# Simon-Kotchou/ViT.rs

Hardware: AMD Instinct MI355X
Metric: images/sec (train step) ViT-B/16 224² bf16 at 1/2/4/8 MI355X; % MFMA roofline (higher is better)
Workload: dtype bf16; 1 GPU; vit_b16 224x224 train step (fwd+bwd+SGD), batch 256/GPU, bf16; model=vit_b16, global_batch=256, seq_len=197, parallelism=dp1

## Files before the change

### include/vit_ops.h

```cpp
#ifndef VIT_OPS_H
#define VIT_OPS_H

#include <stddef.h>
#include <stdint.h>

#ifdef __cplusplus
extern "C" {
#endif

int vit_init(int device);
void vit_set_stream(void* hip_stream);
void* vit_get_stream(void);
int vit_sync(void);
int vit_last_error(const char** msg);
void vit_clear_error(void);
void* vit_malloc(size_t bytes);
void vit_free(void* p);
int vit_memcpy_h2d(void* dst, const void* src, size_t bytes);
int vit_memcpy_d2h(void* dst, const void* src, size_t bytes);
int vit_memcpy_d2d(void* dst, const void* src, size_t bytes);
int vit_memset(void* dst, int value, size_t bytes);
enum {
    VIT_HIT_GEMM_128 = 0,
    VIT_HIT_GEMM_256x256 = 16,
// ... 22 lines not shown
float vit_event_elapsed_ms(void* start, void* stop);

void residual_forward(float* out, const float* inp1, const float* inp2, int N);
void matmul_forward(float* out, const float* inp, const float* weight, const float* bias,
                    int B, int T, int C, int OC);
void attention_forward(float* out, float* preatt, float* att, const float* inp,
                       int B, int T, int C, int NH);
void layernorm_forward(float* out, float* mean, float* rstd, const float* inp,
                       const float* weight, const float* bias, int B, int T, int C);
void gelu_forward(float* out, const float* inp, int N);
void softmax_forward(float* probs, const float* logits, int B, int T, int V);
void crossentropy_forward(float* losses, const float* probs, const int* targets,
                          int B, int T, int V);
void residual_backward(float* dinp1, float* dinp2, const float* dout, int N);
void matmul_backward(float* dinp, float* dweight, float* dbias, const float* dout,
                     const float* inp, const float* weight, int B, int T, int C, int OC);
void attention_backward(float* dinp, float* dpreatt, float* datt, const float* dout,
                        const float* inp, const float* att, int B, int T, int C, int NH);
void layernorm_backward(float* dinp, float* dweight, float* dbias, const float* dout,
                        const float* inp, const float* weight, const float* mean,
                        const float* rstd, int B, int T, int C);
void gelu_backward(float* dinp, const float* inp, const float* dout, int N);
void crossentropy_softmax_backward(float* dlogits, const float* dlosses, const float* probs,
                                   const int* targets, int B, int T, int V);
void softmax_crossentropy_soft_forward(float* probs, float* losses, const float* logits,
                                       const int* ta, const int* tb, float lam, float eps,
                                       int B, int T, int V);
void crossentropy_soft_softmax_backward(float* dlogits, const float* dlosses, const float* probs,
                                        const int* ta, const int* tb, float lam, float eps,
                                        int B, int T, int V);
void patch_embed_forward(float* encoded, const float* pixels, const float* patch_w,
                         const float* patch_b, const float* cls, const float* wpe,
                         int B, int IMG, int P, int C);
void patch_embed_backward(float* dpatch_w, float* dpatch_b, float* dcls, float* dwpe,
                          const float* dencoded, const float* pixels, int B, int IMG, int P,
                          int C);
void sgd_step(float* params, const float* grads, long long n, float lr);
void grad_sumsq(double* out, const float* x, long long n);

void matmul_forward_bf16(uint16_t* out, const uint16_t* inp, const uint16_t* weight,
                         const float* bias, int B, int T, int C, int OC);
void matmul_backward_bf16(float* dinp, float* dweight, float* dbias, const uint16_t* dout,
                          const uint16_t* inp, const uint16_t* weight, int B, int T, int C,
                          int OC);
int vit_attention_kernel_kind(int T, int C, int NH);
void attention_forward_fused_bf16(uint16_t* out, float* lse, const uint16_t* inp,
                                  int B, int T, int C, int NH);
void attention_backward_fused_bf16(uint16_t* dinp, const uint16_t* dout, const uint16_t* inp,
                                   const uint16_t* out, const float* lse, int B, int T, int C,
                                   int NH);
void attention_backward_fused_bf16_ex(uint16_t* dinp, const uint16_t* dout, const uint16_t* inp,
                                      const uint16_t* out, const float* lse, int B, int T, int C, int NH,
                                      float* dqkv_bias);
void layernorm_forward_bf16(uint16_t* out, float* mean, float* rstd, const float* inp,
                            const float* weight, const float* bias, int B, int T, int C);
void layernorm_backward_bf16(float* dinp, float* dweight, float* dbias, const uint16_t* dout,
                             const float* inp, const float* weight, const float* mean,
                             const float* rstd, int B, int T, int C);
void gelu_forward_bf16(uint16_t* out, const uint16_t* inp, int N);
void gelu_backward_bf16(float* dinp, const uint16_t* inp, const uint16_t* dout, int N);
void gemm_bf16_ex(void* C, long long ldc, const uint16_t* A, long long lda, int a_kcontig,
                  const uint16_t* B, long long ldb, int b_kcontig, const float* bias,
                  float* dbias, int M, int N, int K, int epi, int splitk);
void gemm_bf16_fused(void* C, void* C2, long long ldc, const void* aux, long long ldaux,
                     const uint16_t* A, long long lda, int a_kcontig, const uint16_t* B,
                     long long ldb, int b_kcontig, const float* bias, float* colsum_out, int M,
                     int N, int K, int epi);
long long mx_scale_size(long long rows, int K);
void quantize_mx_bf16_ex(uint8_t* q, uint8_t* scales, const uint16_t* x, long long R, int K,
                         long long ldx, long long ldq);
void quantize_mx_f32_ex(uint8_t* q, uint8_t* scales, const float* x, long long R, int K,
                        long long ldx, long long ldq);
long long mx_cols_padded(long long R);
void quantize_mx_cols_bf16_ex(uint8_t* q, uint8_t* scales, const uint16_t* x, long long R, int C,
                              long long ldx);
void quantize_mx_rowcol_bf16_ex(uint8_t* qr, uint8_t* scales_r, uint8_t* qc, uint8_t* scales_c,
                                const uint16_t* x, long long R, int C, long long ldx, long long ldqc,
                                long long tok_off, long long ntok);
void layernorm_backward_stream(uint16_t* dres_out, uint8_t* lo_out, const uint16_t* dres_in, const uint8_t* lo_in,
                               float* dweight, float* dbias, float* dres_colsum, const uint16_t* dout, const float* inp,
                               const float* weight, const float* mean, const float* rstd, long long R, int C);
void layernorm_backward_stream_mx(uint16_t* dres_out, uint8_t* lo_out, const uint16_t* dres_in, const uint8_t* lo_in,
                                  float* dweight, float* dbias, float* dres_colsum, const uint16_t* dout,
                                  const float* inp, const float* weight, const float* mean, const float* rstd,
                                  long long R, int C, uint8_t* qr, uint8_t* scales_r, uint8_t* qc, uint8_t* scales_c,
                                  long long ldqc, long long tok_off, long long ntok);
void layernorm_forward_mx(uint8_t* qr, uint8_t* scales_r, uint8_t* qc, uint8_t* scales_c, float* mean,
                          float* rstd, const float* inp, const float* weight, const float* bias, long long R,
                          int C, long long ldqc, long long tok_off, long long ntok);
void gemm_fp8_fused(void* C, void* C2, long long ldc, const void* aux, long long ldaux,
                    const uint8_t* A, const uint8_t* a_scale, long long lda, const uint8_t* B,
                    const uint8_t* b_scale, long long ldb, const float* bias, float* colsum_out,
                    int M, int N, int K, int epi);
void gemm_fp8_fused_mx(void* C, void* C2, long long ldc, const void* aux, long long ldaux, const uint8_t* A,
                       const uint8_t* a_scale, long long lda, const uint8_t* B, const uint8_t* b_scale,
                       long long ldb, const float* bias, float* colsum_out, int M, int N, int K, int epi,
                       uint8_t* mx_q, uint8_t* mx_s);
void gemm_fp8_fused_mxc(void* C, void* C2, long long ldc, const void* aux, long long ldaux, const uint8_t* A,
                        const uint8_t* a_scale, long long lda, const uint8_t* B, const uint8_t* b_scale,
                        long long ldb, const float* bias, float* colsum_out, int M, int N, int K, int epi,
                        uint8_t* mx_q, uint8_t* mx_s, uint8_t* mxc_q, uint8_t* mxc_s, long long mxc_ld,
                        long long mxc_off);
void gemm_bf16_set_variant(int variant);
void gemm_bf16_set_debug(int flags);
void gemm_bf16_set_trace(unsigned long long* trace);
void convert_f32_to_bf16(uint16_t* out, const float* inp, long long n);
// ... 7 lines not shown
```

### vit.rs_amd/__init__.py

```python
import ctypes
import os
import sys

import numpy as np

HERE = os.path.dirname(os.path.abspath(__file__))
LIB_PATH = os.environ.get("VIT_LIB") or os.path.join(HERE, "libvit_hip.so")

from . import data
from . import mix
from . import groups
from . import augment

VIT_FP32, VIT_BF16, VIT_FP8 = 0, 1, 2
MIX_NONE, MIX_MIXUP, MIX_CUTMIX = 0, 1, 2
_lib = None


class VitError(RuntimeError):
    pass


class VitConfigC(ctypes.Structure):
    _fields_ = [("img", ctypes.c_int), ("patch", ctypes.c_int), ("in_ch", ctypes.c_int),
# ... 10 lines not shown
    _fields_ = [("cfg", VitConfigC), ("num_params", ctypes.c_longlong), ("has_opt", ctypes.c_int),
                ("step", ctypes.c_int), ("adamw", AdamWC)]


def _cfg_c(cfg):
    return VitConfigC(cfg.img, cfg.patch, cfg.in_ch, cfg.channels, cfg.num_layers, cfg.num_heads,
                      cfg.num_classes)


def build(quiet=True):
    import subprocess
    jobs = str(min(8, os.cpu_count() or 1))
    subprocess.run(["make", "-s", "-j", jobs, "-C", HERE], check=True,
                   stdout=subprocess.DEVNULL if quiet else None)


_VOID = [("vit_clear_error", []), ("vit_set_stream", [ctypes.c_void_p]),
         ("vit_free", [ctypes.c_void_p]), ("vit_event_destroy", [ctypes.c_void_p]),
         ("vit_trainer_destroy", [ctypes.c_void_p]), ("vit_trainer_timing_reset", [ctypes.c_void_p]),
         ("vit_loader_close", [ctypes.c_void_p]), ("vit_jpeg_loader_close", [ctypes.c_void_p]), ("vit_kernel_hits_reset", [])]

P, I, LL, F, S = ctypes.c_void_p, ctypes.c_int, ctypes.c_longlong, ctypes.c_float, ctypes.c_size_t
_SIGS = {
    "vit_init": (I, [I]), "vit_get_stream": (P, []), "vit_sync": (I, []),
    "vit_last_error": (I, [ctypes.POINTER(ctypes.c_char_p)]),
    "vit_malloc": (P, [S]), "vit_memcpy_h2d": (I, [P, P, S]), "vit_memcpy_d2h": (I, [P, P, S]),
    "vit_memcpy_d2d": (I, [P, P, S]), "vit_memset": (I, [P, I, S]),
    "vit_event_create": (P, []), "vit_event_record": (I, [P]), "vit_event_elapsed_ms": (F, [P, P]),
    "residual_forward": (None, [P, P, P, I]),
    "matmul_forward": (None, [P, P, P, P, I, I, I, I]),
    "attention_forward": (None, [P, P, P, P, I, I, I, I]),
    "layernorm_forward": (None, [P, P, P, P, P, P, I, I, I]),
    "gelu_forward": (None, [P, P, I]),
    "softmax_forward": (None, [P, P, I, I, I]),
    "crossentropy_forward": (None, [P, P, P, I, I, I]),
    "residual_backward": (None, [P, P, P, I]),
    "matmul_backward": (None, [P, P, P, P, P, P, I, I, I, I]),
    "attention_backward": (None, [P, P, P, P, P, P, I, I, I, I]),
    "layernorm_backward": (None, [P, P, P, P, P, P, P, P, I, I, I]),
    "gelu_backward": (None, [P, P, P, I]),
    "crossentropy_softmax_backward": (None, [P, P, P, P, I, I, I]),
    "softmax_crossentropy_soft_forward": (None, [P, P, P, P, P, F, F, I, I, I]),
    "crossentropy_soft_softmax_backward": (None, [P, P, P, P, P, F, F, I, I, I]),
    "patch_embed_forward": (None, [P, P, P, P, P, P, I, I, I, I]),
    "patch_embed_backward": (None, [P, P, P, P, P, P, I, I, I, I]),
    "sgd_step": (None, [P, P, LL, F]),
    "grad_sumsq": (None, [P, P, LL]),
    "matmul_forward_bf16": (None, [P, P, P, P, I, I, I, I]),
    "matmul_backward_bf16": (None, [P, P, P, P, P, P, I, I, I, I]),
    "attention_forward_fused_bf16": (None, [P, P, P, I, I, I, I]),
    "vit_attention_kernel_kind": (I, [I, I, I]),
    "attention_backward_fused_bf16": (None, [P, P, P, P, P, I, I, I, I]),
    "attention_backward_fused_bf16_ex": (None, [P, P, P, P, P, I, I, I, I, P]),
    "layernorm_forward_bf16": (None, [P, P, P, P, P, P, I, I, I]),
    "layernorm_backward_bf16": (None, [P, P, P, P, P, P, P, P, I, I, I]),
    "gelu_forward_bf16": (None, [P, P, I]),
    "gelu_backward_bf16": (None, [P, P, P, I]),
    "gemm_bf16_ex": (None, [P, LL, P, LL, I, P, LL, I, P, P, I, I, I, I, I]),
    "gemm_bf16_fused": (None, [P, P, LL, P, LL, P, LL, I, P, LL, I, P, P, I, I, I, I]),
    "mx_scale_size": (LL, [LL, I]),
    "quantize_mx_bf16_ex": (None, [P, P, P, LL, I, LL, LL]),
    "quantize_mx_f32_ex": (None, [P, P, P, LL, I, LL, LL]),
    "mx_cols_padded": (LL, [LL]),
    "quantize_mx_cols_bf16_ex": (None, [P, P, P, LL, I, LL]),
    "quantize_mx_rowcol_bf16_ex": (None, [P, P, P, P, P, LL, I, LL, LL, LL, LL]),
    "layernorm_forward_mx": (None, [P, P, P, P, P, P, P, P, P, LL, I, LL, LL, LL]),
    "layernorm_backward_stream": (None, [P, P, P, P, P, P, P, P, P, P, P, P, LL, I]),
    "layernorm_backward_stream_mx": (None, [P, P, P, P, P, P, P, P, P, P, P, P, LL, I, P, P, P, P, LL, LL, LL]),
    "gemm_fp8_fused": (None, [P, P, LL, P, LL, P, P, LL, P, P, LL, P, P, I, I, I, I]),
    "gemm_fp8_fused_mx": (None, [P, P, LL, P, LL, P, P, LL, P, P, LL, P, P, I, I, I, I, P, P]),
    "gemm_fp8_fused_mxc": (None, [P, P, LL, P, LL, P, P, LL, P, P, LL, P, P, I, I, I, I, P, P, P, P, LL, LL]),
    "gemm_bf16_set_variant": (None, [I]), "gemm_bf16_set_debug": (None, [I]),
    "gemm_bf16_set_trace": (None, [P]),
    "vit_kernel_hits": (I, [P, I]),
    "convert_f32_to_bf16": (None, [P, P, LL]),
    "convert_bf16_to_f32": (None, [P, P, LL]),
    "vit_trainer_create": (P, [ctypes.POINTER(VitConfigC), I, I, I]),
    "vit_trainer_num_params": (LL, [P]), "vit_trainer_device_bytes": (LL, [P]),
    "vit_trainer_set_params": (I, [P, P]), "vit_trainer_get_params": (I, [P, P]),
    "vit_trainer_get_grads": (I, [P, P]), "vit_trainer_set_batch": (I, [P, P, P]),
    "vit_trainer_set_batch_device": (I, [P, P, P]),
    "vit_trainer_set_label_smoothing": (I, [P, F]),
    "vit_trainer_mix_batch": (I, [P, I, F, I, I, I, I]),
    "vit_trainer_get_pixels": (I, [P, P]),
    "vit_trainer_forward": (I, [P, I]), "vit_trainer_zero_grad": (I, [P]),
    "vit_trainer_backward": (I, [P]), "vit_trainer_step": (I, [P, F]),
    "vit_trainer_train_step": (I, [P, F, I]), "vit_trainer_mean_loss": (F, [P]),
    "vit_trainer_get_logits": (I, [P, P]), "vit_trainer_sync": (I, [P]),
    "vit_trainer_stream": (P, [P]),
    "vit_layout_query": (I, [ctypes.POINTER(VitConfigC), P, P, ctypes.POINTER(LL)]),
    "vit_dp_unique_id_size": (I, []), "vit_dp_get_unique_id": (I, [ctypes.c_char_p]),
    "vit_trainer_dp_init": (I, [P, I, I, ctypes.c_char_p, I]),
    "vit_trainer_dp_ranks": (I, [P]),
    "vit_trainer_get_dp_snapshot": (I, [P, P]),
    "vit_trainer_set_timing": (I, [P, I]), "vit_trainer_set_concurrency": (I, [P, I]),
    "vit_trainer_set_option": (I, [P, ctypes.c_char_p, I]),
    "vit_trainer_timing": (I, [P, ctypes.POINTER(ctypes.c_char_p), ctypes.POINTER(ctypes.c_double),
                               ctypes.POINTER(ctypes.c_longlong), ctypes.POINTER(ctypes.c_double), I]),
    "vit_trainer_step_adamw": (I, [P, F, F, F, F, F]),
    "vit_trainer_get_adamw_state": (I, [P, P, P, ctypes.POINTER(I)]),
    "vit_trainer_set_grad_clip": (I, [P, F]), "vit_trainer_grad_norm": (F, [P]),
    "vit_trainer_set_param_groups": (I, [P, P, P]),
    "vit_trainer_get_param_groups": (I, [P, P, P, ctypes.POINTER(I)]),
    "vit_trainer_eval": (I, [P, P, ctypes.POINTER(I)]),
    "vit_config_num_params": (LL, [ctypes.POINTER(VitConfigC)]),
    "vit_checkpoint_read_info": (I, [ctypes.c_char_p, P]),
# ... 591 lines not shown
```

### vit.rs_amd/csrc/attention.hip

```cpp
#include <string>

#include "attn_fused.h"

namespace vit {

__global__ __launch_bounds__(256) void attn_fwd_f32_k(float* __restrict__ out,
                                                      float* __restrict__ preatt,
                                                      float* __restrict__ att,
                                                      const float* __restrict__ inp, int B, int T,
                                                      int C, int NH) {
    extern __shared__ float sc[];
    const int lane = threadIdx.x & 63, w = threadIdx.x >> 6;
    const long long nrows = (long long)B * T * NH;
    const long long bth = blockIdx.x * 4LL + w;
    const bool valid = bth < nrows;
    const int hs = C / NH;
    const long long C3 = 3LL * C;
    const float scale = 1.0f / sqrtf((float)hs);
    float* s = sc + w * T;
    long long b = 0, t = 0, h = 0;
    if (valid) {
        b = bth / ((long long)T * NH);
        t = (bth / NH) % T;
        h = bth % NH;
// ... 440 lines not shown
    }
}

bool attn_fused_supported(int T, int C, int NH) {
    return NH > 0 && C % NH == 0 && T >= 1 && T <= fa_max_t(C / NH) && C % 8 == 0 && !getenv("VIT_ATTN_GENERIC");
}

__global__ __launch_bounds__(256) void attn_colsum_part_k(float* __restrict__ scratch, const float* __restrict__ part,
                                                          int R, int NH, int C, int HS) {
    __shared__ float4 red[256];
    const int sh = blockIdx.x, sct = sh / NH, h = sh - sct * NH, ch = blockIdx.y, nch = gridDim.y;
    const int lpr = HS / 4, nb = 256 / lpr, d4 = threadIdx.x % lpr, lb = threadIdx.x / lpr;
    const int r0 = (int)((long long)R * ch / nch), r1 = (int)((long long)R * (ch + 1) / nch);
    float4 t[4] = {};
    const long long rs = (long long)NH * 3 * HS;
    const float* base = part + (long long)h * 3 * HS + sct * HS + 4 * d4;
    int r = lb < nb ? r0 + lb : r1;
    for (; r + 3 * nb < r1; r += 4 * nb)
#pragma unroll
        for (int u = 0; u < 4; u++) {
            const float4 v = *reinterpret_cast<const float4*>(base + (long long)(r + u * nb) * rs);
            t[u].x += v.x; t[u].y += v.y; t[u].z += v.z; t[u].w += v.w;
        }
    for (; r < r1; r += nb) {
        const float4 v = *reinterpret_cast<const float4*>(base + (long long)r * rs);
        t[0].x += v.x; t[0].y += v.y; t[0].z += v.z; t[0].w += v.w;
    }
    red[threadIdx.x] = make_float4(t[0].x + t[1].x + t[2].x + t[3].x, t[0].y + t[1].y + t[2].y + t[3].y,
                                   t[0].z + t[1].z + t[2].z + t[3].z, t[0].w + t[1].w + t[2].w + t[3].w);
    __syncthreads();
    if (lb == 0) {
        float4 a = red[d4];
        for (int j = 1; j < nb; j++) {
            const float4 b = red[j * lpr + d4];
            a.x += b.x; a.y += b.y; a.z += b.z; a.w += b.w;
        }
        *reinterpret_cast<float4*>(scratch + (long long)ch * 3 * C + sct * C + h * HS + 4 * d4) = a;
    }
}
__global__ __launch_bounds__(256) void attn_colsum_final_k(float* __restrict__ out, const float* __restrict__ scratch,
                                                           int nch, int C3, int store) {
    const int j = blockIdx.x * 256 + threadIdx.x;
    if (j >= C3) return;
    float a = 0.f;
    for (int ch = 0; ch < nch; ch++) a += scratch[(long long)ch * C3 + j];
    out[j] = store ? a : out[j] + a;
}

size_t attn_backward_ws_floats(int B, int T, int C, int NH) {
    const size_t per_bh = std::max((size_t)T, (size_t)3 * (C / NH) * (fa::ATTN_PART_ROWS + 1));
    return (size_t)B * NH * per_bh + (size_t)cdiv((long long)B * T, 256) * 3 * C;
}

void attn_forward_fused(bf16_t* out, float* lse, const bf16_t* qkv, int B, int T, int C, int NH,
                        hipStream_t s) {
    if (!attn_fused_supported(T, C, NH)) {
        if (!attn_generic_supported(T, C, NH)) {
            set_error("attention_forward_fused: unsupported shape (T=%d C=%d NH=%d)", T, C, NH);
            return;
        }
        const size_t lds = gen::lds_bytes(T, C / NH, gen::nw_fwd(C / NH));
        switch (C / NH) {
#define VIT_GEN_FWD(HS)                                                                              \
    case HS:                                                                                         \
        if (!gen_lds_attr((const void*)gen::fwd_k<HS>, lds)) { set_error("attention: LDS attribute"); return; } \
        gen::fwd_k<HS><<<dim3(B * NH, gen::CHUNKS), gen::nw_fwd(HS) * 64, lds, s>>>(out, lse, qkv, T, C, NH); \
        break;
            VIT_GEN_FWD(32) VIT_GEN_FWD(64) VIT_GEN_FWD(80) VIT_GEN_FWD(96) VIT_GEN_FWD(128)
#undef VIT_GEN_FWD
            default: set_error("attention: no generic kernel for head size %d", C / NH); return;
        }
        after_launch("attention_forward_generic");
        count_hit(VIT_HIT_ATTN_GENERIC);
        return;
    }
    bool ok = false;
    switch (C / NH) {
        case 32: ok = fa_forward_h32(out, lse, qkv, B, T, C, NH, s); break;
        case 64: ok = fa_forward_h64(out, lse, qkv, B, T, C, NH, s); break;
        case 80: ok = fa_forward_h80(out, lse, qkv, B, T, C, NH, s); break;
        case 96: ok = fa_forward_h96(out, lse, qkv, B, T, C, NH, s); break;
        case 128: ok = fa_forward_h128(out, lse, qkv, B, T, C, NH, s); break;
    }
    if (!ok) { set_error("fused attention: no kernel for T=%d head size %d", T, C / NH); return; }
    after_launch("attention_forward_fused");
}

void attn_backward_fused(bf16_t* dqkv, const bf16_t* dout, const bf16_t* qkv, const bf16_t* out,
                         const float* lse, int B, int T, int C, int NH, hipStream_t s,
                         float* dqkv_colsum, float* ws, bool colsum_store) {
    if (!attn_fused_supported(T, C, NH)) {
        if (!attn_generic_supported(T, C, NH)) {
            set_error("attention_backward_fused: unsupported shape (T=%d C=%d NH=%d)", T, C, NH);
            return;
        }
        if (!ws) ws = (float*)workspace(attn_backward_ws_floats(B, T, C, NH) * sizeof(float));
        if (!ws) return;
        const size_t lds = gen::lds_bytes(T, C / NH, gen::nw_bwd(C / NH));
        const dim3 g(B * NH, gen::CHUNKS);
        switch (C / NH) {
#define VIT_GEN_BWD(HS)                                                                            \
    case HS:                                                                                       \
        if (!gen_lds_attr((const void*)gen::bwd_q_k<HS>, lds) ||                                   \
            !gen_lds_attr((const void*)gen::bwd_kv_k<HS>, lds)) {                                  \
            set_error("attention: LDS attribute");                                                 \
            return;                                                                                \
        }                                                                                          \
        gen::bwd_q_k<HS><<<g, gen::nw_bwd(HS) * 64, lds, s>>>(dqkv, ws, dout, qkv, out, lse, T, C, NH);    \
        gen::bwd_kv_k<HS><<<g, gen::nw_bwd(HS) * 64, lds, s>>>(dqkv, ws, dout, qkv, lse, T, C, NH);        \
        break;
            VIT_GEN_BWD(32) VIT_GEN_BWD(64) VIT_GEN_BWD(80) VIT_GEN_BWD(96) VIT_GEN_BWD(128)
#undef VIT_GEN_BWD
            default: set_error("attention: no generic kernel for head size %d", C / NH); return;
        }
        after_launch("attention_backward_generic");
        count_hit(VIT_HIT_ATTN_GENERIC);
        if (dqkv_colsum) {
            if (colsum_store) VIT_HIP(hipMemsetAsync(dqkv_colsum, 0, 3 * (size_t)C * sizeof(float), s));
            colsum_bf16(dqkv_colsum, dqkv, B * T, 3 * C, 3LL * C, s, ws + (size_t)B * NH * T);
        }
        return;
    }
    const int HS = C / NH;
    if (!ws) ws = (float*)workspace(attn_backward_ws_floats(B, T, C, NH) * sizeof(float));
    if (!ws) return;
    float* part = dqkv_colsum ? ws : nullptr;
    int rows = 0;
    switch (HS) {
        case 32: rows = fa_backward_h32(dqkv, dout, qkv, out, lse, B, T, C, NH, part, s); break;
        case 64: rows = fa_backward_h64(dqkv, dout, qkv, out, lse, B, T, C, NH, part, s); break;
        case 80: rows = fa_backward_h80(dqkv, dout, qkv, out, lse, B, T, C, NH, part, s); break;
        case 96: rows = fa_backward_h96(dqkv, dout, qkv, out, lse, B, T, C, NH, part, s); break;
        case 128: rows = fa_backward_h128(dqkv, dout, qkv, out, lse, B, T, C, NH, part, s); break;
    }
    if (!rows) { set_error("fused attention backward: no kernel for T=%d head size %d", T, HS); return; }
    after_launch("attention_backward_fused");
    if (dqkv_colsum) {
        const int nch = std::min(8, B);
        float* scratch = part + (size_t)B * rows * NH * 3 * HS;
        attn_colsum_part_k<<<dim3(3 * NH, nch), 256, 0, s>>>(scratch, part, B * rows, NH, C, HS);
        attn_colsum_final_k<<<cdiv(3 * C, 256), 256, 0, s>>>(dqkv_colsum, scratch, nch, 3 * C, colsum_store ? 1 : 0);
        after_launch("attention_colsum_reduce");
    }
}

}

using namespace vit;
extern "C" {
void attention_forward(float* out, float* preatt, float* att, const float* inp, int B, int T, int C,
                       int NH) {
    attn_forward_f32(out, preatt, att, inp, B, T, C, NH, stream());
}
void attention_backward(float* dinp, float* dpreatt, float* datt, const float* dout,
                        const float* inp, const float* att, int B, int T, int C, int NH) {
    attn_backward_f32(dinp, dpreatt, datt, dout, inp, att, B, T, C, NH, stream());
}
int vit_attention_kernel_kind(int T, int C, int NH) {
    if (attn_fused_supported(T, C, NH)) return 1;
    if (attn_generic_supported(T, C, NH)) return 2;
    return 0;
}
void attention_forward_fused_bf16(uint16_t* out, float* lse, const uint16_t* inp, int B, int T,
                                  int C, int NH) {
    attn_forward_fused(out, lse, inp, B, T, C, NH, stream());
}
void attention_backward_fused_bf16(uint16_t* dinp, const uint16_t* dout, const uint16_t* inp,
                                   const uint16_t* out, const float* lse, int B, int T, int C,
                                   int NH) {
    attn_backward_fused(dinp, dout, inp, out, lse, B, T, C, NH, stream());
}
void attention_backward_fused_bf16_ex(uint16_t* dinp, const uint16_t* dout, const uint16_t* inp,
                                      const uint16_t* out, const float* lse, int B, int T, int C, int NH,
                                      float* dqkv_bias) {
    attn_backward_fused(dinp, dout, inp, out, lse, B, T, C, NH, stream(), dqkv_bias);
}
}
```

### vit.rs_amd/csrc/attn_fused.h

```cpp
#pragma once
#include "ops_internal.h"

namespace vit {
namespace fa {

#ifndef VIT_ATTN_DIAG
#define VIT_ATTN_DIAG 0
#endif
#if VIT_ATTN_DIAG & 4
static __device__ unsigned long long attn_trace[8 * 16 * 16 * 16];
#define ATTN_STAMP(k)                                                                                   \
    do {                                                                                                \
        if (blockIdx.x < 8 && it < 16 && lane == 0)                                                     \
            attn_trace[((blockIdx.x * 16 + it) * 16 + w) * 16 + (k)] = __builtin_amdgcn_s_memtime();   \
    } while (0)
#else
#define ATTN_STAMP(k) \
    do {              \
    } while (0)
#endif

constexpr float LOG2E = 1.4426950408889634f;

template <int HS>
// ... 116 lines not shown
__device__ __forceinline__ void store4(bf16_t* dst, f32x4_t v, float mul) {
    *reinterpret_cast<uint2*>(dst) = pack4_bf16(v, mul);
}

__device__ __forceinline__ __amdgpu_buffer_rsrc_t buf_rsrc(const void* base, uint32_t bytes) {
    return __builtin_amdgcn_make_buffer_rsrc(const_cast<void*>(base), (short)0, (int)bytes, 0x00020000);
}
__device__ __forceinline__ uint4 buf_ld16(__amdgpu_buffer_rsrc_t r, uint32_t off) {
    return __builtin_bit_cast(uint4, __builtin_amdgcn_raw_buffer_load_b128(r, off, 0, 0));
}
__device__ __forceinline__ float buf_ldf(__amdgpu_buffer_rsrc_t r, uint32_t off) {
    return __builtin_bit_cast(float, __builtin_amdgcn_raw_buffer_load_b32(r, off, 0, 0));
}
typedef uint32_t v2u32_t __attribute__((ext_vector_type(2)));
template <int HS>
__device__ __forceinline__ bf16x8_t frag_buf(__amdgpu_buffer_rsrc_t r, uint32_t ld_bytes, int row, int s, int lane) {
    const uint32_t off = (uint32_t)row * ld_bytes + 2u * (32 * s + 4 * (lane >> 4));
    const bf16x4_t lo = __builtin_bit_cast(bf16x4_t, __builtin_amdgcn_raw_buffer_load_b64(r, off, 0, 0));
    bf16x4_t hi = {};
    if (!(Geo<HS>::HALF && s == Geo<HS>::KS - 1))
        hi = __builtin_bit_cast(bf16x4_t, __builtin_amdgcn_raw_buffer_load_b64(r, off + 32, 0, 0));
    return __builtin_shufflevector(lo, hi, 0, 1, 2, 3, 4, 5, 6, 7);
}

__device__ __forceinline__ int gray8(int r) { return (r ^ (r >> 1)) & 7; }
__device__ __forceinline__ int sl_off(int row, int byte) { return row * 128 + ((((byte >> 4) ^ gray8(row)) << 4) | (byte & 15)); }
__device__ __forceinline__ int ds_off(int row, int byte) { return row * 64 + ((((byte >> 3) ^ gray8(row)) << 3) | (byte & 7)); }
__device__ __forceinline__ bf16x4_t lds4(const char* img, int off) { return *reinterpret_cast<const bf16x4_t*>(img + off); }
__device__ __forceinline__ bf16x4_t lds4tr(const char* img, int off) {
    return __builtin_amdgcn_ds_read_tr16_b64_v4bf16(LDS_PTR(bf16x4_t, img + off));
}
__device__ __forceinline__ bf16x8_t frag_row_sw(const char* img, int r0, int s, int lane) {
    const int i = lane & 15, g = lane >> 4;
    return __builtin_shufflevector(lds4(img, sl_off(r0 + i, 64 * s + 8 * g)), lds4(img, sl_off(r0 + i, 64 * s + 32 + 8 * g)),
                                   0, 1, 2, 3, 4, 5, 6, 7);
}
__device__ __forceinline__ bf16x8_t frag_tr_sw(const char* img, int kb, int c0, int lane) {
    const int i = lane & 15, g = lane >> 4, r = kb + 4 * g + (i >> 2), b = 2 * c0 + 8 * (i & 3);
    return __builtin_shufflevector(lds4tr(img, sl_off(r, b)), lds4tr(img, sl_off(r + 16, b)), 0, 1, 2, 3, 4, 5, 6, 7);
}
__device__ __forceinline__ bf16x8_t frag_tr_ds(const char* img, int kb, int c0, int lane) {
    const int i = lane & 15, g = lane >> 4, r = kb + 4 * g + (i >> 2), b = 2 * c0 + 8 * (i & 3);
    return __builtin_shufflevector(lds4tr(img, ds_off(r, b)), lds4tr(img, ds_off(r + 16, b)), 0, 1, 2, 3, 4, 5, 6, 7);
}

template <int HS, int NKT>
constexpr int fwd_lds_bytes() { return NKT * 16 * (Geo<HS>::SK + Geo<HS>::SV) * 2; }
template <int HS, int NKT>
constexpr int fwd_occ() { return fwd_lds_bytes<HS, NKT>() <= 80 * 1024 ? 2 : 1; }

#ifndef VIT_ATTN_FWD_BUF
#define VIT_ATTN_FWD_BUF 1
#endif
template <int HS, int NKT, int NS = NKT>
__global__ __launch_bounds__(256, (fwd_occ<HS, NKT>())) void attn_fwd_k(bf16_t* __restrict__ out,
                                                                        float* __restrict__ lse,
                                                                        const bf16_t* __restrict__ qkv,
                                                                        int T, int C, int NH) {
    using G = Geo<HS>;
    constexpr int TP = NKT * 16;
    __shared__ __attribute__((aligned(16))) bf16_t Ks[TP * G::SK];
    __shared__ __attribute__((aligned(16))) bf16_t Vs[TP * G::SV];
    const int bh = blockIdx.x, b = bh / NH, h = bh % NH;
    const long long C3 = 3LL * C;
    const bf16_t* base = qkv + (long long)b * T * C3 + h * HS;
    const int lane = threadIdx.x & 63, w = threadIdx.x >> 6, i = lane & 15, g = lane >> 4;
    [[maybe_unused]] int it = 15;
    ATTN_STAMP(0);
    [[maybe_unused]] const auto rq = buf_rsrc(base, (uint32_t)(T * C3 * 2));
    [[maybe_unused]] const auto ro = buf_rsrc(out + (long long)b * T * C + h * HS, (uint32_t)(T * C * 2));
    [[maybe_unused]] const auto rl = buf_rsrc(lse + (long long)bh * T, (uint32_t)(T * 4));
    auto load_q = [&](int qt, bf16x8_t (&qf)[G::KS]) {
#pragma unroll
        for (int s = 0; s < G::KS; s++) {
            if constexpr (VIT_ATTN_FWD_BUF) qf[s] = frag_buf<HS>(rq, (uint32_t)(C3 * 2), qt * 16 + i, s, lane);
            else qf[s] = frag_glb<HS>(base, C3, qt * 16 + i, T, s, lane);
        }
    };
    const int nqt = (T + 15) / 16;
    bf16x8_t qn[G::KS];
    load_q(w, qn);
    if constexpr (VIT_ATTN_FWD_BUF) {
        const auto rkv = buf_rsrc(base + C, (uint32_t)(T * C3 * 2 - 2 * C));
        constexpr int CH = G::CH, PER = (TP * CH + 255) / 256;
        uint4 v[2][PER];
#pragma unroll
        for (int o = 0; o < 2; o++)
#pragma unroll
            for (int j = 0; j < PER; j++) {
                const int idx = j * 256 + (int)threadIdx.x, t = idx / CH, cc = idx - t * CH;
                v[o][j] = buf_ld16(rkv, (uint32_t)t * (uint32_t)(C3 * 2) + (uint32_t)(o * C * 2) + 16 * cc);
            }
#pragma unroll
        for (int o = 0; o < 2; o++)
#pragma unroll
            for (int j = 0; j < PER; j++) {
                const int idx = j * 256 + (int)threadIdx.x, t = idx / CH, cc = idx - t * CH;
                if ((TP * CH) % 256 == 0 || idx < TP * CH)
                    *reinterpret_cast<uint4*>((o ? Vs + t * G::SV : Ks + t * G::SK) + cc * 8) = v[o][j];
            }
    } else {
        bf16_t* const img[2] = {Ks, Vs};
        const int st[2] = {G::SK, G::SV};
        const bf16_t* const src[2] = {base + C, base + 2 * C};
        const long long ld[2] = {C3, C3};
        load_images<HS, TP, 256, 2>(img, st, src, ld, T);
    }
    ATTN_STAMP(1);
    __syncthreads();
    ATTN_STAMP(2);
    const float c = LOG2E / sqrtf((float)HS);
#ifndef VIT_ATTN_FWD_SPLIT
#define VIT_ATTN_FWD_SPLIT 1
#endif
    const RowBases<HS> kb(Ks, G::SK, lane);
    for (int qt = w; qt < nqt; qt += 4) {
        const int q = qt * 16 + i;
        it = qt / 4;
        ATTN_STAMP(0);
        bf16x8_t qf[G::KS];
#pragma unroll
        for (int s = 0; s < G::KS; s++) qf[s] = qn[s];
        if (qt + 4 < nqt) load_q(qt + 4, qn);
        f32x4_t sacc[NKT];
#pragma unroll
        for (int kt = NS; kt < NKT; kt++) sacc[kt] = f32x4_t{0.f, 0.f, 0.f, 0.f};
#pragma unroll
        for (int kt = 0; kt < NS; kt++) {
            f32x4_t a = {0.f, 0.f, 0.f, 0.f};
#pragma unroll
            for (int s = 0; s < G::KS; s++) {
                if constexpr (VIT_ATTN_FWD_SPLIT) a = mfma(kb.frag(kt * 16, G::SK, s), qf[s], a);
// ... 1011 lines not shown
        bwd_slice_b<HS, NSL, NW, XK>(Ks, dSs, dq, C3, q0, T, scale, w, lane, xds_s, xk_s);
        ATTN_STAMP(4);
        __syncthreads();
        ATTN_STAMP(5);
    }
    it = 15;
    ATTN_STAMP(6);
    constexpr int NWR = NW + (XK ? 1 : 0);
    bwd_item_end<HS>(R, dq, C, key0, T, scale,
                     dsum ? dsum + ((long long)(b * NWR + w) * NH + h) * 3 * HS : nullptr, lane, it);
    ATTN_STAMP(7);
    if constexpr (XK) {
        if (xo >= 0) {
            const int o = xo, d = o < HS ? o : o - HS;
            const float v = o < HS ? xacc * scale : xacc;
            dq[(long long)(T - 1) * C3 + (o < HS ? C : 2 * C) + d] = f2bf(v);
            if (dsum) {
                float* row = dsum + ((long long)(b * NWR + NW) * NH + h) * 3 * HS;
                row[(o < HS ? HS : 2 * HS) + d] = v;
                if (o < HS) row[d] = scale * xsds * xk_s[d];
            }
        }
    }
}

template <int HS, int NKT, int KK = 2>
#ifndef VIT_ATTN_SKEW
#define VIT_ATTN_SKEW 1
#endif

struct Bwdp {
    using G = Geo<HS>;
    static constexpr int TP = NKT * 16, NW = NKT / KK, NT = NW * 64, NSL = TP / 32, CH = G::CH;
    static constexpr int SK = G::SK, SV = G::SV, SL = slice_stride<HS>(), SDS = sds_stride<HS>();
    static constexpr int K_OFF = 0;
    static constexpr int V_OFF = K_OFF + 2 * TP * SV * 2;
    static constexpr int Q_OFF = V_OFF + TP * SK * 2;
    static constexpr int D_OFF = Q_OFF + 2 * 32 * SL * 2;
    static constexpr int NDS = VIT_ATTN_SKEW ? 2 : 1;
    static constexpr int S_OFF = D_OFF + 2 * 32 * SL * 2;
    static constexpr int L_OFF = S_OFF + NDS * TP * SDS * 2;
    static constexpr int E_OFF = L_OFF + 2 * TP * 4;
    static constexpr int BYTES = E_OFF + 2 * 32 * 4;
    static constexpr int PER = (32 * CH + NT - 1) / NT;
    static constexpr int PERS = (2 * 32 * CH + NT - 1) / NT;
};
template <int HS, int NKT, int KK = 2>
constexpr bool bwdp_fits() {
    using Z = Bwdp<HS, NKT, KK>;
    return Z::BYTES <= 160 * 1024 && (64 % Geo<HS>::CH) == 0 && HS <= 64 && Z::NW <= ATTN_PART_ROWS &&
           NKT % KK == 0 && (KK == 2 ? bwd1_fits<HS, NKT>() : KK == 4 ? (HS == 64 && Z::NW <= 4) : Z::NW <= 16);
}

template <int HS, int NKT, int KK>
__global__ __launch_bounds__(NKT / KK * 64, 1) void attn_bwdp_k(bf16_t* __restrict__ dqkv,
                                                               const bf16_t* __restrict__ dout,
                                                               const bf16_t* __restrict__ qkv,
                                                               const bf16_t* __restrict__ out,
                                                               const float* __restrict__ lse, int T,
                                                               int C, int NH, int BH, float* __restrict__ dsum,
                                                               int stagger) {
    using G = Geo<HS>;
    using Z = Bwdp<HS, NKT, KK>;
    if (stagger > 0 && ((blockIdx.x >> 3) & 1)) {
        const uint64_t t0 = __builtin_amdgcn_s_memrealtime();
        while (__builtin_amdgcn_s_memrealtime() - t0 < (uint64_t)stagger) __builtin_amdgcn_s_sleep(8);
    }
    constexpr int TP = Z::TP, NW = Z::NW, NT = Z::NT, NSL = Z::NSL, SK = Z::SK, SV = Z::SV, SL = Z::SL;
    static_assert((32 * G::CH) % 64 == 0 && NT % 64 == 0, "slice pieces are whole waves");
    constexpr int KS = G::KS, CH = G::CH, PER = Z::PER, PERS = Z::PERS;
    __shared__ __attribute__((aligned(16))) char lds[Z::BYTES];
    bf16_t* Kimg = reinterpret_cast<bf16_t*>(lds + Z::K_OFF);
    bf16_t* Vst = reinterpret_cast<bf16_t*>(lds + Z::V_OFF);
    bf16_t* Qs = reinterpret_cast<bf16_t*>(lds + Z::Q_OFF);
    bf16_t* Ds = reinterpret_cast<bf16_t*>(lds + Z::D_OFF);
    bf16_t* dSs = reinterpret_cast<bf16_t*>(lds + Z::S_OFF);
    float* lse_s = reinterpret_cast<float*>(lds + Z::L_OFF);
    float* del_s = reinterpret_cast<float*>(lds + Z::E_OFF);
    const long long C3 = 3LL * C;
    const int tid = threadIdx.x, lane = tid & 63;
    const int w = __builtin_amdgcn_readfirstlane(tid >> 6);
    const int key0 = w * 16 * KK;
#ifndef VIT_ATTN_SLICE_ALL
#define VIT_ATTN_SLICE_ALL 0
#endif
    constexpr bool SPLIT_SLICE = !VIT_ATTN_SLICE_ALL && Bwdp<HS, NKT, KK>::PER == 1 && (32 * G::CH) % 64 == 0;
    const bool slice_wave = !SPLIT_SLICE || w < 32 * G::CH / 64;
    const float scale = 1.0f / sqrtf((float)HS);
    const float c = LOG2E * scale;
    auto qkv_of = [&](int bh) { return qkv + (long long)(bh / NH) * T * C3 + (bh % NH) * HS; };
    auto row_of = [&](const bf16_t* p, int bh) { return p + (long long)(bh / NH) * T * C + (bh % NH) * HS; };
    uint4 pq[PER], pd[PER], po[PER];
    struct Src { __amdgpu_buffer_rsrc_t q, d, o, kv, l; };
    auto src_of = [&](int bh) {
        Src r;
        r.q = buf_rsrc(qkv_of(bh), (uint32_t)(T * C3 * 2));
        r.d = buf_rsrc(row_of(dout, bh), (uint32_t)(T * C * 2));
        r.o = buf_rsrc(row_of(out, bh), (uint32_t)(T * C * 2));
        r.kv = buf_rsrc(qkv_of(bh) + C, (uint32_t)(T * C3 * 2 - 2 * C));
        r.l = buf_rsrc(lse + (long long)bh * T, (uint32_t)(T * 4));
        return r;
    };
    auto fetch_slice = [&](const Src& sr, int q0) {
        const auto rq = sr.q, rd = sr.d, ro = sr.o;
#pragma unroll
        for (int j = 0; j < PER; j++) {
            const int idx = (j * NT + tid) % (32 * CH), t = idx / CH, cc = idx - t * CH;
            const uint32_t r = (uint32_t)(q0 + t);
            pq[j] = buf_ld16(rq, r * (uint32_t)(C3 * 2) + 16 * cc);
            pd[j] = buf_ld16(rd, r * (uint32_t)(C * 2) + 16 * cc);
            po[j] = buf_ld16(ro, r * (uint32_t)(C * 2) + 16 * cc);
        }
    };
    auto put_slice = [&](int buf) {
#pragma unroll
        for (int j = 0; j < PER; j++) {
            const int idx = (j * NT + tid) % (32 * CH), t = idx / CH, cc = idx - t * CH;
            float dl = dot8_bf16(po[j], pd[j]);
#pragma unroll
            for (int o = 1; o < CH; o <<= 1) dl += __shfl_xor(dl, o, 64);
            slice_put<HS>(Qs + buf * 32 * SL, t, cc, pq[j]);
            slice_put<HS>(Ds + buf * 32 * SL, t, cc, pd[j]);
            if (cc == 0) del_s[buf * 32 + t] = dl;
        }
    };
    uint4 ps[PERS];
    float lse_n = INFINITY;
    auto fetch_side = [&](const Src& sr, int rb) {
        const auto rk = sr.kv;
#pragma unroll
        for (int j = 0; j < PERS; j++) {
            const int idx = (j * NT + tid) % (64 * CH), op = idx >= 32 * CH, rem = idx - op * 32 * CH, t = rem / CH,
                      cc = rem - t * CH, row = 32 * rb + t;
            ps[j] = buf_ld16(rk, (uint32_t)row * (uint32_t)(C3 * 2) + (uint32_t)(op * C * 2) + 16 * cc);
        }
    };
    auto put_side = [&](int kbuf, int rb) {
#pragma unroll
        for (int j = 0; j < PERS; j++) {
            const int idx = (j * NT + tid) % (64 * CH), op = idx >= 32 * CH, rem = idx - op * 32 * CH, t = rem / CH,
                      cc = rem - t * CH, row = 32 * rb + t;
            bf16_t* dst = op ? Vst + row * SK : Kimg + kbuf * TP * SV + row * SV;
            *reinterpret_cast<uint4*>(dst + cc * 8) = ps[j];
        }
    };
    auto load_kv = [&](BwdRegs<HS, KK>& R, int kbuf) {
#pragma unroll
        for (int kk = 0; kk < KK; kk++)
#pragma unroll
            for (int s = 0; s < KS; s++) {
                R.kf[kk][s] = frag_row<HS>(Kimg + kbuf * TP * SV, SV, key0 + 16 * kk, s, lane);
                R.vf[kk][s] = frag_row<HS>(Vst, SK, key0 + 16 * kk, s, lane);
            }
    };
    int bh = blockIdx.x;
    if (bh >= BH) return;
    fetch_slice(src_of(bh), 0);
    {
        bf16_t* const img[2] = {Kimg, Vst};
        const int st[2] = {SV, SK};
        const bf16_t* const src[2] = {qkv_of(bh) + C, qkv_of(bh) + 2 * C};
        const long long ld[2] = {C3, C3};
        load_images<HS, TP, NT, 2>(img, st, src, ld, T);
    }
    for (int t = tid; t < TP; t += NT) lse_s[t] = t < T ? lse[(long long)bh * T + t] : INFINITY;
    put_slice(0);
    if constexpr ((VIT_ATTN_DIAG & 1) != 0) fetch_side(src_of(bh), 0);
    __syncthreads();
    BwdRegs<HS, KK> R;
    load_kv(R, 0);
    int kb = 0, it = 0;
#pragma unroll 1
    for (int n = 0; bh < BH; n++, bh += gridDim.x) {
        const int bhn = bh + gridDim.x;
        const bool has_next = bhn < BH;
        const int bhc = has_next ? bhn : bh;
        const Src s_cur = src_of(bh), s_nxt = src_of(bhc);
        bf16_t* dq = dqkv + (long long)(bh / NH) * T * C3 + (bh % NH) * HS;
        const float* lse_cur = lse_s + (n & 1) * TP;
        R.zero();
#pragma unroll 1
        for (int sl = 0; sl < NSL; sl++, it++) {
            const int cur = it & 1, q0 = sl * 32;
            ATTN_STAMP(0);
            if constexpr (!(VIT_ATTN_DIAG & 1)) {
                if (slice_wave) {
                    if (sl + 1 < NSL) fetch_slice(s_cur, q0 + 32);
                    else fetch_slice(s_nxt, 0);
                }
                fetch_side(s_nxt, sl);
                if (sl == 0) lse_n = buf_ldf(s_nxt.l, 4 * tid);
            }
            if constexpr (VIT_ATTN_SKEW) {
                bf16_t* dS_a = dSs + (sl & 1) * TP * Z::SDS;
                bwd_slice_a<HS, KK>(R, Qs + cur * 32 * SL, Ds + cur * 32 * SL, lse_cur + q0, del_s + cur * 32,
                                    dS_a + key0 * Z::SDS, c, lane);
                ATTN_STAMP(1);
                if (sl > 0)
                    bwd_slice_b<HS, NSL, NW>(Kimg + kb * TP * SV, dSs + ((sl - 1) & 1) * TP * Z::SDS, dq, C3,
                                             q0 - 32, T, scale, w, lane);
                ATTN_STAMP(2);
                if (slice_wave) put_slice(cur ^ 1);
                if (sl == 0 && tid < TP) lse_s[((n + 1) & 1) * TP + tid] = tid < T ? lse_n : INFINITY;
                ATTN_STAMP(3);
                __syncthreads();
                ATTN_STAMP(4);
                put_side(kb ^ 1, sl);
                ATTN_STAMP(5);
            } else {
                bwd_slice_a<HS, KK>(R, Qs + cur * 32 * SL, Ds + cur * 32 * SL, lse_cur + q0, del_s + cur * 32,
                                    dSs + key0 * Z::SDS, c, lane);
                __syncthreads();
                put_slice(cur ^ 1);
                put_side(kb ^ 1, sl);
                if (sl == 0 && tid < TP) lse_s[((n + 1) & 1) * TP + tid] = tid < T ? lse_n : INFINITY;
                bwd_slice_b<HS, NSL, NW>(Kimg + kb * TP * SV, dSs, dq, C3, q0, T, scale, w, lane);
                __syncthreads();
            }
        }
        if constexpr (VIT_ATTN_SKEW) {
            bwd_slice_b<HS, NSL, NW>(Kimg + kb * TP * SV, dSs + ((NSL - 1) & 1) * TP * Z::SDS, dq, C3,
                                     (NSL - 1) * 32, T, scale, w, lane);
            __syncthreads();
        }
        ATTN_STAMP(6);
        bwd_item_end<HS, KK>(R, dq, C, key0, T, scale,
                             dsum ? dsum + ((long long)((bh / NH) * NW + w) * NH + bh % NH) * 3 * HS : nullptr, lane,
                             it);
        ATTN_STAMP(7);
        if (has_next) {
            kb ^= 1;
            load_kv(R, kb);
        }
    }
}

template <int HS>
constexpr int max_tp() {
    int tp = 32;
    while (tp + 32 <= 320 && (tp + 32) * (Geo<HS>::SK + Geo<HS>::SV) * 2 <= 160 * 1024 &&
           2 * (tp + 32) * Geo<HS>::SK * 2 + 2 * (tp + 32) * 4 + 8 * HS * 4 <= 160 * 1024)
        tp += 32;
    return tp;
}

template <int HS, int NKT>
bool launch_fwd(bf16_t* out, float* lse, const bf16_t* qkv, int B, int T, int C, int NH, hipStream_t s) {
    if (T > NKT * 16 || T <= (NKT - 2) * 16) return false;
#ifndef VIT_ATTN_FWD_TRIM
#define VIT_ATTN_FWD_TRIM 1
#endif
    if (VIT_ATTN_FWD_TRIM && (NKT - 1) * 16 >= T)
        attn_fwd_k<HS, NKT, NKT - 1><<<B * NH, 256, 0, s>>>(out, lse, qkv, T, C, NH);
    else
        attn_fwd_k<HS, NKT><<<B * NH, 256, 0, s>>>(out, lse, qkv, T, C, NH);
    count_hit(VIT_HIT_ATTN_FWD_MFMA);
    return true;
}
int attn_bwd_variant();
int attn_cu_count();
template <int HS, int NKT>
int launch_bwd(bf16_t* dqkv, const bf16_t* dout, const bf16_t* qkv, const bf16_t* out, const float* lse, int B,
               int T, int C, int NH, float* part, hipStream_t s) {
    const int v = attn_bwd_variant(), BH = B * NH;
    constexpr int NK4 = (NKT + 7) / 8 * 8;
    if constexpr (bwdp_fits<HS, NK4, 4>()) {
        if (v == 4) {
            attn_bwdp_k<HS, NK4, 4><<<std::min(BH, attn_cu_count()), NK4 / 4 * 64, 0, s>>>(dqkv, dout, qkv, out, lse,
                                                                                          T, C, NH, BH, part, 0);
            count_hit(VIT_HIT_ATTN_BWD_PERSISTENT);
            return NK4 / 4;
        }
    }
    if constexpr (bwdp_fits<HS, NKT, 2>()) {
        if (v == 0) {
            static const int stagger = [] {
                const char* e = getenv("VIT_ATTN_STAGGER");
                return e ? atoi(e) : 0;
            }();
            attn_bwdp_k<HS, NKT, 2><<<std::min(BH, attn_cu_count()), NKT / 2 * 64, 0, s>>>(dqkv, dout, qkv, out, lse,
                                                                                         T, C, NH, BH, part, stagger);
            count_hit(VIT_HIT_ATTN_BWD_PERSISTENT);
            return NKT / 2;
        }
    }
    if constexpr (bwd1_fits<HS, NKT>()) {
        if (v != 2) {
            attn_bwd1_k<HS, NKT><<<BH, NKT / 2 * 64, 0, s>>>(dqkv, dout, qkv, out, lse, T, C, NH, part);
            count_hit(VIT_HIT_ATTN_BWD_ONEPASS);
            return NKT / 2;
        }
    }
    if constexpr (NKT > 2 && bwd1_fits_xk<HS, NKT - 2>()) {
        if (v != 2 && T == (NKT - 2) * 16 + 1) {
            constexpr int NW = (NKT - 2) / 2;
            attn_bwd1_k<HS, NKT - 2, true><<<BH, NW * 64, 0, s>>>(dqkv, dout, qkv, out, lse, T, C, NH, part);
            count_hit(VIT_HIT_ATTN_BWD_XKEY);
            return NW + 1;
        }
    }
    attn_bwd_pair_k<HS, NKT><<<2 * cdiv(BH, 8) * 8, 256, 0, s>>>(dqkv, dout, qkv, out, lse, T, C, NH, BH, part);
    count_hit(VIT_HIT_ATTN_BWD_PAIR);
    return 1;
}
template <int HS, int NKT = 2>
bool dispatch_fwd(int nkt, bf16_t* out, float* lse, const bf16_t* qkv, int B, int T, int C, int NH,
                  hipStream_t s) {
    if constexpr (NKT * 16 > max_tp<HS>()) {
        return false;
    } else {
        if (nkt == NKT) return launch_fwd<HS, NKT>(out, lse, qkv, B, T, C, NH, s);
        return dispatch_fwd<HS, NKT + 2>(nkt, out, lse, qkv, B, T, C, NH, s);
    }
}
template <int HS, int NKT = 2>
int dispatch_bwd(int nkt, bf16_t* dqkv, const bf16_t* dout, const bf16_t* qkv, const bf16_t* out,
                 const float* lse, int B, int T, int C, int NH, float* part, hipStream_t s) {
    if constexpr (NKT * 16 > max_tp<HS>()) {
        return 0;
    } else {
        if (nkt == NKT) return launch_bwd<HS, NKT>(dqkv, dout, qkv, out, lse, B, T, C, NH, part, s);
        return dispatch_bwd<HS, NKT + 2>(nkt, dqkv, dout, qkv, out, lse, B, T, C, NH, part, s);
    }
}

}

#define VIT_FA_DECLARE(HS)                                                                         \
    bool fa_forward_h##HS(bf16_t* out, float* lse, const bf16_t* qkv, int B, int T, int C, int NH, \
                          hipStream_t s);                                                          \
    int fa_backward_h##HS(bf16_t* dqkv, const bf16_t* dout, const bf16_t* qkv, const bf16_t* out, \
                          const float* lse, int B, int T, int C, int NH, float* part, hipStream_t s); \
    int fa_max_t_h##HS();
VIT_FA_DECLARE(32)
VIT_FA_DECLARE(64)
VIT_FA_DECLARE(80)
VIT_FA_DECLARE(96)
VIT_FA_DECLARE(128)

#define VIT_FA_DEFINE(HS)                                                                           \
    bool fa_forward_h##HS(bf16_t* out, float* lse, const bf16_t* qkv, int B, int T, int C, int NH,  \
                          hipStream_t s) {                                                          \
        return fa::dispatch_fwd<HS>(cdiv(T, 32) * 2, out, lse, qkv, B, T, C, NH, s);                \
    }                                                                                               \
    int fa_backward_h##HS(bf16_t* dqkv, const bf16_t* dout, const bf16_t* qkv, const bf16_t* out,   \
                          const float* lse, int B, int T, int C, int NH, float* part, hipStream_t s) { \
        return fa::dispatch_bwd<HS>(cdiv(T, 32) * 2, dqkv, dout, qkv, out, lse, B, T, C, NH, part, s); \
    }                                                                                               \
    int fa_max_t_h##HS() { return fa::max_tp<HS>(); }

}
```

### vit.rs_amd/csrc/gemm.h

```cpp
#pragma once
#include "common.h"

namespace vit {

enum Epi {
    EPI_F32_STORE = 0,
    EPI_F32_ACC = 1,
    EPI_F32_ATOMIC = 2,
    EPI_BF16_STORE = 3,
    EPI_BF16_GELU = 4,
    EPI_F32_RESID = 5,
    EPI_BF16_DGELU = 6,
    EPI_F32_SLAB = 7,
    EPI_BF16_GELU_D = 8,
    EPI_BF16_MUL = 9,
};
constexpr bool epi_aux16(int e) { return e == EPI_BF16_DGELU || e == EPI_BF16_MUL; }
constexpr bool epi_bias(int e) { return e != EPI_F32_ATOMIC && e != EPI_F32_SLAB && !epi_aux16(e); }
constexpr bool epi_mx(int e) { return e == EPI_BF16_GELU || e == EPI_BF16_GELU_D || epi_aux16(e); }

struct GemmArgs {
    const void* A = nullptr;
    long long lda = 0;
    bool a_kcontig = true;
    const void* B = nullptr;
    long long ldb = 0;
    bool b_kcontig = true;
    void* C = nullptr;
    long long ldc = 0;
    void* C2 = nullptr;
    const void* aux = nullptr;
    long long ldaux = 0;
    const float* bias = nullptr;
    float* dbias = nullptr;
    float* colsum_out = nullptr;
    float* colsum_part = nullptr;
    int M = 0, N = 0, K = 0;
    int epi = EPI_F32_STORE;
    int splitk = 0;
    int fill_pct = 0;
    bool rows_gathered = false;
    float* ws = nullptr;
    size_t ws_bytes = 0;
    const void* a_scale = nullptr;
    const void* b_scale = nullptr;
    uint8_t* mx_q = nullptr;
    uint8_t* mx_s = nullptr;
    uint8_t* mxc_q = nullptr;
    uint8_t* mxc_s = nullptr;
    long long mxc_ld = 0;
    long long mxc_off = 0;
};

void gemm_f32(const GemmArgs& a, hipStream_t s);
void gemm_bf16(const GemmArgs& a, hipStream_t s);
bool gemm_bf16_supported(const GemmArgs& a);
void gemm_set_variant(int v);
void gemm_set_debug(int flags);
int gemm_cu_count();
int gemm_persist_grid();
struct GemmParams;
void gemm_set_trace(unsigned long long* trace);
bool gemm_pp_shape(const GemmArgs& a);
void gemm_bf16_pp(const GemmArgs& a, const GemmParams& p, hipStream_t s);
int gemm_colsum_rows(const GemmArgs& a, bool fp8);
bool gemm_streaming();

void gemm_fp8(const GemmArgs& a, hipStream_t s);
bool gemm_fp8_supported(const GemmArgs& a);
void quantize_mx_bf16(uint8_t* q, uint8_t* sl, const bf16_t* x, long long R, int K, long long ldx,
                      long long ldq, hipStream_t s);
void quantize_mx_f32(uint8_t* q, uint8_t* sl, const float* x, long long R, int K, long long ldx,
                     long long ldq, hipStream_t s);
void quantize_mx_batched_bf16(uint8_t* q, uint8_t* sl, const bf16_t* x, long long R, int K, int count,
                              long long xs, long long qs, long long ss, hipStream_t s);
void quantize_mx_batched_f32(uint8_t* q, uint8_t* sl, const float* x, long long R, int K, int count,
                             long long xs, long long qs, long long ss, hipStream_t s);
void quantize_mx_cols_bf16(uint8_t* q, uint8_t* sl, const bf16_t* x, long long R, int C, long long ldx, hipStream_t s);
void quantize_mx_cols_batched_bf16(uint8_t* q, uint8_t* sl, const bf16_t* x, long long R, int C, long long ldx,
                                   int count, long long xs, long long qs, long long ss, hipStream_t s);
bool quantize_mx_rowcol_bf16(uint8_t* qr, uint8_t* slr, uint8_t* qc, uint8_t* slc, const bf16_t* x, long long R,
                             int C, long long ldx, long long ldqc, long long tok_off, long long ntok, hipStream_t s);
long long mx_cols_kp(long long R);
long long mx_rows_padded(long long rows);
size_t mx_scale_bytes(long long rows, int K);
bool ln_forward_mx_supported(int C);
bool ln_backward_mx_supported(int C);
bool ln_backward_bf16_stream_mx(bf16_t* dres_out, uint8_t* lo_out, const bf16_t* dres_in, const uint8_t* lo_in,
                                float* dw, float* db, float* dres_colsum, const bf16_t* dout, const float* inp,
// ... 23 lines not shown
```

### vit.rs_amd/csrc/gemm.hip

```cpp
#include "gemm_common.h"

#include <cstdlib>

#ifndef VIT_G2_ONEPHASE
#define VIT_G2_ONEPHASE 0
#endif

namespace vit {

namespace bf {
constexpr int BM = 128, BN = 128, BK = 64, NT = 256;
constexpr int SK = 72;
constexpr int SMN = 144;
constexpr int TILE = 9216;
static_assert(BM * SK == TILE && BK * SMN == TILE, "image sizes");

template <bool KC, int ROWS>
struct Stager {
    uint4 r[4];
    __device__ __forceinline__ void load(const bf16_t* __restrict__ base, long long ld, int row0,
                                         int rows_lim, int k0, int k_lim, int tid) {
#pragma unroll
        for (int c = 0; c < 4; c++) {
            const int idx = c * NT + tid;
// ... 909 lines not shown
        const long long e = i * 4;
        const int m = (int)(e / N), n = (int)(e - (long long)m * N);
        float4 acc = reinterpret_cast<const float4*>(slab)[i];
        for (int z = 1; z < splits; z++) {
            const float4 t = *reinterpret_cast<const float4*>(slab + z * plane + e);
            acc.x += t.x; acc.y += t.y; acc.z += t.z; acc.w += t.w;
        }
        float4* c = reinterpret_cast<float4*>(C + (long long)m * ldc + n);
        float4 o = *c;
        o.x += acc.x; o.y += acc.y; o.z += acc.z; o.w += acc.w;
        *c = o;
    }
}

static int g_variant = -1;
static int g_debug_flags = 0;
static bool known_variant(int v) { return v == 1 || v == 2 || v == 7 || v == 11; }
static constexpr int kDefaultVariant = 7;
static int gemm_variant() {
    if (g_variant < 0) {
        const char* e = getenv("VIT_GEMM");
        g_variant = e ? atoi(e) : kDefaultVariant;
        if (!known_variant(g_variant)) g_variant = kDefaultVariant;
    }
    return g_variant;
}
void gemm_set_variant(int v) { g_variant = known_variant(v) ? v : -1; }
int gemm_cu_count() {
    static int n = [] {
        int dev = 0, cu = 0;
        (void)hipGetDevice(&dev);
        (void)hipDeviceGetAttribute(&cu, hipDeviceAttributeMultiprocessorCount, dev);
        return cu > 0 ? cu : 256;
    }();
    return n;
}
int gemm_persist_grid() {
    static const int n = [] {
        const char* e = getenv("VIT_PERSIST_CUS");
        const int v = e ? atoi(e) : 0;
        return v >= 64 && v <= gemm_cu_count() ? v : gemm_cu_count();
    }();
    return n;
}
bool gemm_streaming() { return gemm_variant() == 7 || gemm_variant() == 11; }
void gemm_set_debug(int flags) { g_debug_flags = flags; }
static int g_debug_flags_fwd() { return g_debug_flags; }
static unsigned long long* g_trace = nullptr;
void gemm_set_trace(unsigned long long* trace) { g_trace = trace; }

GemmParams make_gemm_params(const GemmArgs& a, int kchunk) {
    GemmParams p;
    p.A = a.A; p.B = a.B; p.C = a.C; p.C2 = a.C2; p.aux = a.aux; p.bias = a.bias; p.dbias = a.dbias; p.colsum_out = nullptr;
    p.lda = a.lda; p.ldb = a.ldb; p.ldc = a.ldc; p.ldaux = a.ldaux;
    if (g_debug_flags & 32) p.ldc = 0;
    p.M = a.M; p.N = a.N; p.K = a.K; p.kchunk = kchunk;
    p.no_epi = (g_debug_flags & 2) ? 1 : 0;
    p.dbg = g_debug_flags & 0xF0;
    static const int gm_env = [] {
        const char* e = getenv("VIT_GEMM_GM");
        return e && *e ? atoi(e) : -1;
    }();
    const int gm_dbg = (g_debug_flags >> 16) & 0xF;
    p.gm = gm_dbg ? gm_dbg - 1 : gm_env >= 0 ? gm_env : (a.K <= 768 ? 8 : 0);
    p.stagger = ((g_debug_flags >> 8) & 0xFF) * 50;
    p.trace = g_trace;
    p.mx_q = a.mx_q;
    p.mx_s = a.mx_s;
    p.mx_rg = (int)(mx_rows_padded(a.M) / 32);
    p.mxc_q = a.mxc_q;
    p.mxc_s = a.mxc_s;
    p.mxc_ld = a.mxc_ld;
    p.mxc_off = (int)a.mxc_off;
    p.mxc_rg = (int)(mx_rows_padded(a.N) / 32);
    p.tiles = 1;
    return p;
}

int choose_split_waves(int tiles, int nk) {
    const int slots = 256;
    int best = 1;
    double best_eff = 0.0;
    for (int s = 1; s <= 32 && nk / s >= 16; s++) {
        const int blocks = tiles * s;
        const int waves = (blocks + slots - 1) / slots;
        const double eff = (double)blocks / (waves * (double)slots) * (blocks >= slots / 2 ? 1.0 : blocks / (slots / 2.0));
        if (eff > best_eff + 1e-9) { best_eff = eff; best = s; }
        if (eff >= 0.9) break;
    }
    return best;
}

static int choose_split(int tiles, int K, int ktile, int want_blocks) {
    int nk = cdiv(K, ktile);
    int s = 1;
    while (tiles * s < want_blocks && nk / (s * 2) >= 8) s *= 2;
    return s;
}

static int grid_blocks(long long n) {
    long long b = (n + 255) / 256;
    return (int)(b < 1 ? 1 : (b > 4096 ? 4096 : b));
}
float* slab_buffer(const GemmArgs& a, int split) {
    const size_t need = (size_t)split * a.M * a.N * sizeof(float);
    float* slab = a.ws ? (a.ws_bytes >= need ? a.ws : nullptr) : (float*)workspace(need);
// ... 144 lines not shown
        if (eff > best_eff + 1e-9) { best_eff = eff; best = s; }
        if (eff >= 0.9) break;
    }
    return best;
}

static void gemm_bf16_g4(const GemmArgs& a, hipStream_t s) {
    const int tiles = cdiv(a.M, g4::BM) * cdiv(a.N, g4::BN);
    int split = a.splitk > 0 ? a.splitk : choose_split_g4(tiles, a.K / g4::KTILE, a.fill_pct);
    int kchunk = cdiv(cdiv(a.K, split), g4::KTILE) * g4::KTILE;
    split = cdiv(a.K, kchunk);
    GemmArgs b = a;
    float* slab = nullptr;
    if (split > 1) {
        if (!(slab = slab_buffer(a, split))) return;
        b.epi = EPI_F32_SLAB;
        b.C = slab;
        b.ldc = a.N;
    } else {
        b.epi = EPI_F32_ACC;
    }
    GemmParams p = make_gemm_params(b, kchunk);
    p.tiles = tiles;
    dim3 grid(tiles, split);
    if (slab) g4::gemm_kernel<EPI_F32_SLAB><<<grid, g4::NT, 0, s>>>(p);
    else g4::gemm_kernel<EPI_F32_ACC><<<grid, g4::NT, 0, s>>>(p);
    after_launch("gemm_bf16_256x128");
    count_hit(VIT_HIT_GEMM_256x128 + b.epi);
    if (slab) slab_reduce(a, slab, split, s);
    if (a.dbias) colsum_bf16(a.dbias, (const bf16_t*)a.A, a.K, a.M, a.lda, s);
}

void gemm_bf16(const GemmArgs& a, hipStream_t s) {
    if (a.M <= 0 || a.N <= 0) return;
    if (a.mx_q || a.mxc_q) {
        set_error("gemm_bf16: the fused MX output is an fp8-engine feature");
        return;
    }
    if (!gemm_bf16_supported(a)) {
        set_error("gemm_bf16: unsupported shape/alignment M=%d N=%d K=%d lda=%lld ldb=%lld",
                  a.M, a.N, a.K, a.lda, a.ldb);
        return;
    }
    if (gemm_variant() != 1 && a.epi == EPI_F32_ATOMIC && !a.a_kcontig && !a.b_kcontig &&
        a.K % g4::KTILE == 0 && a.M >= 256 && a.N >= 128 && a.N % 4 == 0 &&
        (a.splitk > 0 || !a.ws ||
         (size_t)choose_split_g4(cdiv(a.M, g4::BM) * cdiv(a.N, g4::BN), a.K / g4::KTILE) * a.M * a.N * sizeof(float) <=
             a.ws_bytes)) {
        gemm_bf16_g4(a, s);
        return;
    }
    const bool gathered = a.rows_gathered && a.M >= 1 && a.a_kcontig && a.epi != EPI_F32_ATOMIC;
    const bool big = a.K % g2::KTILE == 0 && (a.M >= 256 || gathered) && a.N >= 256 && gemm_variant() != 1;
    if (big) {
        const int tiles = cdiv(a.M, g2::BM) * cdiv(a.N, g2::BN);
        int split = 1;
        if (a.epi == EPI_F32_ATOMIC) split = a.splitk > 0 ? a.splitk : choose_split_waves(tiles, a.K / g2::KTILE);
        int kchunk = cdiv(cdiv(a.K, split), g2::KTILE) * g2::KTILE;
        split = cdiv(a.K, kchunk);
        GemmArgs b = a;
        float* slab = nullptr;
        if (a.epi == EPI_F32_ATOMIC) {
            if (split > 1) {
                if (!(slab = slab_buffer(a, split))) return;
                b.epi = EPI_F32_SLAB;
                b.C = slab;
                b.ldc = a.N;
            } else {
                b.epi = EPI_F32_ACC;
            }
        }
        GemmParams p = make_gemm_params(b, kchunk);
        p.tiles = tiles;
        float* cs_rows = colsum_rows_begin(a);
        if ((a.colsum_out || a.colsum_part) && epi_aux16(a.epi) && !cs_rows) return;
        p.colsum_out = cs_rows;
        const bool late_db = a.dbias && !a.a_kcontig && split > 1;
        if (late_db) p.dbias = nullptr;
        if (split == 1 && pp_taken(b)) {
            gemm_bf16_pp(b, p, s);
            after_launch("gemm_bf16_pp");
            count_hit(VIT_HIT_GEMM_256x256 + b.epi);
            count_hit(VIT_HIT_GEMM_PP);
            colsum_rows_end(a, cs_rows, s);
            return;
        }
        dim3 grid(tiles, split);
        if (a.a_kcontig && a.b_kcontig) launch_g2<true, true>(b, p, grid, s);
        else if (a.a_kcontig && !a.b_kcontig) launch_g2<true, false>(b, p, grid, s);
        else if (!a.a_kcontig && !a.b_kcontig) launch_g2<false, false>(b, p, grid, s);
        else launch_g2<false, true>(b, p, grid, s);
        after_launch("gemm_bf16_256");
        count_hit(VIT_HIT_GEMM_256x256 + b.epi);
        if (slab) slab_reduce(a, slab, split, s);
        colsum_rows_end(a, cs_rows, s);
        if (late_db) colsum_bf16(a.dbias, (const bf16_t*)a.A, a.K, a.M, a.lda, s);
        return;
    }
    const int tiles = cdiv(a.M, bf::BM) * cdiv(a.N, bf::BN);
    int split = 1;
    if (a.epi == EPI_F32_ATOMIC) split = a.splitk > 0 ? a.splitk : choose_split(tiles, a.K, bf::BK, 512);
    int kchunk = cdiv(cdiv(a.K, split), bf::BK) * bf::BK;
    if (kchunk <= 0) kchunk = bf::BK;
    split = cdiv(a.K > 0 ? a.K : 1, kchunk);
    GemmArgs b = a;
    float* slab = nullptr;
    if (a.epi == EPI_F32_ATOMIC) {
        if (split > 1) {
            if (!(slab = slab_buffer(a, split))) return;
            b.epi = EPI_F32_SLAB; b.C = slab; b.ldc = a.N;
        } else {
            b.epi = EPI_F32_ACC;
        }
    }
    GemmParams p = make_gemm_params(b, kchunk);
    const bool late_db = a.dbias && !a.a_kcontig && split > 1;
    if (late_db) p.dbias = nullptr;
    dim3 grid(tiles, split);
    if (a.a_kcontig && a.b_kcontig) launch_bf16<true, true>(b, p, grid, s);
    else if (a.a_kcontig && !a.b_kcontig) launch_bf16<true, false>(b, p, grid, s);
    else if (!a.a_kcontig && !a.b_kcontig) launch_bf16<false, false>(b, p, grid, s);
    else launch_bf16<false, true>(b, p, grid, s);
    after_launch("gemm_bf16");
    count_hit(VIT_HIT_GEMM_128 + b.epi);
    if (slab) slab_reduce(a, slab, split, s);
    if (late_db) colsum_bf16(a.dbias, (const bf16_t*)a.A, a.K, a.M, a.lda, s);
    if ((a.colsum_out || a.colsum_part) && epi_aux16(a.epi)) {
        float* rows = colsum_rows_begin(a);
        if (!rows) return;
// ... 16 lines not shown
```

### vit.rs_amd/csrc/gemm_common.h

```cpp
#pragma once
#include "gemm.h"

namespace vit {

struct GemmParams {
    const void* A;
    const void* B;
    void* C;
    void* C2;
    const void* aux;
    const float* bias;
    float* dbias;
    float* colsum_out;
    long long lda, ldb, ldc, ldaux;
    int M, N, K;
    int kchunk;
    int no_epi;
    int dbg;
    int stagger;
    unsigned long long* trace;
    int tiles;
    int gm;
    uint8_t* mx_q;
    uint8_t* mx_s;
    int mx_rg;
    uint8_t* mxc_q;
    uint8_t* mxc_s;
    long long mxc_ld;
    int mxc_off, mxc_rg;
};

__device__ __forceinline__ int mx_scale_byte(float amax) {
    if (!(amax > 0.f)) return 127;
    const uint32_t u = __float_as_uint(amax);
    const int e = (int)((u >> 23) & 0xff), mant = (int)(u & 0x7fffff);
    int s = e - 8 + (mant > 0x600000 ? 1 : 0);
    return s < 0 ? 0 : (s > 254 ? 254 : s);
}
__device__ __forceinline__ void mx_out8(const GemmParams& p, int m, int n, uint32_t w0, uint32_t w1, uint32_t w2,
                                        uint32_t w3, int lane) {
    const uint32_t w[4] = {w0, w1, w2, w3};
    float v[8];
#pragma unroll
    for (int e = 0; e < 4; e++) {
        v[2 * e] = __uint_as_float(w[e] << 16);
        v[2 * e + 1] = __uint_as_float(w[e] & 0xffff0000u);
    }
    float amax = 0.f;
#pragma unroll
    for (int j = 0; j < 8; j++) amax = fmaxf(amax, fabsf(v[j]));
    amax = fmaxf(amax, __shfl_xor(amax, 1, 64));
    amax = fmaxf(amax, __shfl_xor(amax, 2, 64));
    const int sb = mx_scale_byte(amax);
    if ((lane & 3) == 0) {
        const int kb = n >> 5;
        p.mx_s[((long long)(kb >> 1) * p.mx_rg + (m >> 5)) * 64 + (kb & 1) * 32 + (m & 31)] = (uint8_t)sb;
    }
    const float inv = __uint_as_float((uint32_t)(254 - sb) << 23);
    int t0 = __builtin_amdgcn_cvt_pk_fp8_f32(v[0] * inv, v[1] * inv, 0, false);
    t0 = __builtin_amdgcn_cvt_pk_fp8_f32(v[2] * inv, v[3] * inv, t0, true);
    int t1 = __builtin_amdgcn_cvt_pk_fp8_f32(v[4] * inv, v[5] * inv, 0, false);
    t1 = __builtin_amdgcn_cvt_pk_fp8_f32(v[6] * inv, v[7] * inv, t1, true);
    *reinterpret_cast<uint2*>(p.mx_q + (long long)m * p.N + n) = make_uint2((uint32_t)t0, (uint32_t)t1);
}

__device__ __forceinline__ void stage_back8(float* w, uint32_t w0, uint32_t w1, uint32_t w2, uint32_t w3) {
// ... 150 lines not shown
        const float4 o1 = reinterpret_cast<const float4*>(q)[1];
        v[0] += o0.x; v[1] += o0.y; v[2] += o0.z; v[3] += o0.w;
        v[4] += o1.x; v[5] += o1.y; v[6] += o1.z; v[7] += o1.w;
        st_f32(q);
    } else if constexpr (EPI == EPI_F32_SLAB) {
        st_f32((float*)p.C + (long long)split_index(p.tiles) * p.M * p.ldc + off);
    } else if constexpr (EPI == EPI_BF16_STORE) {
        *reinterpret_cast<uint4*>((bf16_t*)p.C + off) = pack8(v);
    } else if constexpr (EPI == EPI_BF16_GELU) {
        float gv[8];
#pragma unroll
        for (int j = 0; j < 8; j++) gv[j] = gelu_fast_f(v[j]);
        *reinterpret_cast<uint4*>((bf16_t*)p.C + off) = pack8(v);
        const uint4 g8 = pack8(gv);
        if (p.C2) *reinterpret_cast<uint4*>((bf16_t*)p.C2 + off) = g8;
        if constexpr (MX) {
            if (p.mx_q) mx_out8(p, m, n, g8.x, g8.y, g8.z, g8.w, lane);
            if (wb) stage_back8(wb, g8.x, g8.y, g8.z, g8.w);
        }
    } else if constexpr (EPI == EPI_F32_RESID) {
        const float* r = (const float*)p.aux + (long long)m * p.ldaux + n;
        const float4 r0 = reinterpret_cast<const float4*>(r)[0];
        const float4 r1 = reinterpret_cast<const float4*>(r)[1];
        v[0] += r0.x; v[1] += r0.y; v[2] += r0.z; v[3] += r0.w;
        v[4] += r1.x; v[5] += r1.y; v[6] += r1.z; v[7] += r1.w;
        st_f32((float*)p.C + off);
    } else if constexpr (EPI == EPI_BF16_GELU_D) {
        float gv[8], dv[8];
#pragma unroll
        for (int j = 0; j < 8; j++) gelu_pair_fast_f(v[j], gv[j], dv[j]);
        *reinterpret_cast<uint4*>((bf16_t*)p.C + off) = pack8(dv);
        const uint4 g8 = pack8(gv);
        if (p.C2) *reinterpret_cast<uint4*>((bf16_t*)p.C2 + off) = g8;
        if constexpr (MX) {
            if (p.mx_q) mx_out8(p, m, n, g8.x, g8.y, g8.z, g8.w, lane);
            if (wb) stage_back8(wb, g8.x, g8.y, g8.z, g8.w);
        }
    } else if constexpr (epi_aux16(EPI)) {
        const uint4 h = *reinterpret_cast<const uint4*>((const bf16_t*)p.aux + (long long)m * p.ldaux + n);
        const uint32_t hw[4] = {h.x, h.y, h.z, h.w};
        {
#pragma clang fp contract(off)
#pragma unroll
        for (int j = 0; j < 4; j++) {
            const float lo = __uint_as_float(hw[j] << 16), hi = __uint_as_float(hw[j] & 0xffff0000u);
            if constexpr (EPI == EPI_BF16_DGELU) {
                v[2 * j] *= gelu_grad_fast_f(lo);
                v[2 * j + 1] *= gelu_grad_fast_f(hi);
            } else {
                v[2 * j] *= lo;
                v[2 * j + 1] *= hi;
            }
        }
#pragma unroll
        for (int j = 0; j < 8; j++) cs[j] += v[j];
        }
        const uint4 d8 = pack8(v);
        if (p.C) *reinterpret_cast<uint4*>((bf16_t*)p.C + off) = d8;
        if constexpr (MX) {
            if (p.mx_q) mx_out8(p, m, n, d8.x, d8.y, d8.z, d8.w, lane);
            if (wb) stage_back8(wb, d8.x, d8.y, d8.z, d8.w);
        }
    }
}

constexpr int STG_LD = 68;
constexpr int STG_WAVE_BYTES = 64 * STG_LD * 4;
typedef unsigned int epi_u32x4v __attribute__((ext_vector_type(4)));
template <int EPI>
struct EpiAux {
    static constexpr bool AUX16 = epi_aux16(EPI);
    static constexpr bool AUX32 = EPI == EPI_F32_RESID || EPI == EPI_F32_ACC;
    static constexpr int N = AUX16 ? 8 : (AUX32 ? 16 : 0);
    epi_u32x4v ax[N > 0 ? N : 1];
    __device__ __forceinline__ void load(const GemmParams& p, int rr, int mrow, int n) {
        if constexpr (AUX16) {
#pragma unroll
            for (int it = 0; it < 8; it++)
                ax[it] = epi_ld16(p, (const bf16_t*)p.aux + (long long)(mrow + it * 8 + rr) * p.ldaux + n);
        } else if constexpr (AUX32) {
            const float* src = EPI == EPI_F32_RESID ? (const float*)p.aux : (const float*)p.C;
            const long long ld = EPI == EPI_F32_RESID ? p.ldaux : p.ldc;
#pragma unroll
            for (int it = 0; it < 8; it++) {
                const float* q = src + (long long)(mrow + it * 8 + rr) * ld + n;
                ax[2 * it] = epi_ld16(p, q);
                ax[2 * it + 1] = epi_ld16(p, q + 4);
            }
        }
    }
};
template <int EPI>
__device__ __forceinline__ void staged_pass_interior(const GemmParams& p, const float* st, int rr,
                                                     int cc, int mrow, int n, float (&cs)[8],
                                                     const float* bpre, const EpiAux<EPI>* pre = nullptr) {
    const int cc_lane = cc >> 3;
    typedef unsigned int u32x4 __attribute__((ext_vector_type(4)));
    float bv[8] = {0.f, 0.f, 0.f, 0.f, 0.f, 0.f, 0.f, 0.f};
    if constexpr (epi_bias(EPI)) {
        if (bpre) {
#pragma unroll
            for (int j = 0; j < 8; j++) bv[j] = bpre[j];
        } else if (p.bias) {
            const float4 b0 = *reinterpret_cast<const float4*>(p.bias + n);
            const float4 b1 = *reinterpret_cast<const float4*>(p.bias + n + 4);
            bv[0] = b0.x; bv[1] = b0.y; bv[2] = b0.z; bv[3] = b0.w;
            bv[4] = b1.x; bv[5] = b1.y; bv[6] = b1.z; bv[7] = b1.w;
        }
// ... 94 lines not shown
        const f32x4_t lo = *reinterpret_cast<const f32x4_t*>(st + r * STG_LD + cc);
        const f32x4_t hi = *reinterpret_cast<const f32x4_t*>(st + r * STG_LD + cc + 4);
        v[0] = lo[0]; v[1] = lo[1]; v[2] = lo[2]; v[3] = lo[3];
        v[4] = hi[0]; v[5] = hi[1]; v[6] = hi[2]; v[7] = hi[3];
        const int m = m0 + pass * 64 + r, n = n0 + cc;
        if (m >= p.M) continue;
        if (n + 8 <= p.N) {
            epilogue8<EPI>(p, m, n, v, cs, lane,
                           epi_mx(EPI) && p.mxc_q ? const_cast<float*>(st) + r * STG_LD + cc : nullptr);
        } else if (n + 4 <= p.N) {
            f32x4_t t = lo;
            epilogue<EPI>(p, m, n, t);
            if constexpr (epi_aux16(EPI)) {
#pragma clang fp contract(off)
                cs[0] += t[0];
                cs[1] += t[1];
                cs[2] += t[2];
                cs[3] += t[3];
            }
        }
    }
}
__device__ __forceinline__ void mx_cols_pass(const GemmParams& p, const float* st, int lane, int mrow, int n0) {
    if (mrow >= p.M) return;
    typedef unsigned int u32x4 __attribute__((ext_vector_type(4)));
    const int c = n0 + lane;
#pragma unroll
    for (int b = 0; b < 2; b++) {
        float v[32];
        float amax = 0.f;
#pragma unroll
        for (int i = 0; i < 32; i++) {
            v[i] = st[(32 * b + i) * STG_LD + lane];
            amax = fmaxf(amax, fabsf(v[i]));
        }
        const int sb = mx_scale_byte(amax);
        const int tok = p.mxc_off + mrow + 32 * b, kb = tok >> 5;
        p.mxc_s[((long long)(kb >> 1) * p.mxc_rg + (c >> 5)) * 64 + (kb & 1) * 32 + (c & 31)] = (uint8_t)sb;
        const float inv = __uint_as_float((uint32_t)(254 - sb) << 23);
        uint32_t w[8];
#pragma unroll
        for (int j = 0; j < 8; j++) {
            int t = __builtin_amdgcn_cvt_pk_fp8_f32(v[4 * j] * inv, v[4 * j + 1] * inv, 0, false);
            t = __builtin_amdgcn_cvt_pk_fp8_f32(v[4 * j + 2] * inv, v[4 * j + 3] * inv, t, true);
            w[j] = (uint32_t)t;
        }
        uint8_t* dst = p.mxc_q + (long long)c * p.mxc_ld + tok;
        *reinterpret_cast<u32x4*>(dst) = u32x4{w[0], w[1], w[2], w[3]};
        *reinterpret_cast<u32x4*>(dst + 16) = u32x4{w[4], w[5], w[6], w[7]};
    }
}
template <int EPI>
__device__ __forceinline__ bool staged_interior(const GemmParams& p, int m0, int n0) {
    return EPI != EPI_F32_ATOMIC && m0 + 128 <= p.M && n0 + 64 <= p.N;
}
template <int EPI>
__device__ __forceinline__ void staged_colsum(const GemmParams& p, int lane, int m0, int n0, float (&cs)[8]) {
    if constexpr (epi_aux16(EPI)) {
        if (p.colsum_out) {
            const int rr = lane >> 3, cc = (lane & 7) * 8;
#pragma unroll
            for (int j = 0; j < 8; j++) {
                float t = cs[j];
                t += __shfl_xor(t, 8, 64);
                t += __shfl_xor(t, 16, 64);
                t += __shfl_xor(t, 32, 64);
                cs[j] = t;
            }
            if (rr == 0 && m0 < p.M) {
#pragma unroll
                for (int j = 0; j < 8; j++)
                    if (n0 + cc + j < p.N) p.colsum_out[(long long)(m0 >> 7) * p.N + n0 + cc + j] = cs[j];
            }
        }
    }
}

template <int EPI>
__device__ __forceinline__ void staged_bias_prefetch(const GemmParams& p, int lane, int n0, float (&bv)[8]) {
#pragma unroll
    for (int j = 0; j < 8; j++) bv[j] = 0.f;
    if constexpr (epi_bias(EPI)) {
        const int n = n0 + (lane & 7) * 8;
        if (p.bias && n + 8 <= p.N) {
            const float4 b0 = *reinterpret_cast<const float4*>(p.bias + n);
            const float4 b1 = *reinterpret_cast<const float4*>(p.bias + n + 4);
            bv[0] = b0.x; bv[1] = b0.y; bv[2] = b0.z; bv[3] = b0.w;
            bv[4] = b1.x; bv[5] = b1.y; bv[6] = b1.z; bv[7] = b1.w;
        }
    }
}
template <int EPI>
__device__ __forceinline__ void staged_epilogue(const GemmParams& p, f32x4_t (&acc)[8][4],
                                                char* stage, int lane, int m0, int n0,
                                                const float* bpre = nullptr) {
    float* st = reinterpret_cast<float*>(stage);
    const int i = lane & 15, g = lane >> 4;
    float cs[8] = {0.f, 0.f, 0.f, 0.f, 0.f, 0.f, 0.f, 0.f};
    const bool interior = staged_interior<EPI>(p, m0, n0);
    auto stage_pass = [&](int pass) {
#pragma unroll
        for (int a = 0; a < 4; a++)
#pragma unroll
            for (int b = 0; b < 4; b++)
                *reinterpret_cast<f32x4_t*>(st + (a * 16 + i) * STG_LD + b * 16 + 4 * g) = acc[pass * 4 + a][b];
    };
    if (interior && EpiAux<EPI>::N > 0) {
        const int rr = lane >> 3, n = n0 + (lane & 7) * 8;
        EpiAux<EPI> a0, a1;
        a0.load(p, rr, m0, n);
        a1.load(p, rr, m0 + 64, n);
        stage_pass(0);
// ... 245 lines not shown
```

### vit.rs_amd/csrc/ops.hip

```cpp
#include "ops_internal.h"
#include "ln_common.h"

namespace vit {

__global__ void residual_fwd_k(float* __restrict__ out, const float* __restrict__ a,
                               const float* __restrict__ b, long long n) {
    for (long long i = blockIdx.x * (long long)blockDim.x + threadIdx.x; i < n;
         i += (long long)gridDim.x * blockDim.x)
        out[i] = a[i] + b[i];
}
__global__ void residual_bwd_k(float* __restrict__ d1, float* __restrict__ d2,
                               const float* __restrict__ dout, long long n) {
    for (long long i = blockIdx.x * (long long)blockDim.x + threadIdx.x; i < n;
         i += (long long)gridDim.x * blockDim.x) {
        const float g = dout[i];
        d1[i] += g;
        d2[i] += g;
    }
}
__global__ void gelu_fwd_k(float* __restrict__ out, const float* __restrict__ inp, long long n) {
    for (long long i = blockIdx.x * (long long)blockDim.x + threadIdx.x; i < n;
         i += (long long)gridDim.x * blockDim.x)
        out[i] = gelu_f(inp[i]);
}
// ... 295 lines not shown
                pri[j] = reinterpret_cast<const float4*>(io.dinp + r * C)[lane + 64 * j];
            }
        }
        pmu = mean[r];
        prs = rstd[r];
    };
    long long row = blockIdx.x * 4LL + wave;
    if (row < rows) fetch(row);
    for (; row < rows; row += nwaves) {
        float4 dy[NV], xr[NV], ri[NV], nr[NV];
#pragma unroll
        for (int j = 0; j < NV; j++) {
            dy[j] = pdy[j];
            xr[j] = px[j];
            ri[j] = pri[j];
            if constexpr (ST) {
                const uint32_t q = plo[j];
                ri[j] = make_float4(lo8_decode(ri[j].x, q), lo8_decode(ri[j].y, q >> 8), lo8_decode(ri[j].z, q >> 16),
                                    lo8_decode(ri[j].w, q >> 24));
            }
        }
        const float mu = pmu, rs = prs;
        fetch(row + nwaves < rows ? row + nwaves : row);
        __builtin_amdgcn_sched_barrier(0);
        float4 dvv[NV];
        ln_bwd_row<NV>(dy, xr, w4, mu, rs, C, nr, dvv);
#pragma unroll
        for (int j = 0; j < NV; j++) {
            const int k = lane + 64 * j;
            {
                float4 b = pb[k], w = pw[k];
                b.x += dy[j].x; b.y += dy[j].y; b.z += dy[j].z; b.w += dy[j].w;
                w.x += nr[j].x * dy[j].x; w.y += nr[j].y * dy[j].y;
                w.z += nr[j].z * dy[j].z; w.w += nr[j].w * dy[j].w;
                pb[k] = b;
                pw[k] = w;
            }
            const float4 dv = dvv[j];
            const float4 t = make_float4(ri[j].x + dv.x, ri[j].y + dv.y, ri[j].z + dv.z, ri[j].w + dv.w);
            if constexpr (ST) {
                float4 u = ps[k];
                u.x += t.x; u.y += t.y; u.z += t.z; u.w += t.w;
                ps[k] = u;
                const uint2 h = make_uint2(pack_bf16x2(t.x, t.y), pack_bf16x2(t.z, t.w));
                reinterpret_cast<uint2*>(io.hi_out + row * C)[k] = h;
                reinterpret_cast<uint32_t*>(io.lo_out + row * C)[k] =
                    lo8_encode(t.x, __uint_as_float(h.x << 16)) |
                    (lo8_encode(t.y, __uint_as_float(h.x & 0xffff0000u)) << 8) |
                    (lo8_encode(t.z, __uint_as_float(h.y << 16)) << 16) |
                    (lo8_encode(t.w, __uint_as_float(h.y & 0xffff0000u)) << 24);
            } else {
                reinterpret_cast<float4*>(io.dinp + row * C)[k] = t;
            }
        }
    }
    lnb_flush(io, sm, C);
}

struct SoftCE {
    float* losses;
    const int *ta, *tb;
    float lam, oml, eps;
};
template <bool SOFT>
__global__ __launch_bounds__(256) void softmax_k(float* __restrict__ probs,
                                                 const float* __restrict__ logits, int V, SoftCE sc) {
    __shared__ float red[4];
    __shared__ float red2[4];
    const long long row = blockIdx.x;
    const float* l = logits + row * V;
    float* pr = probs + row * V;
    const int lane = threadIdx.x & 63, w = threadIdx.x >> 6;
    float m = -10000.0f;
    for (int i = threadIdx.x; i < V; i += 256) m = fmaxf(m, l[i]);
    m = warp_max(m);
    if (lane == 0) red[w] = m;
    __syncthreads();
    m = fmaxf(fmaxf(red[0], red[1]), fmaxf(red[2], red[3]));
    __syncthreads();
    float s = 0.f, sd = 0.f;
    for (int i = threadIdx.x; i < V; i += 256) {
        const float d = l[i] - m;
        const float e = expf(d);
        pr[i] = e;
        s += e;
        if constexpr (SOFT) sd += d;
    }
    s = warp_sum(s);
    if constexpr (SOFT) sd = warp_sum(sd);
    if (lane == 0) {
        red[w] = s;
        if constexpr (SOFT) red2[w] = sd;
    }
    __syncthreads();
    s = red[0] + red[1] + red[2] + red[3];
    const float inv = 1.0f / s;
    for (int i = threadIdx.x; i < V; i += 256) pr[i] = pr[i] * inv;
    if constexpr (SOFT) {
        if (threadIdx.x == 0) {
            sd = red2[0] + red2[1] + red2[2] + red2[3];
            const int a = sc.ta[row], b = sc.tb ? sc.tb[row] : a;
            float loss = __builtin_nanf("");
            if (a >= 0 && a < V && b >= 0 && b < V) {
                const float hard = sc.lam * (l[a] - m) + sc.oml * (l[b] - m);
                loss = logf(s) - ((1.0f - sc.eps) * hard + (sc.eps / (float)V) * sd);
            }
// ... 257 lines not shown
    const long long i = blockIdx.x * (long long)blockDim.x + threadIdx.x;
    if (i >= n) return;
    float s = 0.f;
    for (int y = 0; y < nch; y++) s += part[y * n + i];
    dwpe[i] += s;
    tsum[i] = s;
}
__global__ void patch_small_grads_fin_k(float* __restrict__ dcls, float* __restrict__ dpb,
                                        const float* __restrict__ tsum, int T, int C) {
    const int c = blockIdx.x * blockDim.x + threadIdx.x;
    if (c >= C) return;
    float ps[8] = {0.f, 0.f, 0.f, 0.f, 0.f, 0.f, 0.f, 0.f};
    int t = 1;
    for (; t + 8 <= T; t += 8) {
#pragma unroll
        for (int j = 0; j < 8; j++) ps[j] += tsum[(long long)(t + j) * C + c];
    }
    for (int j = 0; t < T; t++, j++) ps[j] += tsum[(long long)t * C + c];
    const float s = ((ps[0] + ps[1]) + (ps[2] + ps[3])) + ((ps[4] + ps[5]) + (ps[6] + ps[7]));
    dcls[c] += tsum[c];
    dpb[c] += s;
}

template <typename TO>
static void ln_forward_any(TO* out, float* mean, float* rstd, const float* inp, const float* w,
                           const float* b, long long rows, int C, hipStream_t s, long long rstride = 1) {
    if (rows <= 0) return;
    const int g = cdiv(rows, 4);
    const bool vec = C % 256 == 0 && C <= 2048 && (((uintptr_t)inp | (uintptr_t)out | (uintptr_t)w | (uintptr_t)b) & 15) == 0;
    switch (vec ? C / 256 : 0) {
        case 1: ln_fwd_vec_k<1, TO><<<g, 256, 0, s>>>(out, mean, rstd, inp, w, b, rows, C, rstride); break;
        case 2: ln_fwd_vec_k<2, TO><<<g, 256, 0, s>>>(out, mean, rstd, inp, w, b, rows, C, rstride); break;
        case 3: ln_fwd_vec_k<3, TO><<<g, 256, 0, s>>>(out, mean, rstd, inp, w, b, rows, C, rstride); break;
        case 4: ln_fwd_vec_k<4, TO><<<g, 256, 0, s>>>(out, mean, rstd, inp, w, b, rows, C, rstride); break;
        case 5: ln_fwd_vec_k<5, TO><<<g, 256, 0, s>>>(out, mean, rstd, inp, w, b, rows, C, rstride); break;
        case 6: ln_fwd_vec_k<6, TO><<<g, 256, 0, s>>>(out, mean, rstd, inp, w, b, rows, C, rstride); break;
        case 8: ln_fwd_vec_k<8, TO><<<g, 256, 0, s>>>(out, mean, rstd, inp, w, b, rows, C, rstride); break;
        default: ln_fwd_k<TO><<<g, 256, 0, s>>>(out, mean, rstd, inp, w, b, rows, C, rstride); break;
    }
    after_launch("layernorm_forward");
}
void ln_forward_f32(float* out, float* mean, float* rstd, const float* inp, const float* w,
                    const float* b, long long rows, int C, hipStream_t s) {
    ln_forward_any<float>(out, mean, rstd, inp, w, b, rows, C, s);
}
void ln_forward_bf16(bf16_t* out, float* mean, float* rstd, const float* inp, const float* w,
                     const float* b, long long rows, int C, hipStream_t s, long long row_stride) {
    ln_forward_any<bf16_t>(out, mean, rstd, inp, w, b, rows, C, s, row_stride);
}
int ln_bwd_blocks(long long rows);
template <typename TD, bool ST>
static void ln_backward_any(LnbIo io, const TD* dout, const float* inp, const float* w,
                            const float* mean, const float* rstd, long long rows, int C, hipStream_t s,
                            float* ws = nullptr) {
    if (rows <= 0) return;
    const bool reduce = io.part == nullptr;
    const int nsum = io.dsum ? 3 * C : 2 * C;
    if (reduce) {
        io.part = ws ? ws : (float*)workspace((size_t)ln_bwd_blocks(rows) * nsum * sizeof(float));
        if (!io.part) return;
    }
    const bool vec = C % 256 == 0 && C <= 2048 &&
                     (((uintptr_t)io.dinp | (uintptr_t)dout | (uintptr_t)inp | (uintptr_t)w |
                       (uintptr_t)io.hi_in | (uintptr_t)io.hi_out | (uintptr_t)io.lo_in | (uintptr_t)io.lo_out) & 15) == 0;
    const int grid = ln_bwd_blocks(rows);
    const size_t lds = 12 * (size_t)C * sizeof(float);
    if (lds > 160 * 1024) { set_error("layernorm_backward: C=%d exceeds the LDS column partials", C); return; }
    if (!vec) {
        if (lds > 64 * 1024) VIT_HIP(hipFuncSetAttribute((const void*)ln_bwd_k<TD, ST>,
                                                         hipFuncAttributeMaxDynamicSharedMemorySize, (int)lds));
        ln_bwd_k<TD, ST><<<grid, 256, lds, s>>>(io, dout, inp, w, mean, rstd, rows, C);
    } else {
#define VIT_LNB(NV)                                                                                        \
    if (lds > 64 * 1024) VIT_HIP(hipFuncSetAttribute((const void*)ln_bwd_vec_k<NV, TD, ST>,                 \
                                                     hipFuncAttributeMaxDynamicSharedMemorySize, (int)lds)); \
    ln_bwd_vec_k<NV, TD, ST><<<grid, 256, lds, s>>>(io, dout, inp, w, mean, rstd, rows, C)
        switch (C / 256) {
            case 1: VIT_LNB(1); break;
            case 2: VIT_LNB(2); break;
            case 3: VIT_LNB(3); break;
            case 4: VIT_LNB(4); break;
            case 5: VIT_LNB(5); break;
            case 6: VIT_LNB(6); break;
            case 7: VIT_LNB(7); break;
            default: VIT_LNB(8); break;
        }
#undef VIT_LNB
    }
    after_launch("layernorm_backward");
    if (reduce) {
        const RowsJob jobs[3] = {{io.dweight, io.part, grid, nsum, C}, {io.dbias, io.part + C, grid, nsum, C},
                                 {io.dsum, io.part + 2 * C, grid, nsum, C}};
        rows_reduce_add(jobs, io.dsum ? 3 : 2, s);
    }
}
int ln_bwd_blocks(long long rows) {
    const long long g = (rows + 15) / 16;
    return (int)(g < 1 ? 1 : (g > 768 ? 768 : g));
}
void ln_backward_f32(float* dinp, float* dw, float* db, const float* dout, const float* inp,
                     const float* w, const float* mean, const float* rstd, long long rows, int C,
                     hipStream_t s, float* ws) {
    LnbIo io{};
    io.dinp = dinp; io.dweight = dw; io.dbias = db;
    ln_backward_any<float, false>(io, dout, inp, w, mean, rstd, rows, C, s, ws);
}
void ln_backward_bf16_stream(bf16_t* dres_out, uint8_t* lo_out, const bf16_t* dres_in, const uint8_t* lo_in,
                             float* dw, float* db, float* dres_colsum, const bf16_t* dout, const float* inp,
                             const float* w, const float* mean, const float* rstd, long long rows, int C,
                             hipStream_t s, float* part) {
    if (!dres_out || !lo_out || !dres_in || !lo_in) { set_error("layernorm_backward: the bf16 stream needs its 4 planes"); return; }
    if (((uintptr_t)lo_in | (uintptr_t)lo_out) & 3) { set_error("layernorm_backward: lo8 planes need 4-B alignment"); return; }
    LnbIo io{};
    io.hi_out = dres_out; io.lo_out = lo_out; io.hi_in = dres_in; io.lo_in = lo_in;
    io.dweight = dw; io.dbias = db; io.dsum = dres_colsum; io.part = part;
    ln_backward_any<bf16_t, true>(io, dout, inp, w, mean, rstd, rows, C, s);
}
__global__ __launch_bounds__(256) void transpose_bf16_k(bf16_t* __restrict__ out,
                                                        const bf16_t* __restrict__ in, int R, int Cc,
                                                        long long stride) {
    __shared__ uint16_t tile[64][64 + 2];
    const long long mo = (long long)blockIdx.z * stride;
    const int r0 = blockIdx.y * 64, c0 = blockIdx.x * 64;
    const int t = threadIdx.x, tr = t >> 2, tc = (t & 3) * 16;
#pragma unroll
    for (int h = 0; h < 2; h++) {
        const int r = r0 + tr, c = c0 + tc + h * 8;
        const uint4 ld = *reinterpret_cast<const uint4*>(in + mo + (long long)min(r, R - 1) * Cc + min(c, Cc - 8));
        const uint4 v = (r < R && c < Cc) ? ld : make_uint4(0, 0, 0, 0);
        const uint16_t* e = reinterpret_cast<const uint16_t*>(&v);
#pragma unroll
        for (int j = 0; j < 8; j++) tile[tr][tc + h * 8 + j] = e[j];
    }
    __syncthreads();
#pragma unroll
    for (int h = 0; h < 2; h++) {
        const int oc = c0 + tr, orr = r0 + tc + h * 8;
        if (oc >= Cc || orr >= R) continue;
        uint16_t e[8];
#pragma unroll
        for (int j = 0; j < 8; j++) e[j] = tile[tc + h * 8 + j][tr];
        *reinterpret_cast<uint4*>(out + mo + (long long)oc * R + orr) = *reinterpret_cast<const uint4*>(e);
    }
}
void transpose_bf16(bf16_t* out, const bf16_t* in, int R, int Cc, int count, long long stride,
                    hipStream_t s) {
    if (R <= 0 || Cc <= 0 || count <= 0) return;
    if (R % 8 || Cc % 8) { set_error("transpose_bf16: dims must be multiples of 8 (%d x %d)", R, Cc); return; }
    dim3 grid(cdiv(Cc, 64), cdiv(R, 64), count);
    transpose_bf16_k<<<grid, 256, 0, s>>>(out, in, R, Cc, stride);
    after_launch("transpose_bf16");
}
void convert_f2bf(bf16_t* out, const float* inp, long long n, hipStream_t s) {
    if (n <= 0) return;
    f2bf_k<<<grid_for(n, 256), 256, 0, s>>>(out, inp, n);
    after_launch("convert_f32_to_bf16");
}
void sgd(float* p, const float* g, long long n, float lr, hipStream_t s) {
    if (n <= 0) return;
    sgd_k<<<grid_for(n, 256), 256, 0, s>>>(p, g, n, lr);
    after_launch("sgd_step");
}
void sgd_clip(float* p, const float* g, long long n, float lr, const ClipRec* rec, hipStream_t s) {
    if (n <= 0) return;
    sgd_clip_k<<<grid_for(n, 256), 256, 0, s>>>(p, g, n, lr, rec);
    after_launch("sgd_step_clipped");
}
int group_grid(int ntiles) { return ntiles < 2048 ? ntiles : 2048; }
void sgd_groups(float* p, const float* g, const GroupTab& gt, int tile_begin, int ntiles, float lr,
// ... 401 lines not shown
```

### vit.rs_amd/csrc/ops_internal.h

```cpp
#pragma once
#include "common.h"
#include "gemm.h"
#include "../../include/vit_ops.h"

namespace vit {
int grid_for(long long n, int threads);
void ln_forward_f32(float* out, float* mean, float* rstd, const float* inp, const float* w,
                    const float* b, long long rows, int C, hipStream_t s);
void ln_forward_bf16(bf16_t* out, float* mean, float* rstd, const float* inp, const float* w,
                     const float* b, long long rows, int C, hipStream_t s, long long row_stride = 1);
void ln_backward_f32(float* dinp, float* dw, float* db, const float* dout, const float* inp,
                     const float* w, const float* mean, const float* rstd, long long rows, int C,
                     hipStream_t s, float* ws = nullptr);
void ln_backward_bf16_stream(bf16_t* dres_out, uint8_t* lo_out, const bf16_t* dres_in, const uint8_t* lo_in,
                             float* dw, float* db, float* dres_colsum, const bf16_t* dout, const float* inp,
                             const float* w, const float* mean, const float* rstd, long long rows, int C,
                             hipStream_t s, float* part = nullptr);
int ln_bwd_blocks(long long rows);
void convert_f2bf(bf16_t* out, const float* inp, long long n, hipStream_t s);
void sgd(float* p, const float* g, long long n, float lr, hipStream_t s);
void sgd_clip(float* p, const float* g, long long n, float lr, const ClipRec* rec, hipStream_t s);
int group_grid(int ntiles);
void sgd_groups(float* p, const float* g, const GroupTab& gt, int tile_begin, int ntiles, float lr,
                const ClipRec* rec, hipStream_t s);
int sumsq_blocks(long long n);
void sumsq_partials(double* slots, const float* x, long long n, hipStream_t s);
void sumsq_finish(double* out, const double* slots, int nslots, hipStream_t s);
void clip_finish(ClipRec* rec, const double* slots, int nslots, float max_norm, hipStream_t s);
void softmax_rows(float* probs, const float* logits, long long rows, int V, hipStream_t s);
void ce_forward(float* losses, const float* probs, const int* targets, long long rows, int V,
                hipStream_t s);
void ce_backward(float* dlogits, const float* dlosses, const float* probs, const int* targets,
                 long long rows, int V, hipStream_t s);
void softmax_ce_soft(float* probs, float* losses, const float* logits, const int* ta, const int* tb,
                     float lam, float eps, long long rows, int V, hipStream_t s);
void ce_soft_backward(float* dlogits, const float* dlosses, const float* probs, const int* ta,
                      const int* tb, float lam, float eps, long long rows, int V, hipStream_t s);
void mixup_batch(float* px, int* labels_b, const int* labels, int B, int IMG, float lam, hipStream_t s);
void cutmix_batch(float* px, int* labels_b, const int* labels, int B, int IMG, int x0, int y0, int x1,
                  int y1, hipStream_t s);
void im2col_f32(float* out, const float* px, int B, int IMG, int P, hipStream_t s);
void im2col_bf16(bf16_t* out, const float* px, int B, int IMG, int P, hipStream_t s);
void im2col_pad_bf16(bf16_t* out, const float* px, int B, int IMG, int P, int KPP, hipStream_t s);
void patch_assemble(float* enc, const float* emb, const float* cls, const float* wpe, int B,
                    int NP, int C, hipStream_t s);
void transpose_bf16(bf16_t* out, const bf16_t* in, int R, int Cc, int count, long long stride,
                    hipStream_t s);
void patch_gather_f32(float* out, const float* denc, int B, int NP, int C, hipStream_t s);
void patch_gather_bf16(bf16_t* out, const float* denc, int B, int NP, int C, hipStream_t s);
void patch_gather_f32(float* out, const bf16_t* denc, const uint8_t* lo, int B, int NP, int C, hipStream_t s);
void patch_gather_bf16(bf16_t* out, const bf16_t* denc, int B, int NP, int C, hipStream_t s);
void patch_small_grads(float* dcls, float* dwpe, float* dpb, const float* denc, int B, int T,
                       int C, hipStream_t s, float* ws = nullptr);
constexpr int PSG_CHUNKS = 16;
void patch_small_grads(float* dcls, float* dwpe, float* dpb, const bf16_t* denc, const uint8_t* lo, int B, int T,
                       int C, hipStream_t s, float* ws = nullptr, float* part = nullptr);
void attn_forward_f32(float* out, float* preatt, float* att, const float* inp, int B, int T, int C,
                      int NH, hipStream_t s);
void attn_backward_f32(float* dinp, float* dpreatt, float* datt, const float* dout,
                       const float* inp, const float* att, int B, int T, int C, int NH,
                       hipStream_t s);
bool attn_fused_supported(int T, int C, int NH);
bool attn_generic_supported(int T, int C, int NH);
void attn_forward_fused(bf16_t* out, float* lse, const bf16_t* qkv, int B, int T, int C, int NH,
                        hipStream_t s);
size_t attn_backward_ws_floats(int B, int T, int C, int NH);
void attn_backward_fused(bf16_t* dqkv, const bf16_t* dout, const bf16_t* qkv, const bf16_t* out,
                         const float* lse, int B, int T, int C, int NH, hipStream_t s,
                         float* dqkv_colsum = nullptr, float* ws = nullptr, bool colsum_store = false);
}
```

### vit.rs_amd/csrc/trainer.hip

```cpp
#include <rccl/rccl.h>

#include <algorithm>
#include <cmath>
#include <cstdlib>
#include <cstring>
#include <string>
#include <vector>

#include "augment.h"
#include "ops_internal.h"
#include "../../include/vit_trainer.h"
#include "../../include/vit_checkpoint.h"
#include "../../include/vit_data.h"
#include "../../include/vit_jpeg.h"

namespace vit {
bool jpeg_loader_decode_to(vit_jpeg_loader_t* l, uint8_t* out, int img, hipStream_t st, const int** labels,
                           int expect_n);
namespace {

enum TIdx {
    P_PATCH_W, P_PATCH_B, P_CLS, P_WPE, P_LN1W, P_LN1B, P_QKVW, P_QKVB, P_ATTPROJW, P_ATTPROJB,
    P_LN2W, P_LN2B, P_FCW, P_FCB, P_FCPROJW, P_FCPROJB, P_LNFW, P_LNFB, P_HEADW, P_HEADB
};
// ... 610 lines not shown
        }
        emb_tmp = alloc<float>((long long)B * NP * C);
        la.resize(L);
        if (!lowp()) {
            gemm_ws_bytes = (size_t)32 << 20;
            gemm_ws = alloc<float>((long long)(gemm_ws_bytes / sizeof(float)));
        }
        if (lowp()) {
            if (!(attn_fused_supported(T, C, NH) || attn_generic_supported(T, C, NH)) || C % 8) {
                set_error("trainer: bf16 / fp8 path needs head size 32, 64, 80, 96 or 128 and C %% 8 == 0 (T=%d C=%d NH=%d)", T, C, NH);
                return false;
            }
            const char* pp = getenv("VIT_PATCH_PAD");
            patch_f32 = KP % 8 != 0 && pp && pp[0] == '0';
            patch_pad = KP % 8 != 0 && !patch_f32;
            KPP = patch_pad ? (KP + 63) / 64 * 64 : KP;
            pbf = alloc<bf16_t>(arena_elems);
            pbfT = alloc<bf16_t>(arena_elems);
            if (patch_f32) {
                patches_f = alloc<float>((long long)B * NP * KP);
                dpatch_f = alloc<float>((long long)B * NP * C);
            } else {
                patches_bf = alloc<bf16_t>((long long)B * NP * KPP);
            }
            if (patch_pad) {
                wpatch_pad = alloc<bf16_t>((long long)C * KPP);
                dwpatch_pad = alloc<float>((long long)C * KPP);
                if (wpatch_pad) VIT_HIP(hipMemset(wpatch_pad, 0, (size_t)C * KPP * 2));
            }
            for (int l = 0; l < L; l++) {
                LayerActs& a = la[l];
                a.ln1 = alloc<bf16_t>(BT * C);
                a.ln1_mean = alloc<float>(BT);
                a.ln1_rstd = alloc<float>(BT);
                a.qkv = alloc<bf16_t>(BT * 3 * C);
                a.atty = alloc<bf16_t>(BT * C);
                a.lse = alloc<float>(BT * NH);
                a.res2 = alloc<float>(BT * C);
                a.ln2 = alloc<bf16_t>(BT * C);
                a.ln2_mean = alloc<float>(BT);
                a.ln2_rstd = alloc<float>(BT);
                a.fchd = alloc<bf16_t>(BT * 4 * C);
                a.fchg = alloc<bf16_t>(BT * 4 * C);
                a.res3 = alloc<float>(BT * C);
            }
            if (prec == VIT_BF16 && !has_error()) {
                LayerActs& a = la[L - 1];
                VIT_HIP(hipMemsetAsync(a.ln2_mean, 0, (size_t)BT * 4, s));
                VIT_HIP(hipMemsetAsync(a.ln2_rstd, 0, (size_t)BT * 4, s));
                VIT_HIP(hipMemsetAsync(a.res2, 0, (size_t)BT * C * 4, s));
                VIT_HIP(hipMemsetAsync(a.ln2, 0, (size_t)BT * C * 2, s));
                VIT_HIP(hipMemsetAsync(a.fchd, 0, (size_t)BT * 4 * C * 2, s));
                VIT_HIP(hipMemsetAsync(a.fchg, 0, (size_t)BT * 4 * C * 2, s));
            }
            dln_bf = alloc<bf16_t>(BT * C);
            dres_bf = alloc<bf16_t>(BT * C);
            dres_bf2 = alloc<bf16_t>(BT * C);
            dres_lo = alloc<uint8_t>(BT * C);
            dres_lo2 = alloc<uint8_t>(BT * C);
            dfch = alloc<bf16_t>(BT * 4 * C);
            datty = alloc<bf16_t>(BT * C);
            dqkv = alloc<bf16_t>(BT * 3 * C);
            if (!patch_f32) dpatch_bf = alloc<bf16_t>((long long)B * NP * C);
            gemm_ws_bytes = (size_t)32 * 4 * C * (size_t)std::max(C, KP) * sizeof(float);
            gemm_ws = alloc<float>((long long)(gemm_ws_bytes / sizeof(float)));
            attn_part = alloc<float>((long long)attn_backward_ws_floats(B, T, C, NH) + MAXMB * 3LL * C);
            {
                const long long lnr = (long long)MAXMB * ln_bwd_blocks(BT), fcr = cdiv(BT, 96) + MAXMB;
                sg_ln2 = 0;
                sg_ln1 = sg_ln2 + lnr * 3 * C;
                sg_fcb = sg_ln1 + lnr * 3 * C;
                sg_qkv = sg_fcb + fcr * 4 * C;
                const long long n = sg_qkv + (long long)MAXMB * 3 * C;
                sg_part[0] = alloc<float>(n);
                sg_part[1] = alloc<float>(n);
            }
            if (fp8()) {
                const long long ns[NWK] = {3LL * C, C, 4LL * C, C}, ks[NWK] = {C, C, C, 4LL * C};
                for (int k = 0; k < NWK; k++) {
                    wq_n[k] = ns[k];
                    wq_k[k] = ks[k];
                    wq[k].q = alloc<uint8_t>(L * ns[k] * ks[k]);
                    wq[k].s = alloc<uint8_t>((long long)L * mx_scale_bytes(ns[k], (int)ks[k]));
                    wtq[k].q = alloc<uint8_t>(L * ns[k] * ks[k]);
                    wtq[k].s = alloc<uint8_t>((long long)L * mx_scale_bytes(ks[k], (int)ns[k]));
                }
                for (int k = 0; k < MAXMB; k++) {
                    const long long rows = (long long)(B / (k + 1)) * T;
                    if (rows <= 0) continue;
                    act_q[k] = alloc<uint8_t>(rows * 4 * C);
                    act_s[k] = alloc<uint8_t>((long long)mx_scale_bytes(rows, 4 * C));
                    act_q2[k] = alloc<uint8_t>(rows * 4 * C);
                    act_s2[k] = alloc<uint8_t>((long long)mx_scale_bytes(rows, 4 * C));
                    VIT_HIP(hipMemset(act_s2[k], 0, mx_scale_bytes(rows, 4 * C)));
                }
                const char* fe = getenv("VIT_FP8_FUSE");
                fuse_mx = !(fe && fe[0] == '0');
                const char* wc = getenv("VIT_FP8_WT_COLS");
                wt_cols = !(wc && wc[0] == '0') && C % 64 == 0;
                const char* fw = getenv("VIT_FP8_WGRAD");
                fp8_wgrad = !(fw && fw[0] == '0') && C % 64 == 0;
                if (fp8_wgrad) {
                    const long long kp = mx_cols_kp(BT);
                    wg_a.q = alloc<uint8_t>(4LL * C * kp);
                    wg_a.s = alloc<uint8_t>((long long)mx_scale_bytes(4LL * C, (int)kp));
                    wg_b.q = alloc<uint8_t>(4LL * C * kp);
// ... 143 lines not shown
            const long long N = wq_n[k], K = wq_k[k];
            quantize_mx_batched_f32(wq[k].q, wq[k].s, P(wkinds[k], l0), N, (int)K, L, as, N * K,
                                    (long long)mx_scale_bytes(N, (int)K), s);
            if (wt_cols)
                quantize_mx_cols_batched_bf16(wtq[k].q, wtq[k].s, W(wkinds[k], l0), N, (int)K, K, L, as, N * K,
                                              (long long)mx_scale_bytes(K, (int)N), s);
            else
                quantize_mx_batched_bf16(wtq[k].q, wtq[k].s, WT(wkinds[k], l0), K, (int)N, L, as, N * K,
                                         (long long)mx_scale_bytes(K, (int)N), s);
        }
        tend();
    }
    QMat wq_of(int ti, int l) const {
        const int k = wkind_of(ti), j = wslot(k, l);
        return {wq[k].q + (long long)j * wq_n[k] * wq_k[k], wq[k].s + (long long)j * mx_scale_bytes(wq_n[k], (int)wq_k[k])};
    }
    QMat wtq_of(int ti, int l) const {
        const int k = wkind_of(ti), j = wslot(k, l);
        return {wtq[k].q + (long long)j * wq_n[k] * wq_k[k], wtq[k].s + (long long)j * mx_scale_bytes(wq_k[k], (int)wq_n[k])};
    }
    enum { PRE_NONE = 0, PRE_EPI = 1, PRE_LN = 2 };
    void gemm_w(int cls, GemmArgs a, int ti, int l, bool transposed, int mb, hipStream_t st, int pre = PRE_NONE,
                bool mx_out = false, const QMat* colq = nullptr, int rec_ev = -1) {
        if (!fp8()) { gemm(cls, a, true, st); return; }
        if (mx_out) { a.mx_q = act_q2[mb]; a.mx_s = act_s2[mb]; }
        const uint8_t* aq = act_q[mb];
        const uint8_t* as = act_s[mb];
        if (pre == PRE_EPI) {
            aq = act_q2[mb];
            as = act_s2[mb];
        } else if (pre == PRE_NONE) {
            tbeg(TC_QUANT, 0, st);
            if (colq) {
                const long long r0 = (long long)mb * (B / nmb) * T;
                const long long ntok = mb_ntok(mb, a.M);
                quantize_mx_rowcol_bf16(act_q[mb], act_s[mb], colq->q, colq->s, (const bf16_t*)a.A, a.M, a.K, a.lda,
                                        kp_tok, r0, ntok, st);
            } else {
                quantize_mx_bf16(act_q[mb], act_s[mb], (const bf16_t*)a.A, a.M, a.K, a.lda, a.K, st);
            }
            tend();
            if (rec_ev >= 0 && two_streams) VIT_HIP(hipEventRecord(mev[mb][rec_ev], st));
        }
        const QMat w = transposed ? wtq_of(ti, l) : wq_of(ti, l);
        a.A = aq; a.lda = a.K; a.a_scale = as;
        a.B = w.q; a.ldb = a.K; a.b_scale = w.s; a.b_kcontig = true;
        tbeg(cls, 2.0 * a.M * (double)a.N * a.K, st);
        gemm_fp8(a, st);
        tend();
    }

    bool last_cls = true;
    bool lc_active = false;
    bool lc_dirty = true;
    bool lc_pending = false;
    bool last_cls_on() const { return last_cls && prec == VIT_BF16; }
    void last_cls_clear() {
        if (!lc_dirty) return;
        hipStream_t cs = s;
        if (two_streams && s2) {
            VIT_HIP(hipEventRecord(bev[EV_LC_IN], s));
            VIT_HIP(hipStreamWaitEvent(s2, bev[EV_LC_IN], 0));
            cs = s2;
        }
        VIT_HIP(hipMemsetAsync(dln_bf, 0, (size_t)BT * C * 2, cs));
        VIT_HIP(hipMemsetAsync(datty, 0, (size_t)BT * C * 2, cs));
        if (cs != s) {
            VIT_HIP(hipEventRecord(bev[EV_LC], cs));
            lc_pending = true;
        }
        lc_dirty = false;
    }
    void last_cls_wait() {
        if (!lc_pending) return;
        VIT_HIP(hipStreamWaitEvent(s, bev[EV_LC], 0));
        lc_pending = false;
    }

    bool head_sk = true;
    bool patch_tail = true;
    int head_split(int M, int N, int K) const {
        if (!head_sk) return 0;
        int sp = std::min(16, std::max(1, K / 64));
        while (sp > 1 && (size_t)sp * M * N * sizeof(float) > gemm_ws_bytes) sp--;
        return sp;
    }
    void head_forward() {
        tbeg(TC_HEAD, 2.0 * B * C * NC);
        const float* last = la[L - 1].res3;
        VIT_HIP(hipMemcpy2DAsync(cls_x, C * 4, last, (size_t)T * C * 4, C * 4, B, hipMemcpyDeviceToDevice, s));
        ln_forward_f32(lnf, lnf_mean, lnf_rstd, cls_x, P(P_LNFW), P(P_LNFB), B, C, s);
        GemmArgs a;
        a.A = lnf; a.lda = C; a.B = P(P_HEADW); a.ldb = C; a.C = logits; a.ldc = NC;
        a.bias = P(P_HEADB); a.M = B; a.N = NC; a.K = C; a.epi = EPI_F32_STORE;
        if (lowp()) {
            bcast_rows_k<<<cdiv((long long)B * NC, 256), 256, 0, s>>>(logits, P(P_HEADB), B, NC);
            a.bias = nullptr;
            a.epi = EPI_F32_ATOMIC;
            a.splitk = head_split(a.M, a.N, a.K);
        }
        a.ws = gemm_ws; a.ws_bytes = gemm_ws_bytes;
        gemm_f32(a, s);
        if (has_targets && soft_targets()) {
            softmax_ce_soft(probs, losses, logits, labels, two_labels() ? labels_b : nullptr, mix_lam,
                            smooth_eps, B, NC, s);
        } else {
            softmax_rows(probs, logits, B, NC, s);
            if (has_targets) ce_forward(losses, probs, labels, B, NC, s);
        }
        tend();
    }
    void head_backward(float* dres, bf16_t* dres_bf = nullptr, uint8_t* dres_lo = nullptr) {
        tbeg(TC_HEAD, 4.0 * B * C * NC);
        fill_k<<<cdiv(B, 256), 256, 0, s>>>(dlosses, 1.0f / (float)b_global, B);
        VIT_HIP(hipMemsetAsync(dlogits, 0, (size_t)B * NC * 4, s));
        if (soft_targets())
            ce_soft_backward(dlogits, dlosses, probs, labels, two_labels() ? labels_b : nullptr, mix_lam,
                             smooth_eps, B, NC, s);
        else
            ce_backward(dlogits, dlosses, probs, labels, B, NC, s);
        VIT_HIP(hipMemsetAsync(dlnf, 0, (size_t)B * C * 4, s));
        GemmArgs a;
        a.A = dlogits; a.lda = NC; a.a_kcontig = true;
        a.B = P(P_HEADW); a.ldb = C; a.b_kcontig = false;
        a.C = dlnf; a.ldc = C; a.M = B; a.N = C; a.K = NC; a.epi = lowp() ? EPI_F32_ATOMIC : EPI_F32_ACC;
        if (lowp()) a.splitk = head_split(a.M, a.N, a.K);
        a.ws = gemm_ws; a.ws_bytes = gemm_ws_bytes;
        gemm_f32(a, s);
        GemmArgs w;
        w.A = dlogits; w.lda = NC; w.a_kcontig = false;
        w.B = lnf; w.ldb = C; w.b_kcontig = false;
        w.C = G(P_HEADW); w.ldc = C; w.M = NC; w.N = C; w.K = B; w.epi = lowp() ? EPI_F32_ATOMIC : EPI_F32_ACC;
        if (lowp()) w.splitk = head_split(w.M, w.N, w.K);
        w.ws = gemm_ws; w.ws_bytes = gemm_ws_bytes;
        gemm_f32(w, s);
        colsum_f32(G(P_HEADB), dlogits, B, NC, NC, s, red_ws);
        VIT_HIP(hipMemsetAsync(dcls_x, 0, (size_t)B * C * 4, s));
        ln_backward_f32(dcls_x, G(P_LNFW), G(P_LNFB), dlnf, cls_x, P(P_LNFW), lnf_mean, lnf_rstd, B, C, s, red_ws);
        if (dres_bf) {
            VIT_HIP(hipMemsetAsync(dres_bf, 0, (size_t)BT * C * 2, s));
            VIT_HIP(hipMemsetAsync(dres_lo, 0, (size_t)BT * C, s));
            rows_to_bf16_k<<<cdiv((long long)B * C, 256), 256, 0, s>>>(dres_bf, dres_lo, (long long)T * C, dcls_x, B, C);
        } else {
            VIT_HIP(hipMemsetAsync(dres, 0, (size_t)BT * C * 4, s));
            VIT_HIP(hipMemcpy2DAsync(dres, (size_t)T * C * 4, dcls_x, C * 4, C * 4, B, hipMemcpyDeviceToDevice, s));
        }
        tend();
    }

    void forward_bf16() {
        const int Bm = B / nmb;
        const long long R = (long long)Bm * T;
        lc_active = last_cls_on();
        if (lc_active) last_cls_clear();
        mb_fork();
        for (int mb = 0; mb < nmb; mb++) {
            hipStream_t st = ms[mb];
            const long long img0 = (long long)mb * Bm;
            tbeg(TC_PATCH, 2.0 * Bm * NP * (double)KP * C, st);
            GemmArgs a;
            a.C = emb_tmp + img0 * NP * C; a.ldc = C; a.bias = P(P_PATCH_B);
            a.M = Bm * NP; a.N = C; a.K = KP; a.epi = EPI_F32_STORE;
            if (patch_f32) {
                im2col_f32(patches_f + img0 * NP * KP, pixels + img0 * 3 * cfg.img * cfg.img, Bm, cfg.img,
                           cfg.patch, st);
                a.A = patches_f + img0 * NP * KP; a.lda = KP; a.B = P(P_PATCH_W); a.ldb = KP;
                gemm_f32(a, st);
            } else if (patch_pad) {
                im2col_pad_bf16(patches_bf + img0 * NP * KPP, pixels + img0 * 3 * cfg.img * cfg.img, Bm, cfg.img,
                                cfg.patch, KPP, st);
                a.A = patches_bf + img0 * NP * KPP; a.lda = KPP; a.B = wpatch_pad; a.ldb = KPP; a.K = KPP;
                gemm_bf16(a, st);
            } else {
                im2col_bf16(patches_bf + img0 * NP * KP, pixels + img0 * 3 * cfg.img * cfg.img, Bm, cfg.img,
                            cfg.patch, st);
                a.A = patches_bf + img0 * NP * KP; a.lda = KP; a.B = W(P_PATCH_W); a.ldb = KP;
                gemm_bf16(a, st);
            }
            patch_assemble(encoded + img0 * T * C, emb_tmp + img0 * NP * C, P(P_CLS), P(P_WPE), Bm, NP, C, st);
            tend();
        }
        for (int l = 0; l < L; l++) {
            LayerActs& a = la[l];
            const float* xl = l == 0 ? encoded : la[l - 1].res3;
            const bool lc = lc_active && l == L - 1;
            const int Mr = lc ? Bm : (int)R;
            const long long rs = lc ? T : 1;
            const bool lcg = lc && R >= 256;
            for (int mb = 0; mb < nmb; mb++) {
                hipStream_t st = ms[mb];
                const long long r0 = (long long)mb * R;
                const float* x = xl + r0 * C;
                const bool rc = rowcol_on(), lm = lnmx_on();
                QMat c_ln1 = rc ? actc_of(0, l) : QMat{}, c_atty = rc ? actc_of(1, l) : QMat{},
                     c_ln2 = rc ? actc_of(2, l) : QMat{};
                tbeg(TC_LN_FWD, 0, st);
                if (lm)
                    ln_forward_mx(act_q[mb], act_s[mb], c_ln1.q, c_ln1.s, a.ln1_mean + r0, a.ln1_rstd + r0, x,
                                  P(P_LN1W, l), P(P_LN1B, l), R, C, kp_tok, r0, mb_ntok(mb, R), st,
                                  ln_left ? lnb_scr[mb] : nullptr);
                else
                    ln_forward_bf16(a.ln1 + r0 * C, a.ln1_mean + r0, a.ln1_rstd + r0, x, P(P_LN1W, l), P(P_LN1B, l), R, C, st);
                tend();
                GemmArgs q;
                q.A = a.ln1 + r0 * C; q.lda = C; q.B = W(P_QKVW, l); q.ldb = C; q.C = a.qkv + r0 * 3 * C;
                q.ldc = 3 * C; q.bias = P(P_QKVB, l); q.M = (int)R; q.N = 3 * C; q.K = C; q.epi = EPI_BF16_STORE;
                gemm_w(TC_QKV_FWD, q, P_QKVW, l, false, mb, st, lm ? PRE_LN : PRE_NONE, false,
                       rc && !lm ? &c_ln1 : nullptr);
                tbeg(TC_ATTN_FWD, 4.0 * Bm * (double)T * T * C, st);
                attn_forward_fused(a.atty + r0 * C, a.lse + (long long)mb * Bm * NH * T, a.qkv + r0 * 3 * C, Bm, T, C, NH, st);
                tend();
                GemmArgs pr;
                pr.A = a.atty + r0 * C; pr.lda = rs * C; pr.B = W(P_ATTPROJW, l); pr.ldb = C; pr.C = a.res2 + r0 * C;
                pr.ldc = rs * C; pr.bias = P(P_ATTPROJB, l); pr.aux = x; pr.ldaux = rs * C;
                pr.M = Mr; pr.N = C; pr.K = C; pr.epi = EPI_F32_RESID; pr.rows_gathered = lcg;
                gemm_w(TC_PROJ_FWD, pr, P_ATTPROJW, l, false, mb, st, PRE_NONE, false, rc ? &c_atty : nullptr);
                tbeg(TC_LN_FWD, 0, st);
                if (lm)
                    ln_forward_mx(act_q[mb], act_s[mb], c_ln2.q, c_ln2.s, a.ln2_mean + r0, a.ln2_rstd + r0,
                                  a.res2 + r0 * C, P(P_LN2W, l), P(P_LN2B, l), R, C, kp_tok, r0, mb_ntok(mb, R), st,
                                  ln_left ? lnb_scr[mb] : nullptr);
                else
                    ln_forward_bf16(a.ln2 + r0 * C, a.ln2_mean + r0, a.ln2_rstd + r0, a.res2 + r0 * C, P(P_LN2W, l),
                                    P(P_LN2B, l), Mr, C, st, rs);
                tend();
                GemmArgs f;
                f.A = a.ln2 + r0 * C; f.lda = rs * C; f.B = W(P_FCW, l); f.ldb = C; f.C = a.fchd + r0 * 4 * C;
                f.C2 = a.fchg + r0 * 4 * C; f.ldc = rs * 4 * C; f.bias = P(P_FCB, l); f.M = Mr; f.N = 4 * C;
                f.K = C; f.epi = EPI_BF16_GELU_D; f.rows_gathered = lcg;
                if (epicol_on()) {
                    const QMat g = fchgc_of(l);
                    f.C2 = nullptr;
                    f.mxc_q = g.q; f.mxc_s = g.s; f.mxc_ld = kp_tok; f.mxc_off = r0;
                }
                gemm_w(TC_FC_FWD, f, P_FCW, l, false, mb, st, lm ? PRE_LN : PRE_NONE, fuse_mx,
                       rc && !lm ? &c_ln2 : nullptr);
                GemmArgs fp;
                fp.A = a.fchg + r0 * 4 * C; fp.lda = rs * 4 * C; fp.B = W(P_FCPROJW, l); fp.ldb = 4 * C;
                fp.C = a.res3 + r0 * C; fp.ldc = rs * C; fp.bias = P(P_FCPROJB, l); fp.aux = a.res2 + r0 * C;
                fp.ldaux = rs * C; fp.M = Mr; fp.N = C; fp.K = 4 * C; fp.epi = EPI_F32_RESID; fp.rows_gathered = lcg;
                gemm_w(TC_FCPROJ_FWD, fp, P_FCPROJW, l, false, mb, st, fuse_mx ? PRE_EPI : PRE_NONE);
            }
        }
        mb_join();
        head_forward();
    }

    void wgrad(int cls, const bf16_t* dout, int OC, const bf16_t* inp, int Cin, float* dW, int ready,
               int done, const QMat* dout_c = nullptr, const QMat* inp_c = nullptr) {
        GemmArgs w;
        w.A = dout; w.lda = OC; w.a_kcontig = false;
        w.B = inp; w.ldb = Cin; w.b_kcontig = false;
        w.C = dW; w.ldc = Cin; w.M = OC; w.N = Cin; w.K = (int)BT; w.epi = EPI_F32_ATOMIC;
        w.ws = gemm_ws; w.ws_bytes = gemm_ws_bytes;
        w.fill_pct = two_streams ? 0 : 80;
        hipStream_t st = two_streams ? s2 : s;
        if (two_streams) {
            for (int mb = 0; mb < nmb; mb++) {
                if (!dout_c) VIT_HIP(hipEventRecord(mev[mb][ready], ms[mb]));
                VIT_HIP(hipStreamWaitEvent(s2, mev[mb][ready], 0));
            }
        }
        if (fp8() && fp8_wgrad) {
// ... 35 lines not shown
        const float* p2 = sg_rows(l, sg_ln2);
        const float* p1 = sg_rows(l, sg_ln1);
        RowsJob jobs[8] = {
            {G(P_LN2W, l), p2, nb, 3 * C, C},
            {G(P_LN2B, l), p2 + C, nb, 3 * C, C},
            {G(P_ATTPROJB, l), p2 + 2 * C, nb, 3 * C, C},
            {G(P_LN1W, l), p1, nb, w1, C},
            {G(P_LN1B, l), p1 + C, nb, w1, C},
            {G(P_FCB, l), sg_rows(l, sg_fcb), nmb * fcb_rows, 4 * C, 4 * C},
            {G(P_QKVB, l), sg_rows(l, sg_qkv), nmb, 3 * C, 3 * C},
            {l > 0 ? G(P_FCPROJB, l - 1) : nullptr, p1 + 2 * C, nb, w1, C},
        };
        tbeg(TC_COLSUM, 0, st);
        rows_reduce_add(jobs, l > 0 ? 8 : 7, st);
        tend();
    }

    void backward_bf16() {
        pre_side_wait();
        last_cls_wait();
        lc_dirty = true;
        bf16_t* rbA = dres_bf;
        bf16_t* rbB = dres_bf2;
        uint8_t* loA = dres_lo;
        uint8_t* loB = dres_lo2;
        head_backward(nullptr, rbA, loA);
        chunk_done(0);
        colsum_f32(G(P_FCPROJB, L - 1), dcls_x, B, C, C, s, red_ws);
        mb_fork();
        const int Bm = B / nmb;
        const long long R = (long long)Bm * T;
        for (int l = L - 1; l >= 0; l--) {
            LayerActs& a = la[l];
            const float* xl = l == 0 ? encoded : la[l - 1].res3;
            const bool lc = lc_active && l == L - 1;
            const int Mr = lc ? Bm : (int)R;
            const long long rs = lc ? T : 1;
            const bool lcg = lc && R >= 256;
            const bool rc = rowcol_on();
            QMat c_ln1 = rc ? actc_of(0, l) : QMat{}, c_atty = rc ? actc_of(1, l) : QMat{}, c_ln2 = rc ? actc_of(2, l) : QMat{};
            const bool lbm = lnbmx_on(), resa_pre = lbm && l < L - 1;
            const bool ec = epicol_on();
            QMat c_fchg = ec ? fchgc_of(l) : QMat{};
            if (!rc) wgrad(TC_FCPROJ_WGRAD, rbA, C, a.fchg, 4 * C, G(P_FCPROJW, l), EV_RESA, EV_W1);
            for (int mb = 0; mb < nmb; mb++) {
                const long long r0 = mb * R;
                after_wgrad(EV_W2, ms[mb]);
                GemmArgs d1;
                d1.A = rbA + r0 * C; d1.lda = C; dgrad_b(d1, P_FCPROJW, l, C, 4 * C);
                d1.C = dfch + r0 * 4 * C; d1.ldc = 4 * C; d1.aux = a.fchd + r0 * 4 * C; d1.ldaux = 4 * C;
                d1.M = (int)R; d1.N = 4 * C; d1.K = C; d1.epi = EPI_BF16_MUL;
                fcb_rows = gemm_colsum_rows(d1, fp8());
                d1.colsum_part = sg_rows(l, sg_fcb) + (long long)mb * fcb_rows * 4 * C;
                if (ec) {
                    d1.C = nullptr;
                    d1.mxc_q = dfchc.q; d1.mxc_s = dfchc.s; d1.mxc_ld = kp_tok; d1.mxc_off = r0;
                }
                gemm_w(TC_FCPROJ_DGRAD, d1, P_FCPROJW, l, true, mb, ms[mb], resa_pre ? PRE_LN : PRE_NONE, fuse_mx,
                       rc && !resa_pre ? &dcol[0] : nullptr, resa_pre ? -1 : EV_RESA);
                if (ec && two_streams) VIT_HIP(hipEventRecord(mev[mb][EV_DFCH], ms[mb]));
            }
            if (rc) wgrad(TC_FCPROJ_WGRAD, rbA, C, a.fchg, 4 * C, G(P_FCPROJW, l), EV_RESA, EV_W1, &dcol[0],
                          ec ? &c_fchg : nullptr);
            wgrad(TC_FC_WGRAD, dfch, 4 * C, a.ln2, C, G(P_FCW, l), EV_DFCH, EV_W2, ec ? &dfchc : nullptr,
                  rc ? &c_ln2 : nullptr);
            for (int mb = 0; mb < nmb; mb++) {
                const long long r0 = mb * R;
                GemmArgs d2;
                d2.A = dfch + r0 * 4 * C; d2.lda = rs * 4 * C; dgrad_b(d2, P_FCW, l, 4 * C, C);
                d2.C = dln_bf + r0 * C; d2.ldc = rs * C; d2.M = Mr; d2.N = C; d2.K = 4 * C; d2.epi = EPI_BF16_STORE;
                d2.rows_gathered = lcg;
                gemm_w(TC_FC_DGRAD, d2, P_FCW, l, true, mb, ms[mb], fuse_mx ? PRE_EPI : PRE_NONE);
                after_wgrad(EV_W3, ms[mb]);
                tbeg(TC_LN_BWD, 0, ms[mb]);
                if (lbm) {
                    ln_backward_bf16_stream_mx(rbB + r0 * C, loB + r0 * C, rbA + r0 * C, loA + r0 * C, G(P_LN2W, l),
                                               G(P_LN2B, l), G(P_ATTPROJB, l), dln_bf + r0 * C, a.res2 + r0 * C,
                                               P(P_LN2W, l), a.ln2_mean + r0, a.ln2_rstd + r0, R, C, ms[mb],
                                               sg_rows(l, sg_ln2) + (long long)mb * ln_bwd_blocks(R) * 3 * C,
                                               act_q[mb], act_s[mb], dcol[1].q, dcol[1].s, kp_tok, r0, mb_ntok(mb, R),
                                               lnb_scr[mb]);
                    if (two_streams) VIT_HIP(hipEventRecord(mev[mb][EV_RESB], ms[mb]));
                } else {
                    ln_backward_bf16_stream(rbB + r0 * C, loB + r0 * C, rbA + r0 * C, loA + r0 * C, G(P_LN2W, l),
                                            G(P_LN2B, l), G(P_ATTPROJB, l), dln_bf + r0 * C, a.res2 + r0 * C,
                                            P(P_LN2W, l), a.ln2_mean + r0, a.ln2_rstd + r0, R, C, ms[mb],
                                            sg_rows(l, sg_ln2) + (long long)mb * ln_bwd_blocks(R) * 3 * C);
                }
                tend();
            }
            if (!rc) wgrad(TC_PROJ_WGRAD, rbB, C, a.atty, C, G(P_ATTPROJW, l), EV_RESB, EV_W3);
            for (int mb = 0; mb < nmb; mb++) {
                const long long r0 = mb * R;
                GemmArgs d3;
                d3.A = rbB + r0 * C; d3.lda = rs * C; dgrad_b(d3, P_ATTPROJW, l, C, C);
                d3.C = datty + r0 * C; d3.ldc = rs * C; d3.M = Mr; d3.N = C; d3.K = C; d3.epi = EPI_BF16_STORE;
                d3.rows_gathered = lcg;
                gemm_w(TC_PROJ_DGRAD, d3, P_ATTPROJW, l, true, mb, ms[mb], lbm ? PRE_LN : PRE_NONE, false,
                       rc && !lbm ? &dcol[1] : nullptr, lbm ? -1 : EV_RESB);
                after_wgrad(EV_W4, ms[mb]);
                tbeg(TC_ATTN_BWD, 8.0 * Bm * (double)T * T * C, ms[mb]);
                attn_backward_fused(dqkv + r0 * 3 * C, datty + r0 * C, a.qkv + r0 * 3 * C, a.atty + r0 * C,
                                    a.lse + (long long)mb * Bm * NH * T, Bm, T, C, NH, ms[mb],
                                    sg_rows(l, sg_qkv) + (long long)mb * 3 * C,
                                    attn_part + (long long)attn_backward_ws_floats(mb * Bm, T, C, NH), true);
                tend();
            }
            if (rc) wgrad(TC_PROJ_WGRAD, rbB, C, a.atty, C, G(P_ATTPROJW, l), EV_RESB, EV_W3, &dcol[1], &c_atty);
            if (!rc) wgrad(TC_QKV_WGRAD, dqkv, 3 * C, a.ln1, C, G(P_QKVW, l), EV_DQKV, EV_W4);
            for (int mb = 0; mb < nmb; mb++) {
                const long long r0 = mb * R;
                GemmArgs d4;
                d4.A = dqkv + r0 * 3 * C; d4.lda = 3 * C; dgrad_b(d4, P_QKVW, l, 3 * C, C);
                d4.C = dln_bf + r0 * C; d4.ldc = C; d4.M = (int)R; d4.N = C; d4.K = 3 * C; d4.epi = EPI_BF16_STORE;
                gemm_w(TC_QKV_DGRAD, d4, P_QKVW, l, true, mb, ms[mb], PRE_NONE, false, rc ? &dcol[2] : nullptr, EV_DQKV);
                after_wgrad(EV_W1, ms[mb]);
                tbeg(TC_LN_BWD, 0, ms[mb]);
                if (lbm && l > 0) {
                    ln_backward_bf16_stream_mx(rbA + r0 * C, loA + r0 * C, rbB + r0 * C, loB + r0 * C, G(P_LN1W, l),
                                               G(P_LN1B, l), G(P_FCPROJB, l - 1), dln_bf + r0 * C, xl + r0 * C,
                                               P(P_LN1W, l), a.ln1_mean + r0, a.ln1_rstd + r0, R, C, ms[mb],
                                               sg_rows(l, sg_ln1) + (long long)mb * ln_bwd_blocks(R) * 3 * C,
                                               act_q[mb], act_s[mb], dcol[0].q, dcol[0].s, kp_tok, r0, mb_ntok(mb, R),
                                               lnb_scr[mb]);
                    if (two_streams) VIT_HIP(hipEventRecord(mev[mb][EV_RESA], ms[mb]));
                } else {
                    ln_backward_bf16_stream(rbA + r0 * C, loA + r0 * C, rbB + r0 * C, loB + r0 * C, G(P_LN1W, l),
                                            G(P_LN1B, l), l > 0 ? G(P_FCPROJB, l - 1) : nullptr, dln_bf + r0 * C,
                                            xl + r0 * C, P(P_LN1W, l), a.ln1_mean + r0, a.ln1_rstd + r0, R, C, ms[mb],
                                            sg_rows(l, sg_ln1) + (long long)mb * ln_bwd_blocks(R) * (l > 0 ? 3 : 2) * C);
                }
                tend();
            }
            if (rc) wgrad(TC_QKV_WGRAD, dqkv, 3 * C, a.ln1, C, G(P_QKVW, l), EV_DQKV, EV_W4, &dcol[2], &c_ln1);
            sg_finalize(l, R);
            chunk_done(L - l);
        }
        mb_join();
        if (two_streams) {
            VIT_HIP(hipEventRecord(bev[EV_JOIN], s2));
            VIT_HIP(hipStreamWaitEvent(s, bev[EV_JOIN], 0));
        }
        tbeg(TC_PATCH_BWD, 2.0 * B * NP * (double)KP * C);
        const bool psg_side = two_streams && lowp() && patch_tail;
        if (psg_side) {
            VIT_HIP(hipEventRecord(bev[EV_SG], s));
            VIT_HIP(hipStreamWaitEvent(s2, bev[EV_SG], 0));
            patch_small_grads(G(P_CLS), G(P_WPE), G(P_PATCH_B), rbA, loA, B, T, C, s2, pos_sums, psg_part);
            VIT_HIP(hipEventRecord(bev[EV_JOIN], s2));
        }
        if (patch_f32) {
            patch_gather_f32(dpatch_f, rbA, loA, B, NP, C, s);
            GemmArgs w;
            w.A = dpatch_f; w.lda = C; w.a_kcontig = false; w.B = patches_f; w.ldb = KP; w.b_kcontig = false;
            w.C = G(P_PATCH_W); w.ldc = KP; w.M = C; w.N = KP; w.K = B * NP; w.epi = EPI_F32_ATOMIC;
            gemm_f32(w, s);
        } else {
            patch_gather_bf16(dpatch_bf, rbA, B, NP, C, s);
// ... 893 lines not shown
        set_error("vit_trainer_get_dp_snapshot: option dp_probe is off");
        return 1;
    }
    VIT_HIP(hipStreamSynchronize(t.s_comm));
    t.device_to_canon(t.dp_snap, host);
    return vit::has_error();
}
int vit_trainer_dp_ranks(vit_trainer_t* h) {
    if (!h->t.comm) return 0;
    int n = 0;
    ncclResult_t r = ncclCommCount(h->t.comm, &n);
    if (r != ncclSuccess) {
        set_error("ncclCommCount: %s", ncclGetErrorString(r));
        return -1;
    }
    return n;
}
int vit_trainer_set_concurrency(vit_trainer_t* h, int on) {
    auto& t = h->t;
    VIT_HIP(hipStreamSynchronize(t.s2));
    for (int k = 0; k < vit::Trainer::MAXMB; k++) if (t.ms[k]) VIT_HIP(hipStreamSynchronize(t.ms[k]));
    t.two_streams = on != 0;
    t.nmb = t.pick_nmb(t.mb_want);
    return vit::has_error();
}
int vit_trainer_set_option(vit_trainer_t* h, const char* name, int value) {
    auto& t = h->t;
    VIT_HIP(hipDeviceSynchronize());
    const std::string n = name ? name : "";
    if (n == "microbatch") {
        t.mb_want = value;
        t.nmb = t.pick_nmb(value);
    } else if (n == "dgrad_transposed") {
        t.dgrad_wt = value != 0;
    } else if (n == "fp8_ln_mx") {
        t.ln_mx = value != 0;
    } else if (n == "fp8_ln_leftover") {
        t.ln_left = value != 0;
    } else if (n == "early_sgd") {
        t.early_sgd = value < 0 ? -1 : value != 0;
    } else if (n == "pre_side") {
        t.pre_side_wait();
        t.pre_side = value != 0;
    } else if (n == "patch_tail") {
        t.patch_tail = value != 0;
    } else if (n == "head_splitk") {
        t.head_sk = value != 0;
    } else if (n == "fp8_lnb_mx") {
        t.lnb_mx = value != 0;
    } else if (n == "clip_overlap") {
        t.clip_overlap = value < 0 ? -1 : value != 0;
    } else if (n == "last_cls") {
        t.last_cls = value != 0;
    } else if (n == "dp_probe") {
        if (value && !t.dp_snap) {
            t.dp_snap = t.alloc<float>(t.arena_elems);
            if (t.dp_snap) VIT_HIP(hipMemset(t.dp_snap, 0, t.arena_elems * 4));
        }
        t.dp_probe_on = value != 0 && t.dp_snap != nullptr;
    } else {
        set_error("vit_trainer_set_option: unknown option '%s'", n.c_str());
        return 1;
    }
    return vit::has_error();
}
int vit_trainer_set_timing(vit_trainer_t* h, int on) {
    h->t.timing = on != 0;
    return 0;
}
int vit_trainer_timing(vit_trainer_t* h, const char** names, double* ms, long long* calls,
                       double* flops, int max) {
    auto& t = h->t;
    t.collect();
    int n = 0;
    for (int c = 0; c < vit::TC_COUNT && n < max; c++) {
        if (!t.t_calls[c]) continue;
        names[n] = vit::kTimerNames[c];
        ms[n] = t.t_ms[c];
        calls[n] = t.t_calls[c];
        flops[n] = t.t_flops[c];
        n++;
    }
    return n;
}
void vit_trainer_timing_reset(vit_trainer_t* h) {
    auto& t = h->t;
    t.collect();
    for (int c = 0; c < vit::TC_COUNT; c++) {
        t.t_ms[c] = 0;
        t.t_calls[c] = 0;
        t.t_flops[c] = 0;
    }
}
}
```

Measured before the change: 7316 images/s.

## Compute only CLS-row attention and sparse backward in the last ViT block

Extends the existing last-block CLS-only optimization into attention and parts of the backward pass. Only the CLS output is used by the head, so the final block's attention forward computes just the first query tiles. The attention backward gets a single-slice persistent variant that zeros the other dQ rows. LayerNorm backward and the FC1 dgrad colsum restrict work to CLS rows, so non-CLS backward work in the final layer is skipped. This adds memsets of several gradient buffers and new kernel template paths, and it risks wrong results if the zeroed buffers are ever consumed elsewhere.

```diff
diff --git a/include/vit_ops.h b/include/vit_ops.h
--- a/include/vit_ops.h
+++ b/include/vit_ops.h
@@ -98,6 +98,12 @@
 void attention_backward_fused_bf16_ex(uint16_t* dinp, const uint16_t* dout, const uint16_t* inp,
                                       const uint16_t* out, const float* lse, int B, int T, int C, int NH,
                                       float* dqkv_bias);
+int vit_attention_last_cls_supported(int T, int C, int NH);
+void attention_forward_fused_bf16_cls(uint16_t* out, float* lse, const uint16_t* inp,
+                                      int B, int T, int C, int NH);
+void attention_backward_fused_bf16_cls(uint16_t* dinp, const uint16_t* dout, const uint16_t* inp,
+                                       const uint16_t* out, const float* lse, int B, int T, int C, int NH,
+                                       float* dqkv_bias);
 void layernorm_forward_bf16(uint16_t* out, float* mean, float* rstd, const float* inp,
                             const float* weight, const float* bias, int B, int T, int C);
 void layernorm_backward_bf16(float* dinp, float* dweight, float* dbias, const uint16_t* dout,
diff --git a/vit.rs_amd/__init__.py b/vit.rs_amd/__init__.py
--- a/vit.rs_amd/__init__.py
+++ b/vit.rs_amd/__init__.py
@@ -86,6 +86,9 @@
     "vit_attention_kernel_kind": (I, [I, I, I]),
     "attention_backward_fused_bf16": (None, [P, P, P, P, P, I, I, I, I]),
     "attention_backward_fused_bf16_ex": (None, [P, P, P, P, P, I, I, I, I, P]),
+    "vit_attention_last_cls_supported": (I, [I, I, I]),
+    "attention_forward_fused_bf16_cls": (None, [P, P, P, I, I, I, I]),
+    "attention_backward_fused_bf16_cls": (None, [P, P, P, P, P, I, I, I, I, P]),
     "layernorm_forward_bf16": (None, [P, P, P, P, P, P, I, I, I]),
     "layernorm_backward_bf16": (None, [P, P, P, P, P, P, P, P, I, I, I]),
     "gelu_forward_bf16": (None, [P, P, I]),
diff --git a/vit.rs_amd/csrc/attention.hip b/vit.rs_amd/csrc/attention.hip
--- a/vit.rs_amd/csrc/attention.hip
+++ b/vit.rs_amd/csrc/attention.hip
@@ -516,8 +516,21 @@
     return (size_t)B * NH * per_bh + (size_t)cdiv((long long)B * T, 256) * 3 * C;
 }
 
+bool attn_last_cls_supported(int T, int C, int NH) {
+    if (!attn_fused_supported(T, C, NH) || fa::attn_bwd_variant() != 0) return false;
+    switch (C / NH) {
+        case 32: return fa_cls_ok_h32(T);
+        case 64: return fa_cls_ok_h64(T);
+        default: return false;
+    }
+}
+
 void attn_forward_fused(bf16_t* out, float* lse, const bf16_t* qkv, int B, int T, int C, int NH,
-                        hipStream_t s) {
+                        hipStream_t s, bool cls) {
+    if (cls && !attn_fused_supported(T, C, NH)) {
+        set_error("attention_forward_fused: no last_cls form for T=%d C=%d NH=%d", T, C, NH);
+        return;
+    }
     if (!attn_fused_supported(T, C, NH)) {
         if (!attn_generic_supported(T, C, NH)) {
             set_error("attention_forward_fused: unsupported shape (T=%d C=%d NH=%d)", T, C, NH);
@@ -540,11 +553,11 @@
     }
     bool ok = false;
     switch (C / NH) {
-        case 32: ok = fa_forward_h32(out, lse, qkv, B, T, C, NH, s); break;
-        case 64: ok = fa_forward_h64(out, lse, qkv, B, T, C, NH, s); break;
-        case 80: ok = fa_forward_h80(out, lse, qkv, B, T, C, NH, s); break;
-        case 96: ok = fa_forward_h96(out, lse, qkv, B, T, C, NH, s); break;
-        case 128: ok = fa_forward_h128(out, lse, qkv, B, T, C, NH, s); break;
+        case 32: ok = fa_forward_h32(out, lse, qkv, B, T, C, NH, s, cls); break;
+        case 64: ok = fa_forward_h64(out, lse, qkv, B, T, C, NH, s, cls); break;
+        case 80: ok = fa_forward_h80(out, lse, qkv, B, T, C, NH, s, cls); break;
+        case 96: ok = fa_forward_h96(out, lse, qkv, B, T, C, NH, s, cls); break;
+        case 128: ok = fa_forward_h128(out, lse, qkv, B, T, C, NH, s, cls); break;
     }
     if (!ok) { set_error("fused attention: no kernel for T=%d head size %d", T, C / NH); return; }
     after_launch("attention_forward_fused");
@@ -552,7 +565,11 @@
 
 void attn_backward_fused(bf16_t* dqkv, const bf16_t* dout, const bf16_t* qkv, const bf16_t* out,
                          const float* lse, int B, int T, int C, int NH, hipStream_t s,
-                         float* dqkv_colsum, float* ws, bool colsum_store) {
+                         float* dqkv_colsum, float* ws, bool colsum_store, bool cls) {
+    if (cls && !attn_fused_supported(T, C, NH)) {
+        set_error("attention_backward_fused: no last_cls form for T=%d C=%d NH=%d", T, C, NH);
+        return;
+    }
     if (!attn_fused_supported(T, C, NH)) {
         if (!attn_generic_supported(T, C, NH)) {
             set_error("attention_backward_fused: unsupported shape (T=%d C=%d NH=%d)", T, C, NH);
@@ -591,11 +608,11 @@
     float* part = dqkv_colsum ? ws : nullptr;
     int rows = 0;
     switch (HS) {
-        case 32: rows = fa_backward_h32(dqkv, dout, qkv, out, lse, B, T, C, NH, part, s); break;
-        case 64: rows = fa_backward_h64(dqkv, dout, qkv, out, lse, B, T, C, NH, part, s); break;
-        case 80: rows = fa_backward_h80(dqkv, dout, qkv, out, lse, B, T, C, NH, part, s); break;
-        case 96: rows = fa_backward_h96(dqkv, dout, qkv, out, lse, B, T, C, NH, part, s); break;
-        case 128: rows = fa_backward_h128(dqkv, dout, qkv, out, lse, B, T, C, NH, part, s); break;
+        case 32: rows = fa_backward_h32(dqkv, dout, qkv, out, lse, B, T, C, NH, part, s, cls); break;
+        case 64: rows = fa_backward_h64(dqkv, dout, qkv, out, lse, B, T, C, NH, part, s, cls); break;
+        case 80: rows = fa_backward_h80(dqkv, dout, qkv, out, lse, B, T, C, NH, part, s, cls); break;
+        case 96: rows = fa_backward_h96(dqkv, dout, qkv, out, lse, B, T, C, NH, part, s, cls); break;
+        case 128: rows = fa_backward_h128(dqkv, dout, qkv, out, lse, B, T, C, NH, part, s, cls); break;
     }
     if (!rows) { set_error("fused attention backward: no kernel for T=%d head size %d", T, HS); return; }
     after_launch("attention_backward_fused");
@@ -639,4 +656,14 @@
                                       float* dqkv_bias) {
     attn_backward_fused(dinp, dout, inp, out, lse, B, T, C, NH, stream(), dqkv_bias);
 }
-}
+int vit_attention_last_cls_supported(int T, int C, int NH) { return attn_last_cls_supported(T, C, NH) ? 1 : 0; }
+void attention_forward_fused_bf16_cls(uint16_t* out, float* lse, const uint16_t* inp, int B, int T, int C,
+                                      int NH) {
+    attn_forward_fused(out, lse, inp, B, T, C, NH, stream(), true);
+}
+void attention_backward_fused_bf16_cls(uint16_t* dinp, const uint16_t* dout, const uint16_t* inp,
+                                       const uint16_t* out, const float* lse, int B, int T, int C, int NH,
+                                       float* dqkv_bias) {
+    attn_backward_fused(dinp, dout, inp, out, lse, B, T, C, NH, stream(), dqkv_bias, nullptr, false, true);
+}
+}
diff --git a/vit.rs_amd/csrc/attn_fused.h b/vit.rs_amd/csrc/attn_fused.h
--- a/vit.rs_amd/csrc/attn_fused.h
+++ b/vit.rs_amd/csrc/attn_fused.h
@@ -192,7 +192,7 @@
 #ifndef VIT_ATTN_FWD_BUF
 #define VIT_ATTN_FWD_BUF 1
 #endif
-template <int HS, int NKT, int NS = NKT>
+template <int HS, int NKT, int NS = NKT, int NQT = 0>
 __global__ __launch_bounds__(256, (fwd_occ<HS, NKT>())) void attn_fwd_k(bf16_t* __restrict__ out,
                                                                         float* __restrict__ lse,
                                                                         const bf16_t* __restrict__ qkv,
@@ -217,7 +217,7 @@
             else qf[s] = frag_glb<HS>(base, C3, qt * 16 + i, T, s, lane);
         }
     };
-    const int nqt = (T + 15) / 16;
+    const int nqt = NQT ? NQT : (T + 15) / 16;
     bf16x8_t qn[G::KS];
     load_q(w, qn);
     if constexpr (VIT_ATTN_FWD_BUF) {
@@ -1335,7 +1335,7 @@
            NKT % KK == 0 && (KK == 2 ? bwd1_fits<HS, NKT>() : KK == 4 ? (HS == 64 && Z::NW <= 4) : Z::NW <= 16);
 }
 
-template <int HS, int NKT, int KK>
+template <int HS, int NKT, int KK, bool CLS = false>
 __global__ __launch_bounds__(NKT / KK * 64, 1) void attn_bwdp_k(bf16_t* __restrict__ dqkv,
                                                                const bf16_t* __restrict__ dout,
                                                                const bf16_t* __restrict__ qkv,
@@ -1427,6 +1427,25 @@
             *reinterpret_cast<uint4*>(dst + cc * 8) = ps[j];
         }
     };
+    constexpr int PERA = (2 * TP * CH + NT - 1) / NT;
+    static_assert(!CLS || PERA * NT == 2 * TP * CH, "K / V pieces are whole threads");
+    [[maybe_unused]] uint4 pa[CLS ? PERA : 1];
+    [[maybe_unused]] auto fetch_kv_all = [&](const Src& sr) {
+        const auto rk = sr.kv;
+#pragma unroll
+        for (int j = 0; j < PERA; j++) {
+            const int idx = j * NT + tid, op = idx >= TP * CH, rem = idx - op * TP * CH, t = rem / CH, cc = rem - t * CH;
+            pa[j] = buf_ld16(rk, (uint32_t)t * (uint32_t)(C3 * 2) + (uint32_t)(op * C * 2) + 16 * cc);
+        }
+    };
+    [[maybe_unused]] auto put_kv_all = [&](int kbuf) {
+#pragma unroll
+        for (int j = 0; j < PERA; j++) {
+            const int idx = j * NT + tid, op = idx >= TP * CH, rem = idx - op * TP * CH, t = rem / CH, cc = rem - t * CH;
+            bf16_t* dst = op ? Vst + t * SK : Kimg + kbuf * TP * SV + t * SV;
+            *reinterpret_cast<uint4*>(dst + cc * 8) = pa[j];
+        }
+    };
     auto load_kv = [&](BwdRegs<HS, KK>& R, int kbuf) {
 #pragma unroll
         for (int kk = 0; kk < KK; kk++)
@@ -1462,49 +1481,69 @@
         bf16_t* dq = dqkv + (long long)(bh / NH) * T * C3 + (bh % NH) * HS;
         const float* lse_cur = lse_s + (n & 1) * TP;
         R.zero();
+        if constexpr (CLS) {
+            const int cur = it & 1;
+            if (slice_wave) fetch_slice(s_nxt, 0);
+            lse_n = buf_ldf(s_nxt.l, 4 * tid);
+            bwd_slice_a<HS, KK>(R, Qs + cur * 32 * SL, Ds + cur * 32 * SL, lse_cur, del_s + cur * 32, dSs + key0 * Z::SDS,
+                                c, lane);
+            fetch_kv_all(s_nxt);
+            for (int idx = tid; idx < (T - 32) * CH; idx += NT) {
+                const int t = 32 + idx / CH, cc = idx % CH;
+                *reinterpret_cast<uint4*>(dq + (long long)t * C3 + cc * 8) = make_uint4(0, 0, 0, 0);
+            }
+            if (slice_wave) put_slice(cur ^ 1);
+            if (tid < TP) lse_s[((n + 1) & 1) * TP + tid] = tid < T ? lse_n : INFINITY;
+            __syncthreads();
+            bwd_slice_b<HS, NSL, NW>(Kimg + kb * TP * SV, dSs, dq, C3, 0, T, scale, w, lane);
+            put_kv_all(kb ^ 1);
+            __syncthreads();
+            it++;
+        } else {
 #pragma unroll 1
-        for (int sl = 0; sl < NSL; sl++, it++) {
-            const int cur = it & 1, q0 = sl * 32;
-            ATTN_STAMP(0);
-            if constexpr (!(VIT_ATTN_DIAG & 1)) {
-                if (slice_wave) {
-                    if (sl + 1 < NSL) fetch_slice(s_cur, q0 + 32);
-                    else fetch_slice(s_nxt, 0);
+            for (int sl = 0; sl < NSL; sl++, it++) {
+                const int cur = it & 1, q0 = sl * 32;
+                ATTN_STAMP(0);
+                if constexpr (!(VIT_ATTN_DIAG & 1)) {
+                    if (slice_wave) {
+                        if (sl + 1 < NSL) fetch_slice(s_cur, q0 + 32);
+                        else fetch_slice(s_nxt, 0);
+                    }
+                    fetch_side(s_nxt, sl);
+                    if (sl == 0) lse_n = buf_ldf(s_nxt.l, 4 * tid);
                 }
-                fetch_side(s_nxt, sl);
-                if (sl == 0) lse_n = buf_ldf(s_nxt.l, 4 * tid);
+                if constexpr (VIT_ATTN_SKEW) {
+                    bf16_t* dS_a = dSs + (sl & 1) * TP * Z::SDS;
+                    bwd_slice_a<HS, KK>(R, Qs + cur * 32 * SL, Ds + cur * 32 * SL, lse_cur + q0, del_s + cur * 32,
+                                        dS_a + key0 * Z::SDS, c, lane);
+                    ATTN_STAMP(1);
+                    if (sl > 0)
+                        bwd_slice_b<HS, NSL, NW>(Kimg + kb * TP * SV, dSs + ((sl - 1) & 1) * TP * Z::SDS, dq, C3,
+                                                 q0 - 32, T, scale, w, lane);
+                    ATTN_STAMP(2);
+                    if (slice_wave) put_slice(cur ^ 1);
+                    if (sl == 0 && tid < TP) lse_s[((n + 1) & 1) * TP + tid] = tid < T ? lse_n : INFINITY;
+                    ATTN_STAMP(3);
+                    __syncthreads();
+                    ATTN_STAMP(4);
+                    put_side(kb ^ 1, sl);
+                    ATTN_STAMP(5);
+                } else {
+                    bwd_slice_a<HS, KK>(R, Qs + cur * 32 * SL, Ds + cur * 32 * SL, lse_cur + q0, del_s + cur * 32,
+                                        dSs + key0 * Z::SDS, c, lane);
+                    __syncthreads();
+                    put_slice(cur ^ 1);
+                    put_side(kb ^ 1, sl);
+                    if (sl == 0 && tid < TP) lse_s[((n + 1) & 1) * TP + tid] = tid < T ? lse_n : INFINITY;
+                    bwd_slice_b<HS, NSL, NW>(Kimg + kb * TP * SV, dSs, dq, C3, q0, T, scale, w, lane);
+                    __syncthreads();
+                }
             }
             if constexpr (VIT_ATTN_SKEW) {
-                bf16_t* dS_a = dSs + (sl & 1) * TP * Z::SDS;
-                bwd_slice_a<HS, KK>(R, Qs + cur * 32 * SL, Ds + cur * 32 * SL, lse_cur + q0, del_s + cur * 32,
-                                    dS_a + key0 * Z::SDS, c, lane);
-                ATTN_STAMP(1);
-                if (sl > 0)
-                    bwd_slice_b<HS, NSL, NW>(Kimg + kb * TP * SV, dSs + ((sl - 1) & 1) * TP * Z::SDS, dq, C3,
-                                             q0 - 32, T, scale, w, lane);
-                ATTN_STAMP(2);
-                if (slice_wave) put_slice(cur ^ 1);
-                if (sl == 0 && tid < TP) lse_s[((n + 1) & 1) * TP + tid] = tid < T ? lse_n : INFINITY;
-                ATTN_STAMP(3);
+                bwd_slice_b<HS, NSL, NW>(Kimg + kb * TP * SV, dSs + ((NSL - 1) & 1) * TP * Z::SDS, dq, C3,
+                                         (NSL - 1) * 32, T, scale, w, lane);
                 __syncthreads();
-                ATTN_STAMP(4);
-                put_side(kb ^ 1, sl);
-                ATTN_STAMP(5);
-            } else {
-                bwd_slice_a<HS, KK>(R, Qs + cur * 32 * SL, Ds + cur * 32 * SL, lse_cur + q0, del_s + cur * 32,
-                                    dSs + key0 * Z::SDS, c, lane);
-                __syncthreads();
-                put_slice(cur ^ 1);
-                put_side(kb ^ 1, sl);
-                if (sl == 0 && tid < TP) lse_s[((n + 1) & 1) * TP + tid] = tid < T ? lse_n : INFINITY;
-                bwd_slice_b<HS, NSL, NW>(Kimg + kb * TP * SV, dSs, dq, C3, q0, T, scale, w, lane);
-                __syncthreads();
-            }
-        }
-        if constexpr (VIT_ATTN_SKEW) {
-            bwd_slice_b<HS, NSL, NW>(Kimg + kb * TP * SV, dSs + ((NSL - 1) & 1) * TP * Z::SDS, dq, C3,
-                                     (NSL - 1) * 32, T, scale, w, lane);
-            __syncthreads();
+            }
         }
         ATTN_STAMP(6);
         bwd_item_end<HS, KK>(R, dq, C, key0, T, scale,
@@ -1527,9 +1566,21 @@
     return tp;
 }
 
+constexpr int CLS_QT = 2;
 template <int HS, int NKT>
-bool launch_fwd(bf16_t* out, float* lse, const bf16_t* qkv, int B, int T, int C, int NH, hipStream_t s) {
+constexpr bool cls_fits() { return NKT > 2 && bwdp_fits<HS, NKT, 2>(); }
+template <int HS, int NKT>
+bool launch_fwd(bf16_t* out, float* lse, const bf16_t* qkv, int B, int T, int C, int NH, hipStream_t s, bool cls) {
     if (T > NKT * 16 || T <= (NKT - 2) * 16) return false;
+    if (cls) {
+        if constexpr (cls_fits<HS, NKT>()) {
+            if ((NKT - 1) * 16 >= T) attn_fwd_k<HS, NKT, NKT - 1, CLS_QT><<<B * NH, 256, 0, s>>>(out, lse, qkv, T, C, NH);
+            else attn_fwd_k<HS, NKT, NKT, CLS_QT><<<B * NH, 256, 0, s>>>(out, lse, qkv, T, C, NH);
+            count_hit(VIT_HIT_ATTN_FWD_MFMA);
+            return true;
+        }
+        return false;
+    }
 #ifndef VIT_ATTN_FWD_TRIM
 #define VIT_ATTN_FWD_TRIM 1
 #endif
@@ -1544,8 +1595,17 @@
 int attn_cu_count();
 template <int HS, int NKT>
 int launch_bwd(bf16_t* dqkv, const bf16_t* dout, const bf16_t* qkv, const bf16_t* out, const float* lse, int B,
-               int T, int C, int NH, float* part, hipStream_t s) {
+               int T, int C, int NH, float* part, hipStream_t s, bool cls) {
     const int v = attn_bwd_variant(), BH = B * NH;
+    if (cls) {
+        if constexpr (cls_fits<HS, NKT>()) {
+            attn_bwdp_k<HS, NKT, 2, true><<<std::min(BH, attn_cu_count()), NKT / 2 * 64, 0, s>>>(dqkv, dout, qkv, out,
+                                                                                               lse, T, C, NH, BH, part, 0);
+            count_hit(VIT_HIT_ATTN_BWD_PERSISTENT);
+            return NKT / 2;
+        }
+        return 0;
+    }
     constexpr int NK4 = (NKT + 7) / 8 * 8;
     if constexpr (bwdp_fits<HS, NK4, 4>()) {
         if (v == 4) {
@@ -1588,22 +1648,31 @@
 }
 template <int HS, int NKT = 2>
 bool dispatch_fwd(int nkt, bf16_t* out, float* lse, const bf16_t* qkv, int B, int T, int C, int NH,
-                  hipStream_t s) {
+                  hipStream_t s, bool cls) {
     if constexpr (NKT * 16 > max_tp<HS>()) {
         return false;
     } else {
-        if (nkt == NKT) return launch_fwd<HS, NKT>(out, lse, qkv, B, T, C, NH, s);
-        return dispatch_fwd<HS, NKT + 2>(nkt, out, lse, qkv, B, T, C, NH, s);
+        if (nkt == NKT) return launch_fwd<HS, NKT>(out, lse, qkv, B, T, C, NH, s, cls);
+        return dispatch_fwd<HS, NKT + 2>(nkt, out, lse, qkv, B, T, C, NH, s, cls);
     }
 }
 template <int HS, int NKT = 2>
 int dispatch_bwd(int nkt, bf16_t* dqkv, const bf16_t* dout, const bf16_t* qkv, const bf16_t* out,
-                 const float* lse, int B, int T, int C, int NH, float* part, hipStream_t s) {
+                 const float* lse, int B, int T, int C, int NH, float* part, hipStream_t s, bool cls) {
     if constexpr (NKT * 16 > max_tp<HS>()) {
         return 0;
     } else {
-        if (nkt == NKT) return launch_bwd<HS, NKT>(dqkv, dout, qkv, out, lse, B, T, C, NH, part, s);
-        return dispatch_bwd<HS, NKT + 2>(nkt, dqkv, dout, qkv, out, lse, B, T, C, NH, part, s);
+        if (nkt == NKT) return launch_bwd<HS, NKT>(dqkv, dout, qkv, out, lse, B, T, C, NH, part, s, cls);
+        return dispatch_bwd<HS, NKT + 2>(nkt, dqkv, dout, qkv, out, lse, B, T, C, NH, part, s, cls);
+    }
+}
+template <int HS, int NKT = 2>
+bool dispatch_cls_ok(int nkt) {
+    if constexpr (NKT * 16 > max_tp<HS>()) {
+        return false;
+    } else {
+        if (nkt == NKT) return cls_fits<HS, NKT>();
+        return dispatch_cls_ok<HS, NKT + 2>(nkt);
     }
 }
 
@@ -1611,9 +1680,10 @@
 
 #define VIT_FA_DECLARE(HS)                                                                         \
     bool fa_forward_h##HS(bf16_t* out, float* lse, const bf16_t* qkv, int B, int T, int C, int NH, \
-                          hipStream_t s);                                                          \
+                          hipStream_t s, bool cls);                                                \
     int fa_backward_h##HS(bf16_t* dqkv, const bf16_t* dout, const bf16_t* qkv, const bf16_t* out, \
-                          const float* lse, int B, int T, int C, int NH, float* part, hipStream_t s); \
+                          const float* lse, int B, int T, int C, int NH, float* part, hipStream_t s, bool cls); \
+    bool fa_cls_ok_h##HS(int T);                                                                   \
     int fa_max_t_h##HS();
 VIT_FA_DECLARE(32)
 VIT_FA_DECLARE(64)
@@ -1623,13 +1693,14 @@
 
 #define VIT_FA_DEFINE(HS)                                                                           \
     bool fa_forward_h##HS(bf16_t* out, float* lse, const bf16_t* qkv, int B, int T, int C, int NH,  \
-                          hipStream_t s) {                                                          \
-        return fa::dispatch_fwd<HS>(cdiv(T, 32) * 2, out, lse, qkv, B, T, C, NH, s);                \
+                          hipStream_t s, bool cls) {                                                \
+        return fa::dispatch_fwd<HS>(cdiv(T, 32) * 2, out, lse, qkv, B, T, C, NH, s, cls);           \
     }                                                                                               \
     int fa_backward_h##HS(bf16_t* dqkv, const bf16_t* dout, const bf16_t* qkv, const bf16_t* out,   \
-                          const float* lse, int B, int T, int C, int NH, float* part, hipStream_t s) { \
-        return fa::dispatch_bwd<HS>(cdiv(T, 32) * 2, dqkv, dout, qkv, out, lse, B, T, C, NH, part, s); \
+                          const float* lse, int B, int T, int C, int NH, float* part, hipStream_t s, bool cls) { \
+        return fa::dispatch_bwd<HS>(cdiv(T, 32) * 2, dqkv, dout, qkv, out, lse, B, T, C, NH, part, s, cls); \
     }                                                                                               \
+    bool fa_cls_ok_h##HS(int T) { return fa::dispatch_cls_ok<HS>(cdiv(T, 32) * 2); }                \
     int fa_max_t_h##HS() { return fa::max_tp<HS>(); }
 
 }
diff --git a/vit.rs_amd/csrc/gemm.h b/vit.rs_amd/csrc/gemm.h
--- a/vit.rs_amd/csrc/gemm.h
+++ b/vit.rs_amd/csrc/gemm.h
@@ -35,6 +35,7 @@
     float* dbias = nullptr;
     float* colsum_out = nullptr;
     float* colsum_part = nullptr;
+    int colsum_row_mul = 0;
     int M = 0, N = 0, K = 0;
     int epi = EPI_F32_STORE;
     int splitk = 0;
diff --git a/vit.rs_amd/csrc/gemm.hip b/vit.rs_amd/csrc/gemm.hip
--- a/vit.rs_amd/csrc/gemm.hip
+++ b/vit.rs_amd/csrc/gemm.hip
@@ -985,6 +985,7 @@
 GemmParams make_gemm_params(const GemmArgs& a, int kchunk) {
     GemmParams p;
     p.A = a.A; p.B = a.B; p.C = a.C; p.C2 = a.C2; p.aux = a.aux; p.bias = a.bias; p.dbias = a.dbias; p.colsum_out = nullptr;
+    p.cs_row_mul = 0;
     p.lda = a.lda; p.ldb = a.ldb; p.ldc = a.ldc; p.ldaux = a.ldaux;
     if (g_debug_flags & 32) p.ldc = 0;
     p.M = a.M; p.N = a.N; p.K = a.K; p.kchunk = kchunk;
@@ -1235,6 +1236,12 @@
     }
     const bool gathered = a.rows_gathered && a.M >= 1 && a.a_kcontig && a.epi != EPI_F32_ATOMIC;
     const bool big = a.K % g2::KTILE == 0 && (a.M >= 256 || gathered) && a.N >= 256 && gemm_variant() != 1;
+    if (a.colsum_row_mul && !(big && gathered && epi_aux16(a.epi) && a.colsum_part && !a.colsum_out &&
+                              a.colsum_row_mul >= 128 && a.N % 8 == 0 && !pp_taken(a))) {
+        set_error("gemm_bf16: colsum_row_mul needs a row-gathered x-aux call on the 256x256 engine (M=%d N=%d K=%d)",
+                  a.M, a.N, a.K);
+        return;
+    }
     if (big) {
         const int tiles = cdiv(a.M, g2::BM) * cdiv(a.N, g2::BN);
         int split = 1;
@@ -1258,6 +1265,7 @@
         float* cs_rows = colsum_rows_begin(a);
         if ((a.colsum_out || a.colsum_part) && epi_aux16(a.epi) && !cs_rows) return;
         p.colsum_out = cs_rows;
+        p.cs_row_mul = a.colsum_row_mul;
         const bool late_db = a.dbias && !a.a_kcontig && split > 1;
         if (late_db) p.dbias = nullptr;
         if (split == 1 && pp_taken(b)) {
diff --git a/vit.rs_amd/csrc/gemm_common.h b/vit.rs_amd/csrc/gemm_common.h
--- a/vit.rs_amd/csrc/gemm_common.h
+++ b/vit.rs_amd/csrc/gemm_common.h
@@ -12,6 +12,7 @@
     const float* bias;
     float* dbias;
     float* colsum_out;
+    int cs_row_mul;
     long long lda, ldb, ldc, ldaux;
     int M, N, K;
     int kchunk;
@@ -268,8 +269,14 @@
                 v[2 * j + 1] *= hi;
             }
         }
-#pragma unroll
-        for (int j = 0; j < 8; j++) cs[j] += v[j];
+        if (p.cs_row_mul) {
+            float* q = p.colsum_out + (((long long)m * p.cs_row_mul) >> 7) * p.N + n;
+            reinterpret_cast<float4*>(q)[0] = make_float4(v[0] + 0.f, v[1] + 0.f, v[2] + 0.f, v[3] + 0.f);
+            reinterpret_cast<float4*>(q)[1] = make_float4(v[4] + 0.f, v[5] + 0.f, v[6] + 0.f, v[7] + 0.f);
+        } else {
+#pragma unroll
+            for (int j = 0; j < 8; j++) cs[j] += v[j];
+        }
         }
         const uint4 d8 = pack8(v);
         if (p.C) *reinterpret_cast<uint4*>((bf16_t*)p.C + off) = d8;
@@ -470,12 +477,15 @@
 }
 template <int EPI>
 __device__ __forceinline__ bool staged_interior(const GemmParams& p, int m0, int n0) {
+    if constexpr (epi_aux16(EPI)) {
+        if (p.cs_row_mul) return false;
+    }
     return EPI != EPI_F32_ATOMIC && m0 + 128 <= p.M && n0 + 64 <= p.N;
 }
 template <int EPI>
 __device__ __forceinline__ void staged_colsum(const GemmParams& p, int lane, int m0, int n0, float (&cs)[8]) {
     if constexpr (epi_aux16(EPI)) {
-        if (p.colsum_out) {
+        if (p.colsum_out && !p.cs_row_mul) {
             const int rr = lane >> 3, cc = (lane & 7) * 8;
 #pragma unroll
             for (int j = 0; j < 8; j++) {
diff --git a/vit.rs_amd/csrc/ops.hip b/vit.rs_amd/csrc/ops.hip
--- a/vit.rs_amd/csrc/ops.hip
+++ b/vit.rs_amd/csrc/ops.hip
@@ -371,6 +371,60 @@
             } else {
                 reinterpret_cast<float4*>(io.dinp + row * C)[k] = t;
             }
+        }
+    }
+    lnb_flush(io, sm, C);
+}
+
+template <int NV>
+__global__ __launch_bounds__(256) void ln_bwd_sel_k(LnbIo io, const bf16_t* __restrict__ dout, const float* inp,
+                                                    const float* __restrict__ weight, const float* __restrict__ mean,
+                                                    const float* __restrict__ rstd, long long rows, int C,
+                                                    long long rsel) {
+    extern __shared__ float sm[];
+    const int lane = threadIdx.x & 63, wave = threadIdx.x >> 6;
+    float4* pw = reinterpret_cast<float4*>(sm + wave * 3 * C);
+    float4* pb = reinterpret_cast<float4*>(sm + wave * 3 * C + C);
+    float4* ps = reinterpret_cast<float4*>(sm + wave * 3 * C + 2 * C);
+    float4 w4[NV];
+#pragma unroll
+    for (int j = 0; j < NV; j++) {
+        w4[j] = reinterpret_cast<const float4*>(weight)[lane + 64 * j];
+        pw[lane + 64 * j] = pb[lane + 64 * j] = ps[lane + 64 * j] = make_float4(0.f, 0.f, 0.f, 0.f);
+    }
+    const long long nwaves = (long long)gridDim.x * 4;
+    auto dec = [](float hf, uint32_t q8) { return __builtin_fmaf((float)(int)(int8_t)(uint8_t)q8, lo8_step(hf), hf); };
+    for (long long row = blockIdx.x * 4LL + wave; row < rows; row += nwaves) {
+        if (row % rsel) continue;
+        float4 dy[NV], xr[NV], ri[NV], nr[NV], dvv[NV];
+#pragma unroll
+        for (int j = 0; j < NV; j++) {
+            dy[j] = ld4(dout + row * C, lane + 64 * j);
+            xr[j] = reinterpret_cast<const float4*>(inp + row * C)[lane + 64 * j];
+            const float4 h = ld4(io.hi_in + row * C, lane + 64 * j);
+            const uint32_t q = reinterpret_cast<const uint32_t*>(io.lo_in + row * C)[lane + 64 * j];
+            ri[j] = make_float4(dec(h.x, q), dec(h.y, q >> 8), dec(h.z, q >> 16), dec(h.w, q >> 24));
+        }
+        ln_bwd_row<NV>(dy, xr, w4, mean[row], rstd[row], C, nr, dvv);
+#pragma unroll
+        for (int j = 0; j < NV; j++) {
+            const int k = lane + 64 * j;
+            float4 b = pb[k], w = pw[k], u = ps[k];
+            b.x += dy[j].x; b.y += dy[j].y; b.z += dy[j].z; b.w += dy[j].w;
+            w.x = __builtin_fmaf(nr[j].x, dy[j].x, w.x); w.y = __builtin_fmaf(nr[j].y, dy[j].y, w.y);
+            w.z = __builtin_fmaf(nr[j].z, dy[j].z, w.z); w.w = __builtin_fmaf(nr[j].w, dy[j].w, w.w);
+            pb[k] = b;
+            pw[k] = w;
+            const float4 dv = dvv[j];
+            const float4 t = make_float4(ri[j].x + dv.x, ri[j].y + dv.y, ri[j].z + dv.z, ri[j].w + dv.w);
+            u.x += t.x; u.y += t.y; u.z += t.z; u.w += t.w;
+            ps[k] = u;
+            const uint2 h = make_uint2(pack_bf16x2(t.x, t.y), pack_bf16x2(t.z, t.w));
+            reinterpret_cast<uint2*>(io.hi_out + row * C)[k] = h;
+            reinterpret_cast<uint32_t*>(io.lo_out + row * C)[k] =
+                lo8_encode(t.x, __uint_as_float(h.x << 16)) | (lo8_encode(t.y, __uint_as_float(h.x & 0xffff0000u)) << 8) |
+                (lo8_encode(t.z, __uint_as_float(h.y << 16)) << 16) |
+                (lo8_encode(t.w, __uint_as_float(h.y & 0xffff0000u)) << 24);
         }
     }
     lnb_flush(io, sm, C);
@@ -734,7 +788,7 @@
 template <typename TD, bool ST>
 static void ln_backward_any(LnbIo io, const TD* dout, const float* inp, const float* w,
                             const float* mean, const float* rstd, long long rows, int C, hipStream_t s,
-                            float* ws = nullptr) {
+                            float* ws = nullptr, long long row_sel = 0) {
     if (rows <= 0) return;
     const bool reduce = io.part == nullptr;
     const int nsum = io.dsum ? 3 * C : 2 * C;
@@ -748,7 +802,32 @@
     const int grid = ln_bwd_blocks(rows);
     const size_t lds = 12 * (size_t)C * sizeof(float);
     if (lds > 160 * 1024) { set_error("layernorm_backward: C=%d exceeds the LDS column partials", C); return; }
-    if (!vec) {
+    if (row_sel > 0) {
+        if constexpr (ST && sizeof(TD) == 2) {
+            if (!vec || !ln_backward_row_sel_supported(C)) {
+                set_error("layernorm_backward: no selected-rows form for C=%d (or unaligned operands)", C);
+                return;
+            }
+#define VIT_LNS(NV)                                                                                     \
+    if (lds > 64 * 1024) VIT_HIP(hipFuncSetAttribute((const void*)ln_bwd_sel_k<NV>,                      \
+                                                     hipFuncAttributeMaxDynamicSharedMemorySize, (int)lds)); \
+    ln_bwd_sel_k<NV><<<grid, 256, lds, s>>>(io, dout, inp, w, mean, rstd, rows, C, row_sel)
+            switch (C / 256) {
+                case 1: VIT_LNS(1); break;
+                case 2: VIT_LNS(2); break;
+                case 3: VIT_LNS(3); break;
+                case 4: VIT_LNS(4); break;
+                case 5: VIT_LNS(5); break;
+                case 6: VIT_LNS(6); break;
+                case 7: VIT_LNS(7); break;
+                default: VIT_LNS(8); break;
+            }
+#undef VIT_LNS
+        } else {
+            set_error("layernorm_backward: the selected-rows form is the bf16 stream's");
+            return;
+        }
+    } else if (!vec) {
         if (lds > 64 * 1024) VIT_HIP(hipFuncSetAttribute((const void*)ln_bwd_k<TD, ST>,
                                                          hipFuncAttributeMaxDynamicSharedMemorySize, (int)lds));
         ln_bwd_k<TD, ST><<<grid, 256, lds, s>>>(io, dout, inp, w, mean, rstd, rows, C);
@@ -776,6 +855,7 @@
         rows_reduce_add(jobs, io.dsum ? 3 : 2, s);
     }
 }
+bool ln_backward_row_sel_supported(int C) { return C % 256 == 0 && C <= 2048; }
 int ln_bwd_blocks(long long rows) {
     const long long g = (rows + 15) / 16;
     return (int)(g < 1 ? 1 : (g > 768 ? 768 : g));
@@ -790,13 +870,13 @@
 void ln_backward_bf16_stream(bf16_t* dres_out, uint8_t* lo_out, const bf16_t* dres_in, const uint8_t* lo_in,
                              float* dw, float* db, float* dres_colsum, const bf16_t* dout, const float* inp,
                              const float* w, const float* mean, const float* rstd, long long rows, int C,
-                             hipStream_t s, float* part) {
+                             hipStream_t s, float* part, long long row_sel) {
     if (!dres_out || !lo_out || !dres_in || !lo_in) { set_error("layernorm_backward: the bf16 stream needs its 4 planes"); return; }
     if (((uintptr_t)lo_in | (uintptr_t)lo_out) & 3) { set_error("layernorm_backward: lo8 planes need 4-B alignment"); return; }
     LnbIo io{};
     io.hi_out = dres_out; io.lo_out = lo_out; io.hi_in = dres_in; io.lo_in = lo_in;
     io.dweight = dw; io.dbias = db; io.dsum = dres_colsum; io.part = part;
-    ln_backward_any<bf16_t, true>(io, dout, inp, w, mean, rstd, rows, C, s);
+    ln_backward_any<bf16_t, true>(io, dout, inp, w, mean, rstd, rows, C, s, nullptr, row_sel);
 }
 __global__ __launch_bounds__(256) void transpose_bf16_k(bf16_t* __restrict__ out,
                                                         const bf16_t* __restrict__ in, int R, int Cc,
diff --git a/vit.rs_amd/csrc/ops_internal.h b/vit.rs_amd/csrc/ops_internal.h
--- a/vit.rs_amd/csrc/ops_internal.h
+++ b/vit.rs_amd/csrc/ops_internal.h
@@ -15,7 +15,8 @@
 void ln_backward_bf16_stream(bf16_t* dres_out, uint8_t* lo_out, const bf16_t* dres_in, const uint8_t* lo_in,
                              float* dw, float* db, float* dres_colsum, const bf16_t* dout, const float* inp,
                              const float* w, const float* mean, const float* rstd, long long rows, int C,
-                             hipStream_t s, float* part = nullptr);
+                             hipStream_t s, float* part = nullptr, long long row_sel = 0);
+bool ln_backward_row_sel_supported(int C);
 int ln_bwd_blocks(long long rows);
 void convert_f2bf(bf16_t* out, const float* inp, long long n, hipStream_t s);
 void sgd(float* p, const float* g, long long n, float lr, hipStream_t s);
@@ -62,10 +63,12 @@
                        hipStream_t s);
 bool attn_fused_supported(int T, int C, int NH);
 bool attn_generic_supported(int T, int C, int NH);
+bool attn_last_cls_supported(int T, int C, int NH);
 void attn_forward_fused(bf16_t* out, float* lse, const bf16_t* qkv, int B, int T, int C, int NH,
-                        hipStream_t s);
+                        hipStream_t s, bool cls = false);
 size_t attn_backward_ws_floats(int B, int T, int C, int NH);
 void attn_backward_fused(bf16_t* dqkv, const bf16_t* dout, const bf16_t* qkv, const bf16_t* out,
                          const float* lse, int B, int T, int C, int NH, hipStream_t s,
-                         float* dqkv_colsum = nullptr, float* ws = nullptr, bool colsum_store = false);
+                         float* dqkv_colsum = nullptr, float* ws = nullptr, bool colsum_store = false,
+                         bool cls = false);
 }
diff --git a/vit.rs_amd/csrc/trainer.hip b/vit.rs_amd/csrc/trainer.hip
--- a/vit.rs_amd/csrc/trainer.hip
+++ b/vit.rs_amd/csrc/trainer.hip
@@ -686,6 +686,8 @@
                 VIT_HIP(hipMemsetAsync(a.ln2, 0, (size_t)BT * C * 2, s));
                 VIT_HIP(hipMemsetAsync(a.fchd, 0, (size_t)BT * 4 * C * 2, s));
                 VIT_HIP(hipMemsetAsync(a.fchg, 0, (size_t)BT * 4 * C * 2, s));
+                VIT_HIP(hipMemsetAsync(a.atty, 0, (size_t)BT * C * 2, s));
+                VIT_HIP(hipMemsetAsync(a.lse, 0, (size_t)BT * NH * 4, s));
             }
             dln_bf = alloc<bf16_t>(BT * C);
             dres_bf = alloc<bf16_t>(BT * C);
@@ -935,6 +937,13 @@
 
     bool last_cls = true;
     bool lc_active = false;
+    bool last_cls_attn = true;
+    bool lc_attn_active = false;
+    bool last_cls_bwd = true;
+    bool lc_bwd_active = false;
+    bool last_cls_bwd_on() const {
+        return last_cls_bwd && T >= 128 && (long long)(B / nmb) * T >= 256 && ln_backward_row_sel_supported(C);
+    }
     bool lc_dirty = true;
     bool lc_pending = false;
     bool last_cls_on() const { return last_cls && prec == VIT_BF16; }
@@ -948,6 +957,11 @@
         }
         VIT_HIP(hipMemsetAsync(dln_bf, 0, (size_t)BT * C * 2, cs));
         VIT_HIP(hipMemsetAsync(datty, 0, (size_t)BT * C * 2, cs));
+        if (lc_bwd_active) {
+            VIT_HIP(hipMemsetAsync(dfch, 0, (size_t)BT * 4 * C * 2, cs));
+            VIT_HIP(hipMemsetAsync(dres_bf2, 0, (size_t)BT * C * 2, cs));
+            VIT_HIP(hipMemsetAsync(dres_lo2, 0, (size_t)BT * C, cs));
+        }
         if (cs != s) {
             VIT_HIP(hipEventRecord(bev[EV_LC], cs));
             lc_pending = true;
@@ -1035,6 +1049,9 @@
         const int Bm = B / nmb;
         const long long R = (long long)Bm * T;
         lc_active = last_cls_on();
+        lc_attn_active = lc_active && last_cls_attn && attn_last_cls_supported(T, C, NH);
+        if (lc_active && last_cls_bwd_on() && !lc_bwd_active) lc_dirty = true;
+        lc_bwd_active = lc_active && last_cls_bwd_on();
         if (lc_active) last_cls_clear();
         mb_fork();
         for (int mb = 0; mb < nmb; mb++) {
@@ -1091,7 +1108,8 @@
                 gemm_w(TC_QKV_FWD, q, P_QKVW, l, false, mb, st, lm ? PRE_LN : PRE_NONE, false,
                        rc && !lm ? &c_ln1 : nullptr);
                 tbeg(TC_ATTN_FWD, 4.0 * Bm * (double)T * T * C, st);
-                attn_forward_fused(a.atty + r0 * C, a.lse + (long long)mb * Bm * NH * T, a.qkv + r0 * 3 * C, Bm, T, C, NH, st);
+                attn_forward_fused(a.atty + r0 * C, a.lse + (long long)mb * Bm * NH * T, a.qkv + r0 * 3 * C, Bm, T, C, NH, st,
+                                   lc && lc_attn_active);
                 tend();
                 GemmArgs pr;
                 pr.A = a.atty + r0 * C; pr.lda = rs * C; pr.B = W(P_ATTPROJW, l); pr.ldb = C; pr.C = a.res2 + r0 * C;
@@ -1233,6 +1251,11 @@
                 d1.M = (int)R; d1.N = 4 * C; d1.K = C; d1.epi = EPI_BF16_MUL;
                 fcb_rows = gemm_colsum_rows(d1, fp8());
                 d1.colsum_part = sg_rows(l, sg_fcb) + (long long)mb * fcb_rows * 4 * C;
+                if (lcg && lc_bwd_active && fcb_rows == (int)((R + 127) / 128)) {
+                    VIT_HIP(hipMemsetAsync(d1.colsum_part, 0, (size_t)fcb_rows * 4 * C * sizeof(float), ms[mb]));
+                    d1.lda = rs * C; d1.ldc = rs * 4 * C; d1.ldaux = rs * 4 * C; d1.M = Mr;
+                    d1.rows_gathered = true; d1.colsum_row_mul = T;
+                }
                 if (ec) {
                     d1.C = nullptr;
                     d1.mxc_q = dfchc.q; d1.mxc_s = dfchc.s; d1.mxc_ld = kp_tok; d1.mxc_off = r0;
@@ -1266,7 +1289,8 @@
                     ln_backward_bf16_stream(rbB + r0 * C, loB + r0 * C, rbA + r0 * C, loA + r0 * C, G(P_LN2W, l),
                                             G(P_LN2B, l), G(P_ATTPROJB, l), dln_bf + r0 * C, a.res2 + r0 * C,
                                             P(P_LN2W, l), a.ln2_mean + r0, a.ln2_rstd + r0, R, C, ms[mb],
-                                            sg_rows(l, sg_ln2) + (long long)mb * ln_bwd_blocks(R) * 3 * C);
+                                            sg_rows(l, sg_ln2) + (long long)mb * ln_bwd_blocks(R) * 3 * C,
+                                            lc && lc_bwd_active ? T : 0);
                 }
                 tend();
             }
@@ -1284,7 +1308,8 @@
                 attn_backward_fused(dqkv + r0 * 3 * C, datty + r0 * C, a.qkv + r0 * 3 * C, a.atty + r0 * C,
                                     a.lse + (long long)mb * Bm * NH * T, Bm, T, C, NH, ms[mb],
                                     sg_rows(l, sg_qkv) + (long long)mb * 3 * C,
-                                    attn_part + (long long)attn_backward_ws_floats(mb * Bm, T, C, NH), true);
+                                    attn_part + (long long)attn_backward_ws_floats(mb * Bm, T, C, NH), true,
+                                    lc && lc_attn_active);
                 tend();
             }
             if (rc) wgrad(TC_PROJ_WGRAD, rbB, C, a.atty, C, G(P_ATTPROJW, l), EV_RESB, EV_W3, &dcol[1], &c_atty);
@@ -2284,6 +2309,10 @@
         t.clip_overlap = value < 0 ? -1 : value != 0;
     } else if (n == "last_cls") {
         t.last_cls = value != 0;
+    } else if (n == "last_cls_bwd") {
+        t.last_cls_bwd = value != 0;
+    } else if (n == "last_cls_attn") {
+        t.last_cls_attn = value != 0;
     } else if (n == "dp_probe") {
         if (value && !t.dp_snap) {
             t.dp_snap = t.alloc<float>(t.arena_elems);
```

Measured after the change: 7355 images/s, median of 6. No clear change (+0.5%).
